# nlesc-dirac/sagecal

Measured on NVIDIA H100. Metric: baseline_visibilities_per_sec_predict_jacobian, higher is better.
Workload: dtype f64

## Files before the change

sagecal_b200/csrc/internal.cuh:

```cuda
#pragma once
#include <cuda_runtime.h>
#include <stdint.h>
#include <stdio.h>
#include <stdlib.h>

#define DB_CHECK(call)                                                                          \
  do {                                                                                          \
    cudaError_t err__ = (call);                                                                 \
    if (err__ != cudaSuccess) {                                                                 \
      fprintf(stderr, "dirac_b200: CUDA error %s at %s:%d: %s\n", cudaGetErrorName(err__),      \
              __FILE__, __LINE__, cudaGetErrorString(err__));                                   \
      exit(1);          \
    }                                                                                           \
  } while (0)


#define TILE_P 8
#define TILE_Q 32
#define TILE_THREADS (TILE_P * TILE_Q)

struct TileDesc {
  short pb, qb;
};

// ... 39 lines not shown
}
__host__ __device__ __forceinline__ double2 cadd(double2 a, double2 b) {
  return make_double2(a.x + b.x, a.y + b.y);
}
__host__ __device__ __forceinline__ double2 csub(double2 a, double2 b) {
  return make_double2(a.x - b.x, a.y - b.y);
}
__host__ __device__ __forceinline__ void cfma(double2 &acc, double2 a, double2 b) {
  acc.x = fma(a.x, b.x, acc.x);
  acc.x = fma(-a.y, b.y, acc.x);
  acc.y = fma(a.x, b.y, acc.y);
  acc.y = fma(a.y, b.x, acc.y);
}
__host__ __device__ __forceinline__ void cfmac(double2 &acc, double2 a, double2 b) {
  acc.x = fma(a.x, b.x, acc.x);
  acc.x = fma(a.y, b.y, acc.x);
  acc.y = fma(a.y, b.x, acc.y);
  acc.y = fma(-a.x, b.y, acc.y);
}
__host__ __device__ __forceinline__ void cfmacl(double2 &acc, double2 a, double2 b) {
  acc.x = fma(a.x, b.x, acc.x);
  acc.x = fma(a.y, b.y, acc.x);
  acc.y = fma(a.x, b.y, acc.y);
  acc.y = fma(-a.y, b.x, acc.y);
}

__host__ __device__ __forceinline__ double2 cdot2(double2 a0, double2 b0, double2 a1, double2 b1) {
  double re = a0.x * b0.x;
  re = fma(-a0.y, b0.y, re);
  re = fma(a1.x, b1.x, re);
  re = fma(-a1.y, b1.y, re);
  double im = a0.x * b0.y;
  im = fma(a0.y, b0.x, im);
  im = fma(a1.x, b1.y, im);
  im = fma(a1.y, b1.x, im);
  return make_double2(re, im);
}
__host__ __device__ __forceinline__ double2 cdot2c(double2 a0, double2 b0, double2 a1, double2 b1) {
  double re = a0.x * b0.x;
  re = fma(a0.y, b0.y, re);
  re = fma(a1.x, b1.x, re);
  re = fma(a1.y, b1.y, re);
  double im = a0.y * b0.x;
  im = fma(-a0.x, b0.y, im);
  im = fma(a1.y, b1.x, im);
  im = fma(-a1.x, b1.y, im);
  return make_double2(re, im);
}
__host__ __device__ __forceinline__ void cdot2c_acc(double2 &acc, double2 a0, double2 b0, double2 a1,
                                           double2 b1) {
  acc.x = fma(a0.x, b0.x, acc.x);
  acc.x = fma(a0.y, b0.y, acc.x);
  acc.x = fma(a1.x, b1.x, acc.x);
  acc.x = fma(a1.y, b1.y, acc.x);
  acc.y = fma(a0.y, b0.x, acc.y);
  acc.y = fma(-a0.x, b0.y, acc.y);
  acc.y = fma(a1.y, b1.x, acc.y);
  acc.y = fma(-a1.x, b1.y, acc.y);
}
__host__ __device__ __forceinline__ void mat_ab(const double2 *a, const double2 *b, double2 *c) {
  c[0] = cdot2(a[0], b[0], a[1], b[2]);
  c[1] = cdot2(a[0], b[1], a[1], b[3]);
  c[2] = cdot2(a[2], b[0], a[3], b[2]);
  c[3] = cdot2(a[2], b[1], a[3], b[3]);
}
__host__ __device__ __forceinline__ void mat_abh(const double2 *a, const double2 *b, double2 *c) {
  c[0] = cdot2c(a[0], b[0], a[1], b[1]);
  c[1] = cdot2c(a[0], b[2], a[1], b[3]);
  c[2] = cdot2c(a[2], b[0], a[3], b[1]);
  c[3] = cdot2c(a[2], b[2], a[3], b[3]);
}
__host__ __device__ __forceinline__ void mat_abh_acc(const double2 *a, const double2 *b, double2 *c) {
  cdot2c_acc(c[0], a[0], b[0], a[1], b[1]);
  cdot2c_acc(c[1], a[0], b[2], a[1], b[3]);
  cdot2c_acc(c[2], a[2], b[0], a[3], b[1]);
  cdot2c_acc(c[3], a[2], b[2], a[3], b[3]);
}
__host__ __device__ __forceinline__ void mat_ahb(const double2 *a, const double2 *b, double2 *c) {
  c[0] = cadd(cmulcl(a[0], b[0]), cmulcl(a[2], b[2]));
  c[1] = cadd(cmulcl(a[0], b[1]), cmulcl(a[2], b[3]));
  c[2] = cadd(cmulcl(a[1], b[0]), cmulcl(a[3], b[2]));
  c[3] = cadd(cmulcl(a[1], b[1]), cmulcl(a[3], b[3]));
}

__device__ __forceinline__ double2 ld_stream(const double2 *p) {
  double2 v;
  asm volatile("ld.global.nc.L1::no_allocate.v2.f64 {%0,%1}, [%2];" : "=d"(v.x), "=d"(v.y) : "l"(p));
  return v;
}
__device__ __forceinline__ void st_stream(double2 *p, double2 v) {
  asm volatile("st.global.L1::no_allocate.v2.f64 [%0], {%1,%2};" ::"l"(p), "d"(v.x), "d"(v.y)
               : "memory");
}

__device__ __forceinline__ double warp_sum(double v) {
#pragma unroll
  for (int o = 16; o > 0; o >>= 1) v += __shfl_xor_sync(0xffffffffu, v, o);
  return v;
}

__device__ __forceinline__ void load_jones(const double *pblk, int sta, double2 *J) {
  const double2 *s = reinterpret_cast<const double2 *>(pblk + 8 * (long long)sta);
  J[0] = __ldg(s + 0);
  J[1] = __ldg(s + 1);
  J[2] = __ldg(s + 2);
  J[3] = __ldg(s + 3);
}

__device__ __forceinline__ int row_chunk(long long r, long long R, int nchunk) {
  return nchunk == 1 ? 0 : (int)(r / ((R + nchunk - 1) / nchunk));
}

struct GradArgs {
  const double2 *coh;
  const double2 *res;
  const unsigned char *flag;
  const double *pp;
  const ClusterDesc *clus;
  const int *chunk_poff;
  const TileDesc *tiles;
  double *g;
  long long R;
  int N, Nbase, tilesz, M;
  int robust;
  double nu;
  double scale;
  int tb0;
  long long w_lo, w_hi;
};

struct ClusterPassArgs {
  const double2 *coh_k;
  const double2 *in;
  const unsigned char *flag;
  const double *pblk;
  const TileDesc *tiles;
  double2 *out;
  double *jte;
  double *partials;
  double *cost;
  unsigned int *counter;
  long long R;
  int N, Nbase;
  int t_begin, t_end, tslice;
  int mode;
  int write_out;
  double beta;
  const double *pblk_old;
  int form_hidden;
  const short2 *blpq;
  double *jte_part;
  unsigned int *gcounter;
  const double2 *wt;
};

struct WeightedJtjArgs {
  const double2 *coh_k;
  const double2 *wt;
  const unsigned char *flag;
  const double *pblk;
  const TileDesc *tiles;
  double *JTJ;
  double *HP, *HQ;
  long long R;
  int N, Nbase;
  int t_begin, t_end, tslice;
};

struct StreamAllArgs {
  const double2 *coh;
  const double2 *x;
  const unsigned char *flag;
  const double *pp;
  const double *pk;
  const ClusterDesc *clus;
  const int *chunk_poff;
  const short2 *blpq;
  double2 *out;
  double2 *E0, *E1, *E2;
  double *poly_part;
  double *partials, *cost;
  unsigned int *counter;
  long long R;
  int N, Nbase, tilesz, M;
  int out_mode, cost_mode;
  double inv_nu;
  int partial;
  long long row0;
  long long w_lo, w_hi;
};

struct GramArgs {
  const double2 *coh;
  const unsigned char *flag;
  const TileDesc *tiles;
  double *T;
  long long R;
  int N, Nbase;
  int k0;
  int t_begin, t_end, t_step;
};

struct AssembleArgs {
  const double *T;
  const double *pblk;
  const int *list;
  const int *tix;
  const int *poff;
  double *JTJ;
  long long stride;
  double *Hst;
  const double *mu_dev;
  double mu;
  int lower;
  int N, Nbase;
};

enum { DB_OPT_CP_ROWS = 0, DB_OPT_LINE_DIRECT = 1, DB_OPT_OS_CONSISTENT = 2,
       DB_OPT_RTR_NU_UNJOINED = 3, DB_OPT_ADMM_LM = 4, DB_OPT_SWEEP_RESIDUAL = 5,
       DB_OPT_COUNT = 8 };
int db_opt(int id);
int db_sm_count();
static inline int db_cp_max_slices(int Nbase, int tilesz) {
  const int nbg = (Nbase + 255) / 256;
  int nsl = (db_sm_count() + nbg - 1) / nbg;
  if ((tilesz + 31) / 32 > nsl) nsl = (tilesz + 31) / 32;
  return nsl;
}

extern "C" {
void db_launch_coh_to_planar(const double2 *src, double2 *dst, long long r0, int nr, int M,
                             long long R, cudaStream_t st);
void db_launch_coh_from_planar(const double2 *src, double2 *dst, long long r0, int nr, int M,
                               long long R, cudaStream_t st);
void db_launch_vis_to_planar(const double2 *src, double2 *dst, long long R, cudaStream_t st);
void db_launch_vis_from_planar(const double2 *src, double2 *dst, long long R, cudaStream_t st);
void db_launch_grad_tma(const GradArgs *a, int ntile, cudaStream_t st);
void db_launch_grad_window_tma(const GradArgs *a, int ntile, long long r_lo, long long r_hi,
                               cudaStream_t st);
void db_launch_grad_band_tma(const GradArgs *a, int ntile, int nchan, cudaStream_t st);
int db_cluster_pass_nblocks(int ntile, int nt, int tslice);
enum { DB_CP_LIN = 0, DB_CP_LIN_GRAD = 1, DB_CP_SPLIT = 2, DB_CP_TILE = 3, DB_CP_NONE = 4 };
int db_launch_cluster_pass(const ClusterPassArgs *a, int ntile, cudaStream_t st);
int db_cluster_pass_forms_hidden(int N, int Nbase);
void db_launch_coh_gram(const GramArgs *a, int ntile, int nk, cudaStream_t st);
void db_launch_station_sums(const AssembleArgs *a, int nb, cudaStream_t st);
void db_launch_assemble_tiles(const AssembleArgs *a, int nb, cudaStream_t st);
void db_launch_batch_mu0(const double *Hst, double *mu, int N, double tau, int nb, cudaStream_t st);
void db_launch_copy_add_diag(const double *A0, double *A, int n, double mu, cudaStream_t st);
int db_chol_max_n();
int db_chol_available();
size_t db_chol_ws_doubles(int n);
int db_tri_available(int n);
void db_chol_set_step(const double *pcur, double *pnew, double *sc, double *zero);
void db_launch_tri_solve(const double *L, int n, const double *b, double *x, cudaStream_t st);
void db_launch_tri_solve_ld(const double *L, int ld, int n, const double *b, double *x,
                            cudaStream_t st);
void db_launch_chol_factor_batched(const double *A, int n, const double *mu, double *ws,
                                   long long ws_stride, int *info, int nb, cudaStream_t st);
void db_launch_chol_solve(const double *A, int n, double mu, const double *b, double *x, double *ws,
                          int *info, cudaStream_t st);
int db_bigtri_available(int n);
size_t db_bigtri_ws_doubles(int n);
void db_launch_bigtri_solve(const double *L, int ld, int n, const double *b, double *x, double *ws,
                            int *status, cudaStream_t st);
int db_stream_all_nblocks(int Nbase, int tilesz);
void db_launch_predict_tma(const StreamAllArgs *a, cudaStream_t st);
void db_launch_cost_window_tma(const StreamAllArgs *a, cudaStream_t st);
int db_band_nblocks(int Nbase, int tilesz, int nchan);
void db_launch_band_tma(const StreamAllArgs *a, int nchan, cudaStream_t st);
void db_launch_band_tma(const StreamAllArgs *a, int nchan, cudaStream_t st);
unsigned db_launch_line_setup_tma(const StreamAllArgs *a, cudaStream_t st);
void db_launch_line_poly_finish(const double *part, unsigned nparts, double *partials, double *out,
                                unsigned int *counter, cudaStream_t st);
void db_line_setup_shape_reset();
void db_line_setup_shape(int *shape);
}
```

sagecal_b200/csrc/kernels_stream.cu:

```cuda
#include "internal.cuh"
#include "tma.cuh"

#define XP_ROWS 8
__global__ void k_coh_to_planar(const double2 *__restrict__ src, double2 *__restrict__ dst,
                                long long r0, int nr, int M, long long R) {
  __shared__ double2 tile[4][XP_ROWS][33];
  const int kx = blockIdx.x * 32 + threadIdx.x;
  const int ry = blockIdx.y * XP_ROWS + threadIdx.y;
  if (kx < M && ry < nr) {
    const double2 *s = src + ((long long)ry * M + kx) * 4;
#pragma unroll
    for (int c = 0; c < 4; c++) tile[c][threadIdx.y][threadIdx.x] = s[c];
  }
  __syncthreads();
  const int tid = threadIdx.y * 32 + threadIdx.x;
  const int rr = tid % XP_ROWS, kk = tid / XP_ROWS;
  const int k = blockIdx.x * 32 + kk;
  const int r = blockIdx.y * XP_ROWS + rr;
  if (k < M && r < nr) {
#pragma unroll
    for (int c = 0; c < 4; c++) dst[((long long)k * 4 + c) * R + r0 + r] = tile[c][rr][kk];
  }
}

// ... 353 lines not shown
          }
          if (a.write_out) st_stream(a.out + (long long)c * a.R + row, o);
        }
      }
      if (a.mode <= 1) {
        if (a.wt) {
#pragma unroll
          for (int c = 0; c < 4; c++) {
            const double2 wv = ld_stream(a.wt + (long long)c * a.R + row);
            const double ex = wv.x * e[c].x, ey = wv.y * e[c].y;
            cost = fma(ex, ex, cost);
            cost = fma(ey, ey, cost);
            e[c] = make_double2(wv.x * ex, wv.y * ey);
          }
        } else {
#pragma unroll
          for (int c = 0; c < 4; c++) {
            cost = fma(e[c].x, e[c].x, cost);
            cost = fma(e[c].y, e[c].y, cost);
          }
        }
      }
    }
  }
  if (a.mode <= 1) grid_reduce_sum(cost, a.partials, a.cost, a.counter);
}

__global__ void __launch_bounds__(2 * TILE_THREADS)
k_cluster_pass_split(ClusterPassArgs a) {
  __shared__ double sq[2 * TILE_P][8][TILE_Q];
  const TileDesc td = a.tiles[blockIdx.x];
  const int h = threadIdx.x >> 8, w = (threadIdx.x >> 5) & 7, lane = threadIdx.x & 31;
  const int p = td.pb * TILE_P + w;
  const int q = td.qb * TILE_Q + lane;
  const bool valid = (q > p) && (q < a.N);
  const int ts = a.t_begin + blockIdx.y * a.tslice;
  const int te = min(ts + a.tslice, a.t_end);
  double cost = 0.0;
  double2 Jr[2], Jq[4], W[8];
#pragma unroll
  for (int z = 0; z < 8; z++) W[z] = make_double2(0.0, 0.0);
  Jr[0] = Jr[1] = make_double2(0.0, 0.0);
#pragma unroll
  for (int c = 0; c < 4; c++) Jq[c] = make_double2(0.0, 0.0);
  if (valid) {
    {
      const double2 *jp = reinterpret_cast<const double2 *>(a.pblk + 8 * (long long)p + 4 * h);
      Jr[0] = __ldg(jp);
      Jr[1] = __ldg(jp + 1);
    }
    load_jones(a.pblk, q, Jq);
    const long long b = baseline_index(p, q, a.N);
    const long long c0 = (long long)(2 * h) * a.R, c1 = c0 + a.R;
#pragma unroll 2
    for (int t = ts; t < te; t++) {
      const long long row = (long long)t * a.Nbase + b;
      double2 C[4], v[2];
#pragma unroll
      for (int c = 0; c < 4; c++) C[c] = ld_stream(a.coh_k + (long long)c * a.R + row);
      v[0] = ld_stream(a.in + c0 + row);
      v[1] = ld_stream(a.in + c1 + row);
      const bool fl = a.flag[row] != 0;
      const double2 T0 = cdot2(Jr[0], C[0], Jr[1], C[2]);
      const double2 T1 = cdot2(Jr[0], C[1], Jr[1], C[3]);
      double2 m[2];
      m[0] = cdot2c(T0, Jq[0], T1, Jq[1]);
      m[1] = cdot2c(T0, Jq[2], T1, Jq[3]);
      if (fl) m[0] = m[1] = make_double2(0.0, 0.0);
      double2 e[2];
      if (a.mode == 0) {
#pragma unroll
        for (int j = 0; j < 2; j++) {
          const double2 d = cadd(make_double2(a.beta * v[j].x, a.beta * v[j].y), m[j]);
          if (a.write_out) st_stream(a.out + (j ? c1 : c0) + row, d);
          e[j] = csub(d, m[j]);
        }
      } else {
#pragma unroll
        for (int j = 0; j < 2; j++) {
          e[j] = (a.mode == 4) ? v[j] : csub(v[j], m[j]);
          if (a.write_out) st_stream(a.out + (j ? c1 : c0) + row, e[j]);
        }
      }
      if (a.wt) {
#pragma unroll
        for (int j = 0; j < 2; j++) {
          const double2 wv = ld_stream(a.wt + (j ? c1 : c0) + row);
          const double ex = wv.x * e[j].x, ey = wv.y * e[j].y;
          cost = fma(ex, ex, cost);
          cost = fma(ey, ey, cost);
          e[j] = make_double2(wv.x * ex, wv.y * ey);
        }
      } else {
#pragma unroll
        for (int j = 0; j < 2; j++) {
          cost = fma(e[j].x, e[j].x, cost);
          cost = fma(e[j].y, e[j].y, cost);
        }
      }
      if (!fl) {
#pragma unroll
        for (int j = 0; j < 2; j++)
#pragma unroll
          for (int lm = 0; lm < 4; lm++) cfmac(W[j * 4 + lm], e[j], C[lm]);
      }
    }
  }
  double2 Gp[2], Gq[4];
  Gp[0] = Gp[1] = make_double2(0.0, 0.0);
#pragma unroll
  for (int c = 0; c < 4; c++) Gq[c] = make_double2(0.0, 0.0);
  if (valid) {
#pragma unroll
    for (int l = 0; l < 2; l++)
#pragma unroll
      for (int j = 0; j < 2; j++)
#pragma unroll
        for (int m = 0; m < 2; m++) cfma(Gp[l], Jq[2 * j + m], W[j * 4 + l * 2 + m]);
#pragma unroll
    for (int j = 0; j < 2; j++)
#pragma unroll
      for (int m = 0; m < 2; m++)
#pragma unroll
        for (int l = 0; l < 2; l++) cfmac(Gq[2 * j + m], Jr[l], W[j * 4 + l * 2 + m]);
  }
  {
    double vp[4];
    vp[0] = warp_sum(Gp[0].x);
    vp[1] = warp_sum(Gp[0].y);
    vp[2] = warp_sum(Gp[1].x);
    vp[3] = warp_sum(Gp[1].y);
    if (p < a.N - 1 && lane < 4) {
      double v = vp[0];
#pragma unroll
      for (int c = 1; c < 4; c++) v = (lane == c) ? vp[c] : v;
      atomicAdd(a.jte + 8 * (long long)p + 4 * h + lane, v);
    }
  }
#pragma unroll
  for (int c = 0; c < 4; c++) {
    sq[h * TILE_P + w][2 * c][lane] = Gq[c].x;
    sq[h * TILE_P + w][2 * c + 1][lane] = Gq[c].y;
  }
  __syncthreads();
  if (h == 0) {
    double s = 0.0;
#pragma unroll
    for (int ww = 0; ww < 2 * TILE_P; ww++) s += sq[ww][w][lane];
    if (q < a.N && s != 0.0) atomicAdd(a.jte + 8 * (long long)q + w, s);
  }
  grid_reduce_sum(cost, a.partials, a.cost, a.counter);
}

template <int NST, bool GRAD>
__global__ void __launch_bounds__(512)
k_cluster_pass_lin(ClusterPassArgs a) {
  extern __shared__ __align__(128) unsigned char smem_raw[];
  constexpr int BL = 256;
  constexpr int STAGE_ELEMS = 8 * BL;
  double2 *ring = reinterpret_cast<double2 *>(smem_raw);
  double *acc = reinterpret_cast<double *>(ring + (size_t)NST * STAGE_ELEMS);
  unsigned long long *bars = reinterpret_cast<unsigned long long *>(acc + ((8 * a.N + 1) & ~1));
  const int tid = threadIdx.x, h = tid >> 8, bl = tid & (BL - 1);
  const long long b0 = (long long)blockIdx.x * BL;
  const int nvalid = (int)min((long long)BL, (long long)a.Nbase - b0);
  const bool valid = bl < nvalid;
  const int ts = a.t_begin + blockIdx.y * a.tslice;
  const int te = min(ts + a.tslice, a.t_end);
  const int nrow = te - ts;
  if (GRAD)
    for (int i = tid; i < 8 * a.N; i += 512) acc[i] = 0.0;
  if (tid == 0) {
#pragma unroll
    for (int s = 0; s < NST; s++) mbar_init(&bars[s], 1);
    mbar_fence_init();
  }
  __syncthreads();
  auto issue = [&](int j, int s) {
    const unsigned row_bytes = (unsigned)nvalid * 16u;
    const long long row0 = (long long)(ts + j) * a.Nbase + b0;
    double2 *dst = ring + (size_t)s * STAGE_ELEMS;
    mbar_expect_tx(&bars[s], 8u * row_bytes);
#pragma unroll
    for (int c = 0; c < 4; c++) {
      bulk_g2s(dst + c * BL, a.coh_k + (long long)c * a.R + row0, row_bytes, &bars[s]);
      bulk_g2s(dst + (4 + c) * BL, a.in + (long long)c * a.R + row0, row_bytes, &bars[s]);
    }
  };
  if (tid == 0) {
#pragma unroll
    for (int s = 0; s < NST - 1; s++)
      if (s < nrow) issue(s, s);
  }
  int p = 0, q = 0;
  double2 Jr[2], Jq[4], W[8];
#pragma unroll
  for (int z = 0; z < 8; z++) W[z] = make_double2(0.0, 0.0);
  Jr[0] = Jr[1] = make_double2(0.0, 0.0);
#pragma unroll
  for (int c = 0; c < 4; c++) Jq[c] = make_double2(0.0, 0.0);
  unsigned flagbits = 0;
  const long long b = b0 + bl;
  const bool recover = (!GRAD) && a.mode == 3 && a.pblk_old != nullptr && !a.form_hidden;
  const bool old_model = recover || a.form_hidden;
  const double gamma = recover ? (1.0 - a.beta) / a.beta : 0.0;
  double2 Jro[2], Jqo[4];
  Jro[0] = Jro[1] = make_double2(0.0, 0.0);
#pragma unroll
  for (int c = 0; c < 4; c++) Jqo[c] = make_double2(0.0, 0.0);
  auto load_old_jones = [&]() {
    const double2 *jo = reinterpret_cast<const double2 *>(a.pblk_old + 8 * (long long)p + 4 * h);
    Jro[0] = __ldg(jo);
    Jro[1] = __ldg(jo + 1);
    load_jones(a.pblk_old, q, Jqo);
  };
  if (valid) {
    const short2 pq = a.blpq[b];
    p = pq.x;
    q = pq.y;
    const double2 *jp = reinterpret_cast<const double2 *>(a.pblk + 8 * (long long)p + 4 * h);
    Jr[0] = __ldg(jp);
    Jr[1] = __ldg(jp + 1);
    load_jones(a.pblk, q, Jq);
    if (old_model && !GRAD) load_old_jones();
    for (int j = 0; j < nrow; j++)
      flagbits |= (a.flag[(long long)(ts + j) * a.Nbase + b] != 0 ? 1u : 0u) << j;
  }
  const long long c0 = (long long)(2 * h) * a.R, c1 = c0 + a.R;
  double cost = 0.0;
  for (int j = 0; j < nrow; j++) {
    const int s = j % NST;
    if (tid == 0 && j + NST - 1 < nrow) issue(j + NST - 1, (j + NST - 1) % NST);
    mbar_wait(&bars[s], (unsigned)((j / NST) & 1));
    if (valid) {
      const double2 *st = ring + (size_t)s * STAGE_ELEMS + bl;
      const long long row = (long long)(ts + j) * a.Nbase + b;
      double2 C[4], v[2];
#pragma unroll
      for (int c = 0; c < 4; c++) C[c] = lds_v2(st + c * BL);
      v[0] = lds_v2(st + (4 + 2 * h) * BL);
      v[1] = lds_v2(st + (5 + 2 * h) * BL);
      const bool fl = (flagbits >> j) & 1u;
      const double2 T0 = cdot2(Jr[0], C[0], Jr[1], C[2]);
      const double2 T1 = cdot2(Jr[0], C[1], Jr[1], C[3]);
      double2 m[2];
      m[0] = cdot2c(T0, Jq[0], T1, Jq[1]);
      m[1] = cdot2c(T0, Jq[2], T1, Jq[3]);
      if (fl) m[0] = m[1] = make_double2(0.0, 0.0);
      double2 mo[2];
      if (old_model) {
        if (GRAD) load_old_jones();
        const double2 U0 = cdot2(Jro[0], C[0], Jro[1], C[2]);
        const double2 U1 = cdot2(Jro[0], C[1], Jro[1], C[3]);
        mo[0] = cdot2c(U0, Jqo[0], U1, Jqo[1]);
        mo[1] = cdot2c(U0, Jqo[2], U1, Jqo[3]);
        if (fl) mo[0] = mo[1] = make_double2(0.0, 0.0);
      }
      if (a.form_hidden) {
#pragma unroll
        for (int jj = 0; jj < 2; jj++)
          v[jj] = cadd(make_double2(a.beta * v[jj].x, a.beta * v[jj].y), mo[jj]);
      }
      double2 e[2];
      if (a.mode == 0 || a.mode == 2) {
#pragma unroll
        for (int jj = 0; jj < 2; jj++) {
          const double2 d = cadd(make_double2(a.beta * v[jj].x, a.beta * v[jj].y), m[jj]);
          if (a.write_out) st_stream(a.out + (jj ? c1 : c0) + row, d);
          e[jj] = csub(d, m[jj]);
        }
      } else {
#pragma unroll
        for (int jj = 0; jj < 2; jj++) {
          e[jj] = csub(v[jj], m[jj]);
          double2 o = e[jj];
          if (recover) {
            o.x = fma(gamma, v[jj].x - mo[jj].x, o.x);
            o.y = fma(gamma, v[jj].y - mo[jj].y, o.y);
          }
          if (a.write_out) st_stream(a.out + (jj ? c1 : c0) + row, o);
        }
      }
      if (a.mode <= 1) {
#pragma unroll
        for (int jj = 0; jj < 2; jj++) {
          cost = fma(e[jj].x, e[jj].x, cost);
          cost = fma(e[jj].y, e[jj].y, cost);
        }
      }
      if (GRAD && !fl) {
#pragma unroll
        for (int jj = 0; jj < 2; jj++)
#pragma unroll
          for (int lm = 0; lm < 4; lm++) cfmac(W[jj * 4 + lm], e[jj], C[lm]);
      }
    }
    __syncthreads();
  }
  if (!GRAD) {
    if (a.mode <= 1) grid_reduce_sum(cost, a.partials, a.cost, a.counter);
    return;
  }
  double2 Gp[2], Gq[4];
  Gp[0] = Gp[1] = make_double2(0.0, 0.0);
#pragma unroll
  for (int c = 0; c < 4; c++) Gq[c] = make_double2(0.0, 0.0);
  if (valid) {
#pragma unroll
    for (int l = 0; l < 2; l++)
#pragma unroll
      for (int jj = 0; jj < 2; jj++)
#pragma unroll
        for (int m = 0; m < 2; m++) cfma(Gp[l], Jq[2 * jj + m], W[jj * 4 + l * 2 + m]);
#pragma unroll
    for (int jj = 0; jj < 2; jj++)
#pragma unroll
      for (int m = 0; m < 2; m++)
#pragma unroll
        for (int l = 0; l < 2; l++) cfmac(Gq[2 * jj + m], Jr[l], W[jj * 4 + l * 2 + m]);
  }
  double *gq = reinterpret_cast<double *>(ring);
  double *gp = gq + 512 * 8;
#pragma unroll
  for (int c = 0; c < 4; c++) {
    gq[tid * 8 + 2 * c] = Gq[c].x;
    gq[tid * 8 + 2 * c + 1] = Gq[c].y;
  }
  gp[tid * 4 + 0] = Gp[0].x;
  gp[tid * 4 + 1] = Gp[0].y;
  gp[tid * 4 + 2] = Gp[1].x;
  gp[tid * 4 + 3] = Gp[1].y;
  __syncthreads();
  const int pmin = a.blpq[b0].x, pmax = a.blpq[b0 + nvalid - 1].x;
  for (int i = tid; i < 8 * a.N; i += 512) {
    const int sidx = i >> 3, comp = i & 7;
    double tot = 0.0;
    for (int pp = pmin; pp <= pmax && pp < sidx; pp++) {
      const long long bb = baseline_index(pp, sidx, a.N) - b0;
      if (bb >= 0 && bb < nvalid) tot += gq[bb * 8 + comp] + gq[(256 + bb) * 8 + comp];
    }
    if (sidx >= pmin && sidx <= pmax) {
      const int hh = comp >> 2, cc = comp & 3;
      long long bb = baseline_index(sidx, sidx + 1, a.N) - b0;
      long long be = bb + (a.N - 1 - sidx);
      if (bb < 0) bb = 0;
      if (be > nvalid) be = nvalid;
      for (; bb < be; bb++) tot += gp[(hh * 256 + bb) * 4 + cc];
    }
    acc[i] = tot;
  }
  {
    __shared__ bool last_of_group;
    const int n8 = 8 * a.N;
    double *grp = a.jte_part + (size_t)blockIdx.x * gridDim.y * n8;
    double *mine = grp + (size_t)blockIdx.y * n8;
    for (int i = tid; i < n8; i += 512) mine[i] = acc[i];
    __threadfence();
    __syncthreads();
    if (tid == 0) last_of_group = (atomicAdd(a.gcounter + blockIdx.x, 1u) == gridDim.y - 1);
    __syncthreads();
    if (last_of_group) {
      __threadfence();
      for (int i = tid; i < n8; i += 512) {
        double sacc = 0.0;
        for (unsigned c = 0; c < gridDim.y; c++) sacc += __ldcg(grp + (size_t)c * n8 + i);
        if (sacc != 0.0) atomicAdd(a.jte + i, sacc);
      }
      if (tid == 0) a.gcounter[blockIdx.x] = 0;
    }
  }
  grid_reduce_sum(cost, a.partials, a.cost, a.counter);
}


__global__ void __launch_bounds__(TILE_THREADS)
k_coh_gram(GramArgs a) {
  const TileDesc td = a.tiles[blockIdx.x];
  const int w = threadIdx.x >> 5, lane = threadIdx.x & 31;
  const int p = td.pb * TILE_P + w;
  const int q = td.qb * TILE_Q + lane;
  if (!((q > p) && (q < a.N))) return;
  const long long b = baseline_index(p, q, a.N);
  const double2 *ck = a.coh + (long long)(a.k0 + blockIdx.y) * 4 * a.R;
  double d[4] = {0.0, 0.0, 0.0, 0.0};
  double2 o[6];
#pragma unroll
  for (int z = 0; z < 6; z++) o[z] = make_double2(0.0, 0.0);
#pragma unroll 4
  for (int t = a.t_begin; t < a.t_end; t += a.t_step) {
    const long long row = (long long)t * a.Nbase + b;
    double2 C[4];
#pragma unroll
    for (int c = 0; c < 4; c++) C[c] = ld_stream(ck + (long long)c * a.R + row);
    if (a.flag[row] == 0) {
#pragma unroll
      for (int c = 0; c < 4; c++) {
        d[c] = fma(C[c].x, C[c].x, d[c]);
        d[c] = fma(C[c].y, C[c].y, d[c]);
      }
      cfmacl(o[0], C[0], C[1]);
      cfmacl(o[1], C[0], C[2]);
      cfmacl(o[2], C[0], C[3]);
      cfmacl(o[3], C[1], C[2]);
      cfmacl(o[4], C[1], C[3]);
      cfmacl(o[5], C[2], C[3]);
    }
  }
  double2 *Tb = reinterpret_cast<double2 *>(a.T + ((long long)blockIdx.y * a.Nbase + b) * 16);
  Tb[0] = make_double2(d[0], d[1]);
  Tb[1] = make_double2(d[2], d[3]);
#pragma unroll
  for (int z = 0; z < 6; z++) Tb[2 + z] = o[z];
}

void db_launch_grad_tma(const GradArgs *a, int ntile, cudaStream_t st) {
  constexpr int TB = 4, NST = 2;
  const size_t smem = sizeof(double) * 2 * TILE_P * 8 * TILE_Q +
                      (size_t)TILE_P * NST * TB * 4 * 32 * sizeof(double2) + TILE_P * NST * 8;
  static bool configured = false;
  if (!configured) {
    DB_CHECK(cudaFuncSetAttribute(k_grad_tma_split<TB, NST>,
                                  cudaFuncAttributeMaxDynamicSharedMemorySize, (int)smem));
    configured = true;
  }
  dim3 grid(ntile, (a->tilesz + TB - 1) / TB);
  k_grad_tma_split<TB, NST><<<grid, 2 * TILE_THREADS, smem, st>>>(*a);
}

void db_launch_grad_band_tma(const GradArgs *a, int ntile, int nchan, cudaStream_t st) {
  constexpr int TB = 4, NST = 2;
  const size_t smem = sizeof(double) * 2 * TILE_P * 8 * TILE_Q +
                      (size_t)TILE_P * NST * TB * 4 * 32 * sizeof(double2) + TILE_P * NST * 8;
  static bool configured = false;
  if (!configured) {
    DB_CHECK(cudaFuncSetAttribute(k_grad_tma_band<TB, NST>,
                                  cudaFuncAttributeMaxDynamicSharedMemorySize, (int)smem));
    configured = true;
  }
  dim3 grid(ntile, (a->tilesz + TB - 1) / TB, nchan);
  k_grad_tma_band<TB, NST><<<grid, 2 * TILE_THREADS, smem, st>>>(*a);
}

void db_launch_grad_window_tma(const GradArgs *a, int ntile, long long r_lo, long long r_hi,
                               cudaStream_t st) {
  constexpr int TB = 4, NST = 2;
  if (r_hi <= r_lo) return;
  const size_t smem = sizeof(double) * 2 * TILE_P * 8 * TILE_Q +
                      (size_t)TILE_P * NST * TB * 4 * 32 * sizeof(double2) + TILE_P * NST * 8;
  static bool configured = false;
  if (!configured) {
    DB_CHECK(cudaFuncSetAttribute(k_grad_tma_window<TB, NST>,
                                  cudaFuncAttributeMaxDynamicSharedMemorySize, (int)smem));
    configured = true;
  }
  const int t_lo = (int)(r_lo / a->Nbase), t_hi = (int)((r_hi + a->Nbase - 1) / a->Nbase);
  const int tb_lo = t_lo / TB, tb_hi = (t_hi + TB - 1) / TB;
  GradArgs b = *a;
  b.tb0 = tb_lo;
  b.w_lo = r_lo;
  b.w_hi = r_hi;
  dim3 grid(ntile, tb_hi - tb_lo);
  k_grad_tma_window<TB, NST><<<grid, 2 * TILE_THREADS, smem, st>>>(b);
}

static bool cluster_pass_lin_fits(int N, int Nbase) {
  return (size_t)5 * 8 * 256 * sizeof(double2) + sizeof(double) * ((8 * N + 1) & ~1) + 40 <=
             (size_t)200 * 1024 && (Nbase + 255) / 256 <= 1024;
}

template <bool GRAD>
static void launch_cluster_pass_lin(const ClusterPassArgs *a, cudaStream_t st) {
  constexpr int NST = 5;
  const int nt = a->t_end - a->t_begin;
  const int nbg = (a->Nbase + 255) / 256;
  int nsl = (db_sm_count() + nbg - 1) / nbg;
  if (nsl > nt) nsl = nt;
  ClusterPassArgs b = *a;
  b.tslice = (nt + nsl - 1) / nsl;
  const int forced = db_opt(DB_OPT_CP_ROWS);
  if (forced > 0 && (!GRAD || (nt + forced - 1) / forced <= db_cp_max_slices(a->Nbase, nt)))
    b.tslice = forced;
  if (b.tslice > nt) b.tslice = nt;
  if (b.tslice > 32) b.tslice = 32;
  const size_t smem = (size_t)NST * 8 * 256 * sizeof(double2) +
                      sizeof(double) * ((8 * a->N + 1) & ~1) + NST * 8;
  static bool configured = false;
  if (!configured) {
    DB_CHECK(cudaFuncSetAttribute(k_cluster_pass_lin<NST, GRAD>,
                                  cudaFuncAttributeMaxDynamicSharedMemorySize, 200 * 1024));
    configured = true;
  }
  dim3 grid(nbg, (nt + b.tslice - 1) / b.tslice);
  k_cluster_pass_lin<NST, GRAD><<<grid, 512, smem, st>>>(b);
}

extern "C" {

void db_launch_coh_to_planar(const double2 *src, double2 *dst, long long r0, int nr, int M,
                             long long R, cudaStream_t st) {
  dim3 block(32, XP_ROWS), grid((M + 31) / 32, (nr + XP_ROWS - 1) / XP_ROWS);
  k_coh_to_planar<<<grid, block, 0, st>>>(src, dst, r0, nr, M, R);
}
void db_launch_coh_from_planar(const double2 *src, double2 *dst, long long r0, int nr, int M,
                               long long R, cudaStream_t st) {
  dim3 block(32, XP_ROWS), grid((M + 31) / 32, (nr + XP_ROWS - 1) / XP_ROWS);
  k_coh_from_planar<<<grid, block, 0, st>>>(src, dst, r0, nr, M, R);
}
void db_launch_vis_to_planar(const double2 *src, double2 *dst, long long R, cudaStream_t st) {
  long long n = 4 * R;
  k_vis_to_planar<<<(unsigned)((n + 255) / 256), 256, 0, st>>>(src, dst, R);
}
void db_launch_vis_from_planar(const double2 *src, double2 *dst, long long R, cudaStream_t st) {
  long long n = 4 * R;
  k_vis_from_planar<<<(unsigned)((n + 255) / 256), 256, 0, st>>>(src, dst, R);
}

int db_cluster_pass_nblocks(int ntile, int nt, int tslice) { return ntile * ((nt + tslice - 1) / tslice); }
int db_cluster_pass_forms_hidden(int N, int Nbase) { return cluster_pass_lin_fits(N, Nbase); }
int db_launch_cluster_pass(const ClusterPassArgs *a, int ntile, cudaStream_t st) {
  int nt = a->t_end - a->t_begin;
  dim3 grid(ntile, (nt + a->tslice - 1) / a->tslice);
  if (a->form_hidden && (a->wt || !db_cluster_pass_forms_hidden(a->N, a->Nbase))) {
    fprintf(stderr, "dirac_b200: cluster pass that forms the hidden data requested where only the tile "
                    "kernels run (%s:%d)\n", __FILE__, __LINE__);
    exit(1);
  }
  const bool fits = cluster_pass_lin_fits(a->N, a->Nbase);
  if (a->jte == nullptr || (a->mode > 1 && a->mode != 4)) {
    if (!a->wt && fits) {
      launch_cluster_pass_lin<false>(a, st);
      return DB_CP_LIN;
    }
    k_cluster_pass<<<grid, TILE_THREADS, 0, st>>>(*a);
    return DB_CP_TILE;
  } else if (a->mode == 4 || a->wt || !fits) {
    k_cluster_pass_split<<<grid, 2 * TILE_THREADS, 0, st>>>(*a);
    return DB_CP_SPLIT;
  }
  launch_cluster_pass_lin<true>(a, st);
  return DB_CP_LIN_GRAD;
}
void db_launch_coh_gram(const GramArgs *a, int ntile, int nk, cudaStream_t st) {
  dim3 grid(ntile, nk);
  k_coh_gram<<<grid, TILE_THREADS, 0, st>>>(*a);
}

}
```

sagecal_b200/csrc/lm.cu:

```cuda
#include <float.h>
#include <math.h>
#include <string.h>
#include <vector>

#include "../../include/dirac_b200.h"
#include "problem.h"

#define CS_CHECK(call)                                                                     \
  do {                                                                                     \
    cusolverStatus_t s__ = (call);                                                         \
    if (s__ != CUSOLVER_STATUS_SUCCESS) {                                                  \
      fprintf(stderr, "dirac_b200: cuSOLVER error %d at %s:%d\n", (int)s__, __FILE__, __LINE__); \
      exit(1);                                                                             \
    }                                                                                      \
  } while (0)
#define CB_CHECK(call)                                                                     \
  do {                                                                                     \
    cublasStatus_t s__ = (call);                                                           \
    if (s__ != CUBLAS_STATUS_SUCCESS) {                                                    \
      fprintf(stderr, "dirac_b200: cuBLAS error %d at %s:%d\n", (int)s__, __FILE__, __LINE__); \
      exit(1);                                                                             \
    }                                                                                      \
  } while (0)

extern "C" {
void db_launch_weighted_jtj(const WeightedJtjArgs *a, int ntile, cudaStream_t st);
void db_launch_sum_abs(const double2 *v, long long R, long long r0, long long r1, double *partials,
                       double *out, unsigned int *counter, cudaStream_t st);
void db_launch_update_weights(const double2 *e, double2 *wt, long long R, long long r0,
                              long long r1, double nu0, double *partials, double *out,
                              unsigned int *counter, cudaStream_t st);
void db_launch_scale_vis(double2 *v, long long R, long long r0, long long r1, double alpha,
                         int set_const, cudaStream_t st);
void db_launch_extract_diag(const double *A, double *dst, int n, cudaStream_t st);
void db_launch_lm_step(const double *p, const double *Dp, const double *jte, double *pnew,
                       double *sc, double *zero, int n, cudaStream_t st);
void db_launch_os_shift(const double2 *e, const double2 *wt, double2 *eps, double2 *wout, long long R,
                        long long row_sub0, long long nrow_sub, long long row_chunk0, long long kl,
                        long long nJ, cudaStream_t st);
}

template <typename T>
static T *dalloc(size_t n) {
  return (T *)db_malloc(n * sizeof(T) + 16);
}

void db_lm_init(dirac_b200_problem *pr) {
  LMWork &w = pr->lm;
  if (w.ready) return;
  DevProblem &d = pr->d;
  const int n8 = 8 * d.N;
  w.n8 = n8;
  w.T = dalloc<double>((size_t)d.Mt * d.Nbase * 16);
  w.T_valid = (unsigned char *)calloc(d.Mt, 1);
  w.Tsub = dalloc<double>((size_t)d.Nbase * 16);
  w.JTJ0 = dalloc<double>((size_t)n8 * n8);
  w.JTJ = dalloc<double>((size_t)n8 * n8);
  w.JTe = d.scal + 64 + n8;
  w.JTe_new = d.scal + 64 + 2 * n8;
  w.Hst = dalloc<double>((size_t)4 * d.N);
  w.Dp = d.scal + 64;
  w.pnew = dalloc<double>(n8);
  w.plast = dalloc<double>(n8);
  w.pold = dalloc<double>(n8);
  w.devinfo = reinterpret_cast<int *>(d.scal + 64 + 3 * n8);
  w.tau = dalloc<double>(n8);
  w.svdS = w.svdU = w.svdVT = nullptr;
  w.wbuf = w.ebuf = nullptr;
  w.os_eps = w.os_w = nullptr;
  w.HP = w.HQ = nullptr;
  w.JB = w.LB = nullptr;
  w.sys_T = w.sys_p = w.sys_H = nullptr;
  w.pref_slot = (int *)malloc(sizeof(int) * d.M);
  for (int k = 0; k < d.M; k++) w.pref_slot[k] = -1;
  w.jtj0_cur = nullptr;
  w.jtj_spec = nullptr;
  {
    const int nbg = (d.Nbase + 255) / 256;
    const int nsl = db_cp_max_slices(d.Nbase, d.tilesz);
    w.jte_part = dalloc<double>((size_t)nbg * (nsl + 1) * n8);
  }
  DB_CHECK(cudaEventCreateWithFlags(&w.ev_mail, cudaEventDisableTiming));
  DB_CHECK(cudaMallocHost((void **)&w.h_vec, sizeof(double) * (5 * n8 + 4 * d.N + 64)));
  static cusolverDnHandle_t g_cs = nullptr;
  static cublasHandle_t g_cb = nullptr;
  if (!g_cs) {
    CS_CHECK(cusolverDnCreate(&g_cs));
    CB_CHECK(cublasCreate(&g_cb));
  }
  w.cs = g_cs;
  w.cb = g_cb;
  CS_CHECK(cusolverDnSetStream(w.cs, d.stream));
  CB_CHECK(cublasSetStream(w.cb, d.stream));
  int l1 = 0, l2 = 0, l3 = 0;
  CS_CHECK(cusolverDnDpotrf_bufferSize(w.cs, CUBLAS_FILL_MODE_LOWER, n8, w.JTJ, n8, &l1));
  CS_CHECK(cusolverDnDgeqrf_bufferSize(w.cs, n8, n8, w.JTJ, n8, &l2));
  CS_CHECK(cusolverDnDormqr_bufferSize(w.cs, CUBLAS_SIDE_LEFT, CUBLAS_OP_T, n8, 1, n8, w.JTJ, n8,
                                       w.tau, w.Dp, n8, &l3));
  w.lwork = l1 > l2 ? l1 : l2;
  if (l3 > w.lwork) w.lwork = l3;
  int l4 = 0;
  CS_CHECK(cusolverDnDgesvd_bufferSize(w.cs, n8, n8, &l4));
  if (l4 > w.lwork) w.lwork = l4;
  w.own_chol = n8 <= db_chol_max_n() && db_chol_available() && !getenv("DIRAC_B200_CUSOLVER");
  if (w.own_chol && (size_t)w.lwork < db_chol_ws_doubles(n8)) w.lwork = (int)db_chol_ws_doubles(n8);
  w.cswork = dalloc<double>((size_t)w.lwork);
  w.bc = (!w.own_chol && n8 > 1024) ? db_bigchol_create(n8, BC_BLOCK, BC_INV_PANEL, BC_LOOKAHEAD) : nullptr;
  w.bt_ws = (!w.own_chol && db_bigtri_available(n8)) ? dalloc<double>(db_bigtri_ws_doubles(n8)) : nullptr;
  w.dbuf = dalloc<double2>((size_t)4 * d.R);
  w.ready = true;
}

static void robust_init(dirac_b200_problem *pr) {
  LMWork &w = pr->lm;
  if (w.wbuf) return;
  DevProblem &d = pr->d;
  w.wbuf = dalloc<double2>((size_t)4 * d.R);
  w.ebuf = dalloc<double2>((size_t)4 * d.R);
  w.HP = dalloc<double>((size_t)d.N * 20);
  w.HQ = dalloc<double>((size_t)d.N * 20);
}

static void os_init(dirac_b200_problem *pr) {
  robust_init(pr);
  LMWork &w = pr->lm;
  if (w.os_eps) return;
  w.os_eps = dalloc<double2>((size_t)4 * pr->d.R);
  w.os_w = dalloc<double2>((size_t)4 * pr->d.R);
}

void db_lm_free(dirac_b200_problem *pr) {
  LMWork &w = pr->lm;
  if (!w.ready) return;
  db_free(w.T); db_free(w.Tsub); db_free(w.JTJ0); db_free(w.JTJ);
  db_free(w.Hst); db_free(w.pnew); db_free(w.plast); db_free(w.pold); db_free(w.jte_part);
  db_free(w.tau); db_free(w.cswork); db_free(w.dbuf);
  if (w.bt_ws) db_free(w.bt_ws);
  db_bigchol_destroy(w.bc);
  if (w.svdS) { db_free(w.svdS); db_free(w.svdU); db_free(w.svdVT); }
  if (w.wbuf) { db_free(w.wbuf); db_free(w.ebuf); db_free(w.HP); db_free(w.HQ); }
  if (w.os_eps) { db_free(w.os_eps); db_free(w.os_w); }
  if (w.LB) {
    if (w.JB) db_free(w.JB);
    db_free(w.LB); db_free(w.HB); db_free(w.mu_dev); db_free(w.binfo_dev);
    db_free(w.LBptr_dev); db_free(w.blist_dev); db_free(w.btix_dev); db_free(w.bpoff_dev);
    cudaFreeHost(w.h_mu); cudaFreeHost(w.h_binfo);
  }
  free(w.pref_slot);
  cudaEventDestroy(w.ev_mail);
  cudaFreeHost(w.h_vec);
  free(w.T_valid);
  w.ready = false;
}

static int pick_tslice(const DevProblem &d, int nt) {
  int target_ctas = db_sm_count();
  int slices = (target_ctas + d.ntile - 1) / d.ntile;
  if (slices < 1) slices = 1;
  int ts = (nt + slices - 1) / slices;
  if (ts < 2) ts = 2;
  if (ts > nt) ts = nt;
  if (ts < 1) ts = 1;
  return ts;
}

int db_cluster_pass(dirac_b200_problem *pr, int k, const double *pblk_dev, const double2 *in,
                    double2 *out, int mode, int write_out, double *jte_dev, int cost_slot, int t0,
                    int t1, const double2 *wt, double beta = 1.0, bool jte_zeroed = false,
                    const double *pblk_old = nullptr, bool form_hidden = false);

int db_cluster_pass(dirac_b200_problem *pr, int k, const double *pblk_dev, const double2 *in,
                    double2 *out, int mode, int write_out, double *jte_dev, int cost_slot, int t0,
                    int t1, const double2 *wt, double beta, bool jte_zeroed,
                    const double *pblk_old, bool form_hidden) {
  DevProblem &d = pr->d;
  if (t1 <= t0) {
    if (mode <= 1 || mode == 4)
      DB_CHECK(cudaMemsetAsync(d.scal + cost_slot, 0, sizeof(double), d.stream));
    if (jte_dev) DB_CHECK(cudaMemsetAsync(jte_dev, 0, sizeof(double) * 8 * d.N, d.stream));
    return DB_CP_NONE;
  }
  ClusterPassArgs a;
  a.coh_k = d.coh + (size_t)k * 4 * d.R;
  a.in = in; a.flag = d.flag; a.pblk = pblk_dev; a.tiles = d.tiles; a.out = out; a.jte = jte_dev;
  a.blpq = d.blpq; a.jte_part = pr->lm.jte_part; a.gcounter = d.counters + 16;
  a.partials = pr->partials; a.cost = d.scal + cost_slot; a.counter = d.counters; a.R = d.R;
  a.N = d.N; a.Nbase = d.Nbase; a.t_begin = t0; a.t_end = t1; a.tslice = pick_tslice(d, t1 - t0);
  a.mode = mode; a.write_out = write_out; a.wt = wt; a.beta = beta;
  a.pblk_old = pblk_old; a.form_hidden = form_hidden;
  if (!(jte_dev && (mode <= 1 || mode == 4)) && a.tslice > 1)
    a.tslice = (a.tslice + 1) / 2;
  if (jte_dev && (mode <= 1 || mode == 4) && !jte_zeroed)
    DB_CHECK(cudaMemsetAsync(jte_dev, 0, sizeof(double) * 8 * d.N, d.stream));
  db_prof_begin((jte_dev && (mode <= 1 || mode == 4)) ? 2 : 8, (double)(t1 - t0) * d.Nbase * (129.0 + (write_out ? 64.0 : 0.0) +
                                                 (wt ? 64.0 : 0.0)), d.stream);
  const int kernel = db_launch_cluster_pass(&a, d.ntile, d.stream);
  db_prof_end(d.stream);
  db_count_launch(1);
  return kernel;
}

static void gram(dirac_b200_problem *pr, int k, int t0, int t1, int step, double *Tdst) {
  DevProblem &d = pr->d;
  GramArgs a;
  a.coh = d.coh; a.flag = d.flag; a.tiles = d.tiles; a.T = Tdst; a.R = d.R; a.N = d.N;
  a.Nbase = d.Nbase; a.k0 = k; a.t_begin = t0; a.t_end = t1; a.t_step = step;
  db_prof_begin(3, (double)((t1 - t0 + step - 1) / step) * d.Nbase * 65.0 + 128.0 * d.Nbase,
                d.stream);
  db_launch_coh_gram(&a, d.ntile, 1, d.stream);
  db_prof_end(d.stream);
  db_count_launch(1);
}

static AssembleArgs assemble_args(const DevProblem &d, const double *T, const double *pblk_dev,
                                  double *Hst) {
  AssembleArgs a;
  memset(&a, 0, sizeof(a));
  a.T = T; a.pblk = pblk_dev; a.Hst = Hst; a.N = d.N; a.Nbase = d.Nbase;
  return a;
}

static void station_sums(dirac_b200_problem *pr, const AssembleArgs &a, int nb) {
  DevProblem &d = pr->d;
  db_prof_begin(4, nb * 256.0 * d.Nbase, d.stream);
  db_launch_station_sums(&a, nb, d.stream);
  db_prof_end(d.stream);
  db_count_launch(1);
}

static void assemble_tiles(dirac_b200_problem *pr, const AssembleArgs &a, int nb) {
  DevProblem &d = pr->d;
  const double n = 8.0 * d.N;
  db_prof_begin(4, nb * (a.lower ? 128.0 * d.Nbase + 4.0 * n * (n + 1) : 256.0 * d.Nbase + 8.0 * n * n),
                d.stream);
  db_launch_assemble_tiles(&a, nb, d.stream);
  db_prof_end(d.stream);
  db_count_launch(1);
}

static void assemble(dirac_b200_problem *pr, const double *T, const double *pblk_dev,
                     double *JTJ) {
  AssembleArgs a = assemble_args(pr->d, T, pblk_dev, pr->lm.Hst);
  station_sums(pr, a, 1);
  if (!JTJ) return;
  a.JTJ = JTJ;
  assemble_tiles(pr, a, 1);
}

static void weighted_jtj(dirac_b200_problem *pr, int k, int t0, int t1, const double *pblk_dev,
                         const double2 *wt, double *JTJ) {
  DevProblem &d = pr->d;
  LMWork &w = pr->lm;
  const int n = w.n8;
  DB_CHECK(cudaMemsetAsync(JTJ, 0, sizeof(double) * (size_t)n * n, d.stream));
  DB_CHECK(cudaMemsetAsync(w.HP, 0, sizeof(double) * 20 * d.N, d.stream));
  DB_CHECK(cudaMemsetAsync(w.HQ, 0, sizeof(double) * 20 * d.N, d.stream));
  if (t1 <= t0) return;
  WeightedJtjArgs a;
  a.coh_k = d.coh + (size_t)k * 4 * d.R;
  a.wt = wt; a.flag = d.flag; a.pblk = pblk_dev; a.tiles = d.tiles; a.JTJ = JTJ; a.HP = w.HP;
  a.HQ = w.HQ; a.R = d.R; a.N = d.N; a.Nbase = d.Nbase; a.t_begin = t0; a.t_end = t1;
  a.tslice = pick_tslice(d, t1 - t0);
  db_prof_begin(6, (double)(t1 - t0) * d.Nbase * 129.0 + 8.0 * 64.0 * d.N * d.N, d.stream);
  db_launch_weighted_jtj(&a, d.ntile, d.stream);
  db_prof_end(d.stream);
  db_count_launch(2);
}

void db_chunk_range(const DevProblem &d, int k, int ck, int *t0, int *t1);
static void chunk_range(const DevProblem &d, int k, int ck, int *t0, int *t1) {
  db_chunk_range(d, k, ck, t0, t1);
}
void db_chunk_range(const DevProblem &d, int k, int ck, int *t0, int *t1) {
  int nchunk = d.h_clus[k].nchunk;
  int tilechunk = (d.tilesz + nchunk - 1) / nchunk;
  int a = ck * tilechunk;
  int b = a + tilechunk;
  if (a > d.tilesz) a = d.tilesz;
  if (b > d.tilesz) b = d.tilesz;
  *t0 = a;
  *t1 = b;
}

static int enqueue_solve(dirac_b200_problem *pr, double mu, int linsolv, double eps1) {
  DevProblem &d = pr->d;
  LMWork &w = pr->lm;
  const int n = w.n8;
  int *hinfo = (int *)(w.h_vec + 4 * n + 4 * d.N);
  hinfo[0] = hinfo[1] = 0;
  if (linsolv == 0 && w.own_chol) {
    db_prof_begin(5, 0.0, d.stream);
    db_launch_chol_solve(w.jtj0_cur ? w.jtj0_cur : w.JTJ0, n, mu, w.JTe, w.Dp, w.cswork, w.devinfo,
                         d.stream);
    db_prof_end(d.stream);
    db_count_launch(1);
    w.step_fused = w.step_armed;
    return 1;
  }
  if (linsolv == 0 && w.sys_T) {
    AssembleArgs a = assemble_args(d, w.sys_T, w.sys_p, const_cast<double *>(w.sys_H));
    a.JTJ = w.JTJ;
    a.mu = mu;
    a.lower = 1;
    assemble_tiles(pr, a, 1);
  } else {
    db_prof_begin(4, 16.0 * n * n, d.stream);
    db_launch_copy_add_diag(w.jtj0_cur ? w.jtj0_cur : w.JTJ0, w.JTJ, n, mu, d.stream);
    db_prof_end(d.stream);
    db_count_launch(1);
  }
  if (linsolv != 0 || !w.bt_ws)
    DB_CHECK(cudaMemcpyAsync(w.Dp, w.JTe, sizeof(double) * n, cudaMemcpyDeviceToDevice, d.stream));
  db_prof_begin(5, 0.0, d.stream);
  if (linsolv == 0) {
    CS_CHECK(cusolverDnDpotrf(w.cs, CUBLAS_FILL_MODE_LOWER, n, w.JTJ, n, w.cswork, w.lwork,
                              w.devinfo));
    if (w.bt_ws) {
      db_launch_bigtri_solve(w.JTJ, n, n, w.JTe, w.Dp, w.bt_ws, w.devinfo + 1, d.stream);
      db_count_launch(2);
    } else {
      CS_CHECK(cusolverDnDpotrs(w.cs, CUBLAS_FILL_MODE_LOWER, n, 1, w.JTJ, n, w.Dp, n,
                                w.devinfo + 1));
      db_count_launch(2);
    }
  } else if (linsolv == 1) {
    CS_CHECK(cusolverDnDgeqrf(w.cs, n, n, w.JTJ, n, w.tau, w.cswork, w.lwork, w.devinfo));
    CS_CHECK(cusolverDnDormqr(w.cs, CUBLAS_SIDE_LEFT, CUBLAS_OP_T, n, 1, n, w.JTJ, n, w.tau, w.Dp,
                              n, w.cswork, w.lwork, w.devinfo + 1));
    const double one = 1.0;
    CB_CHECK(cublasDtrsm(w.cb, CUBLAS_SIDE_LEFT, CUBLAS_FILL_MODE_UPPER, CUBLAS_OP_N,
                         CUBLAS_DIAG_NON_UNIT, n, 1, &one, w.JTJ, n, w.Dp, n));
    db_count_launch(3);
  } else {
    if (!w.svdS) {
      w.svdS = dalloc<double>(n);
      w.svdU = dalloc<double>((size_t)n * n);
      w.svdVT = dalloc<double>((size_t)n * n);
    }
    CS_CHECK(cusolverDnDgesvd(w.cs, 'A', 'A', n, n, w.JTJ, n, w.svdS, w.svdU, n, w.svdVT, n,
                              w.cswork, w.lwork, nullptr, w.devinfo));
    db_count_launch(1);
    double *hS = (double *)malloc(sizeof(double) * n);
    double *hb = (double *)malloc(sizeof(double) * n);
    const double one = 1.0, zero = 0.0;
    CB_CHECK(cublasDgemv(w.cb, CUBLAS_OP_T, n, n, &one, w.svdU, n, w.JTe, 1, &zero, w.Dp, 1));
    DB_CHECK(cudaMemcpyAsync(hS, w.svdS, sizeof(double) * n, cudaMemcpyDeviceToHost, d.stream));
    DB_CHECK(cudaMemcpyAsync(hb, w.Dp, sizeof(double) * n, cudaMemcpyDeviceToHost, d.stream));
    db_stream_sync(d.stream);
// ... 95 lines not shown
  db_launch_batch_mu0(w.HB, w.mu_dev, d.N, tau, nb, d.stream);
  db_count_launch(1);
  if (keep_jb) {
    b.JTJ = w.JB;
    b.stride = (long long)nn;
    assemble_tiles(pr, b, nb);
  }
  if (!own_batch) {
    b.JTJ = w.LB;
    b.stride = (long long)lstride;
    b.mu_dev = w.mu_dev;
    b.lower = 1;
    assemble_tiles(pr, b, nb);
  }
  db_prof_begin(5, 0.0, d.stream);
  if (own_batch) {
    db_launch_chol_factor_batched(w.JB, n, w.mu_dev, w.LB, (long long)lstride, w.binfo_dev, nb,
                                  d.stream);
    db_count_launch(1);
  } else if (!w.bc) {
    CS_CHECK(cusolverDnDpotrfBatched(w.cs, CUBLAS_FILL_MODE_LOWER, n, w.LBptr_dev, n, w.binfo_dev, nb));
    db_count_launch(1);
  } else {
    db_bigchol_factor_batch(w.bc, nb, w.binfo_dev, 1, d.stream);
  }
  db_prof_end(d.stream);
  DB_CHECK(cudaMemcpyAsync(w.h_mu, w.mu_dev, sizeof(double) * nb, cudaMemcpyDeviceToHost, d.stream));
  DB_CHECK(cudaMemcpyAsync(w.h_binfo, w.binfo_dev, sizeof(int) * (own_batch ? 2 * nb : nb),
                           cudaMemcpyDeviceToHost, d.stream));
  w.binfo_step = own_batch ? 2 : 1;
  db_stream_sync(d.stream);
}

static long g_noise_decisions = 0;
static long g_lm_stat[4] = {0, 0, 0, 0};
extern "C" void dirac_b200_lm_stats(long *out4, int reset) {
  for (int i = 0; i < 4; i++) {
    if (out4) out4[i] = g_lm_stat[i];
    if (reset) g_lm_stat[i] = 0;
  }
}
extern "C" long dirac_b200_noise_decisions(int reset) {
  const long v = g_noise_decisions;
  if (reset) g_noise_decisions = 0;
  return v;
}

struct LmAug {
  const double *y_dev, *bz_dev;
  const double *y_host, *bz_host;
  double rho;
};
static const LmAug *g_aug = nullptr;
static std::vector<double> g_hpnew;
static double *hpnew_aug(LMWork &w) {
  if ((int)g_hpnew.size() < w.n8) g_hpnew.resize(w.n8);
  return g_hpnew.data();
}
static double aug_cost(const LmAug *a, const double *p, int n) {
  double s = 0.0;
  for (int i = 0; i < n; i++) {
    const double dlt = p[i] - a->bz_host[i];
    s += a->y_host[i] * dlt + 0.5 * a->rho * dlt * dlt;
  }
  return s;
}
extern "C" void db_launch_lm_aug_rhs(double *jte, const double *p, const double *y, const double *bz,
                                     double rho, int n, cudaStream_t st);

struct LmOut {
  double init_eL2, eL2, jacTe_inf, Dp_L2, mu;
  int k, stop;
  bool res_in_dbuf;
};

struct OsLayout {
  int Nsubsets, Ntper;
  bool misaligned;
};
static OsLayout os_layout(int ntiles) {
  OsLayout o;
  o.Nsubsets = ntiles < 10 ? ntiles : 10;
  o.Ntper = o.Nsubsets > 0 ? (ntiles + o.Nsubsets - 1) / o.Nsubsets : ntiles;
  o.misaligned = o.Nsubsets > 0 && (ntiles % o.Nsubsets) != 0 && !db_opt(DB_OPT_OS_CONSISTENT);
  return o;
}

struct OsPath {
  bool misaligned;
  int s0, s1;
  long long nJ;
};

static OsPath os_subset_system(dirac_b200_problem *pr, int k, int t0, int t1, int l,
                               const double *pblk_dev, const double2 *wt) {
  DevProblem &d = pr->d;
  LMWork &w = pr->lm;
  const int ntiles = t1 - t0;
  const OsLayout L = os_layout(ntiles);
  const int Ntper = L.Ntper;
  OsPath path;
  path.misaligned = L.misaligned;
  path.nJ = 0;
  int s0 = t0 + l * Ntper;
  int s1 = (l * Ntper + Ntper < ntiles) ? s0 + Ntper : t1;
  if (s0 > t1) s0 = t1;
  if (!L.misaligned) {
    db_cluster_pass(pr, k, pblk_dev, w.dbuf, nullptr, 1, 0, w.JTe, 2, s0, s1, wt);
    if (wt) {
      weighted_jtj(pr, k, s0, s1, pblk_dev, wt, w.JTJ0);
    } else {
      gram(pr, k, s0, s1, 1, w.Tsub);
      assemble(pr, w.Tsub, pblk_dev, w.JTJ0);
    }
  } else {
    const long long nn = 8ll * ntiles * d.Nbase;
    const long long Nper = (nn + L.Nsubsets - 1) / L.Nsubsets;
    const long long kl = (long long)l * Nper;
    const int tl = l * Ntper;
    long long Nos;
    int tileI;
    if (tl + Ntper < ntiles) {
      Nos = Nper;
      tileI = Ntper;
    } else {
      Nos = nn - kl;
      tileI = ntiles - tl;
    }
    long long nJ = tileI > 0 ? 8ll * d.Nbase * tileI : 0;
    if (Nos < nJ) nJ = Nos;
    if (nJ < 0) nJ = 0;
    s0 = t0 + tl;
    s1 = s0 + (tileI > 0 ? tileI : 0);
    if (s0 > t1) s0 = s1 = t1;
    os_init(pr);
    db_cluster_pass(pr, k, pblk_dev, w.dbuf, w.ebuf, 1, 1, nullptr, 2, t0, t1, nullptr);
    if (s1 > s0) {
      db_launch_os_shift(w.ebuf, wt, w.os_eps, w.os_w, d.R, (long long)s0 * d.Nbase,
                         (long long)(s1 - s0) * d.Nbase, (long long)t0 * d.Nbase, kl, nJ, d.stream);
      db_count_launch(1);
    }
    db_cluster_pass(pr, k, pblk_dev, w.os_eps, nullptr, 4, 0, w.JTe, 2, s0, s1, w.os_w);
    weighted_jtj(pr, k, s0, s1, pblk_dev, w.os_w, w.JTJ0);
    path.nJ = nJ;
  }
  path.s0 = s0;
  path.s1 = s1;
  return path;
}

static void lm_core(dirac_b200_problem *pr, int k, int ck, int t0, int t1, double *pblk_dev,
                    const double2 *wt, int itmax, const double *opts, int linsolv, int os,
                    int os_shift, int randomize, bool have_first, double first_cost, int *nu_damp,
                    bool *evaluated_trial, const double2 *hidden_from, LmOut *out) {
  DevProblem &d = pr->d;
  LMWork &w = pr->lm;
  const int n = w.n8;
  const int ntiles = t1 - t0;
  const double tau = opts[0], eps1 = opts[1], eps2 = opts[2], eps2_sq = opts[2] * opts[2],
               eps3 = opts[3];
  double *hp = w.h_vec;
  double *hjte = w.h_vec + n;
  double *hDp = w.h_vec + 2 * n;
  double *hpnew = w.h_vec + 3 * n;
  double *hH = w.h_vec + 4 * n;

  double p_eL2;
  const LmAug *aug = (!os && !wt) ? g_aug : nullptr;
  const double half_rho = aug ? 0.5 * aug->rho : 0.0;
  if (aug) w.pref_slot[k] = -1;
  const bool defer = have_first && !os && !wt && linsolv == 0 && itmax > 0 && w.pref_slot[k] >= 0 &&
                     std::isnan(first_cost);
  DB_CHECK(cudaMemcpyAsync(hp, pblk_dev, sizeof(double) * n, cudaMemcpyDeviceToHost, d.stream));
  if (aug && have_first)
    db_launch_lm_aug_rhs(w.JTe, pblk_dev, aug->y_dev, aug->bz_dev, aug->rho, n, d.stream);
  if (have_first) {
    p_eL2 = first_cost;
    if (!defer) {
      if (!os)
        DB_CHECK(cudaMemcpyAsync(hjte, w.JTe, sizeof(double) * n, cudaMemcpyDeviceToHost,
                                 d.stream));
      if (std::isnan(first_cost))
        DB_CHECK(cudaMemcpyAsync(d.h_scal + 2, d.scal + 2, sizeof(double), cudaMemcpyDeviceToHost,
                                 d.stream));
      db_stream_sync(d.stream);
      if (std::isnan(first_cost)) p_eL2 = d.h_scal[2];
    } else {
      p_eL2 = 1.0;
    }
  } else {
    db_cluster_pass(pr, k, pblk_dev, w.dbuf, nullptr, 1, 0, os ? nullptr : w.JTe, 1, t0, t1, wt);
    if (aug) db_launch_lm_aug_rhs(w.JTe, pblk_dev, aug->y_dev, aug->bz_dev, aug->rho, n, d.stream);
    if (!os)
      DB_CHECK(cudaMemcpyAsync(hjte, w.JTe, sizeof(double) * n, cudaMemcpyDeviceToHost, d.stream));
    p_eL2 = db_read_scalar(pr, 1);
  }
  if (aug && !defer) p_eL2 += aug_cost(aug, hp, n);
  double init_p_eL2 = p_eL2;
  int stop = 0;
  if (!isfinite(p_eL2)) stop = 7;
  int nu = *nu_damp, nu2;
  double mu = 0.0, Dp_L2 = DBL_MAX, jacTe_inf = 0.0;
  *evaluated_trial = false;
  bool res_in_dbuf = false;
  bool pending_entry = defer;
  w.jtj_spec = nullptr;
  int kiter_adjust = 0;

  const OsLayout osl = os_layout(ntiles);
  const int Nsubsets = osl.Nsubsets;
  const int max_os_iter = os ? (int)ceil(0.1 * (double)Nsubsets) : 1;
  const bool os_misaligned = os && osl.misaligned;

  const int tix = d.h_clus[k].chunk0 + ck;
  double *Tfull = w.T + (size_t)tix * d.Nbase * 16;
  if (!wt && !os && !w.T_valid[tix] && ntiles > 0) {
    gram(pr, k, t0, t1, 1, Tfull);
    w.T_valid[tix] = 1;
  }

  double *hsc = w.h_vec + 4 * n + 4 * d.N + 8;
  double *hjte_new = hpnew;
  int kiter;
  std::vector<int> subI;
  for (kiter = 0; kiter < itmax && !stop; ++kiter) {
    if (!pending_entry && p_eL2 <= eps3) {
      stop = 6;
      break;
    }
    if (os && randomize) {
      subI.resize(Nsubsets);
      for (int i = 0; i < Nsubsets; ++i) {
        const int j = rand() % (i + 1);
        subI[i] = subI[j];
        subI[j] = i;
      }
    }
    for (int ositer = 0; ositer < max_os_iter; ositer++) {
      double mx = 0.0;
      const int slot = (!wt && !os && kiter == 0 && linsolv == 0) ? w.pref_slot[k] : -1;
      const bool prefac = slot >= 0;
      const bool need_mx = (kiter == 0) && !prefac;
      w.jtj0_cur = (prefac && w.JB) ? w.JB + (size_t)slot * n * n : nullptr;
      const bool in_place = !w.own_chol && linsolv == 0 && !wt && !os;
      w.sys_T = in_place ? Tfull : nullptr;
      w.sys_p = pblk_dev;
      w.sys_H = prefac ? w.HB + (size_t)slot * 4 * d.N : w.Hst;
      if (os) {
        const int l = randomize ? subI[ositer] : (os_shift + kiter + ositer) % Nsubsets;
        os_subset_system(pr, k, t0, t1, l, pblk_dev, wt);
        DB_CHECK(cudaMemcpyAsync(hjte, w.JTe, sizeof(double) * n, cudaMemcpyDeviceToHost,
                                 d.stream));
      } else if (prefac) {
        w.pref_slot[k] = -1;
      } else if (wt) {
        weighted_jtj(pr, k, t0, t1, pblk_dev, wt, w.JTJ0);
      } else if (w.jtj_spec) {
        w.jtj0_cur = w.jtj_spec;
        w.jtj_spec = nullptr;
      } else {
        assemble(pr, Tfull, pblk_dev, in_place ? nullptr : w.JTJ0);
      }
      if (need_mx) {
        if (wt || os_misaligned) {
          db_launch_extract_diag(w.JTJ0, w.JTe_new, n, d.stream);
          db_count_launch(1);
          DB_CHECK(cudaMemcpyAsync(hsc, w.JTe_new, sizeof(double) * n, cudaMemcpyDeviceToHost,
                                   d.stream));
        } else {
          DB_CHECK(cudaMemcpyAsync(hH, w.Hst, sizeof(double) * 4 * d.N, cudaMemcpyDeviceToHost,
                                   d.stream));
        }
      }
      if (need_mx || os) db_stream_sync(d.stream);
      if (need_mx) {
        if (wt || os_misaligned) {
          for (int i = 0; i < n; i++)
            if (fabs(hsc[i]) > fabs(mx)) mx = hsc[i];
        } else {
          for (int s = 0; s < d.N; s++) {
            if (fabs(hH[4 * s]) > fabs(mx)) mx = hH[4 * s];
            if (fabs(hH[4 * s + 1]) > fabs(mx)) mx = hH[4 * s + 1];
          }
        }
      }
      double p_L2 = 0.0;
      if (!pending_entry) {
        jacTe_inf = 0.0;
        for (int i = 0; i < n; i++) {
          double a = fabs(hjte[i]);
          if (a > jacTe_inf) jacTe_inf = a;
        }
        p_L2 = nrm2sq(hp, n);
        if (jacTe_inf <= eps1) {
          Dp_L2 = 0.0;
          stop = 1;
          if (!os) kiter_adjust = 1;
          break;
        }
      }
      if (kiter == 0) mu = prefac ? w.h_mu[slot] : tau * (mx + half_rho);
      bool use_factor = prefac;
      while (1) {
        int issolved;
        bool skip_info = false;
        w.step_fused = false;
        w.step_armed = w.own_chol && linsolv == 0;
        if (w.step_armed)
          db_chol_set_step(pblk_dev, w.pnew, d.scal + 8, os ? nullptr : w.JTe_new);
        if (use_factor) {
          use_factor = false;
          db_prof_begin(5, 0.0, d.stream);
          if (w.own_chol && db_tri_available(n)) {
            skip_info = true;
            db_launch_tri_solve_ld(w.LB + (size_t)slot * w.lb_stride, w.lb_ld, n, w.JTe, w.Dp,
                                   d.stream);
            w.step_fused = w.step_armed;
          } else if (w.bt_ws) {
            skip_info = true;
            db_launch_bigtri_solve(w.LB + (size_t)slot * w.lb_stride, n, n, w.JTe, w.Dp, w.bt_ws,
                                   nullptr, d.stream);
          } else {
            DB_CHECK(cudaMemsetAsync(w.devinfo, 0, 2 * sizeof(int), d.stream));
            DB_CHECK(cudaMemcpyAsync(w.Dp, w.JTe, sizeof(double) * n, cudaMemcpyDeviceToDevice,
                                     d.stream));
            CS_CHECK(cusolverDnDpotrs(w.cs, CUBLAS_FILL_MODE_LOWER, n, 1,
                                      w.LB + (size_t)slot * w.lb_stride, n, w.Dp, n, w.devinfo + 1));
          }
          db_prof_end(d.stream);
          db_count_launch(1);
          issolved = (w.h_binfo[slot * w.binfo_step] == 0) ? 1 : 0;
        } else {
          issolved = enqueue_solve(pr, mu + half_rho, linsolv, eps1);
        }
        if (w.step_armed) db_chol_set_step(nullptr, nullptr, nullptr, nullptr);
        if (!w.step_fused)
          db_launch_lm_step(pblk_dev, w.Dp, w.JTe, w.pnew, d.scal + 8, os ? nullptr : w.JTe_new, n,
                            d.stream);
        if (hidden_from) {
          const bool last = kiter == itmax - 1;
          db_cluster_pass(pr, k, w.pnew, hidden_from, last ? w.dbuf : nullptr, 1, last ? 1 : 0,
                          last ? nullptr : w.JTe_new, 1, t0, t1, nullptr, 1.0, true, w.pold,
                          true);
        } else {
          db_cluster_pass(pr, k, w.pnew, w.dbuf, nullptr, 1, 0, os ? nullptr : w.JTe_new, 1, t0, t1,
                          wt, 1.0, true);
        }
        if (aug)
          db_launch_lm_aug_rhs(w.JTe_new, w.pnew, aug->y_dev, aug->bz_dev, aug->rho, n, d.stream);
        if (!w.step_fused) db_count_launch(1);
        int *hinfo = (int *)(w.h_vec + 4 * n + 4 * d.N);
        DB_CHECK(cudaMemcpyAsync(d.h_scal, d.scal, sizeof(double) * (64 + 3 * n + 2),
                                 cudaMemcpyDeviceToHost, d.stream));
        double *spec_buf = nullptr;
        if (w.own_chol && linsolv == 0 && !wt && !os && kiter + 1 < itmax && w.T_valid[tix]) {
          const double *cur = w.jtj0_cur ? w.jtj0_cur : w.JTJ0;
          spec_buf = (cur == w.JTJ0) ? w.JTJ : w.JTJ0;
          DB_CHECK(cudaEventRecord(w.ev_mail, d.stream));
          assemble(pr, Tfull, w.pnew, spec_buf);
          db_event_sync(w.ev_mail);
        } else {
          db_stream_sync(d.stream);
        }
        {
          const double *hm = d.h_scal + 64;
          memcpy(hDp, hm, sizeof(double) * n);
          hsc[n] = d.h_scal[8];
          hsc[n + 1] = d.h_scal[9];
          hsc[n + 2] = d.h_scal[1];
          if (!os) memcpy(hjte_new, hm + (w.JTe_new - w.Dp), sizeof(double) * n);
          if (pending_entry) memcpy(hjte, hm + (w.JTe - w.Dp), sizeof(double) * n);
          memcpy(hinfo, hm + 3 * n, 2 * sizeof(int));
          if (skip_info) hinfo[0] = hinfo[1] = 0;
        }
        if (pending_entry) {
          pending_entry = false;
          p_eL2 = init_p_eL2 = d.h_scal[2];
          if (!isfinite(p_eL2)) {
            stop = 7;
            kiter_adjust = 1;
            break;
          }
          if (p_eL2 <= eps3) {
            stop = 6;
            kiter_adjust = 1;
            break;
          }
          jacTe_inf = 0.0;
          for (int i = 0; i < n; i++) {
            double a = fabs(hjte[i]);
            if (a > jacTe_inf) jacTe_inf = a;
          }
          p_L2 = nrm2sq(hp, n);
          if (jacTe_inf <= eps1) {
            Dp_L2 = 0.0;
            stop = 1;
            kiter_adjust = 1;
            break;
          }
        }
        if (issolved && linsolv != 2) issolved = (hinfo[0] == 0 && hinfo[1] == 0) ? 1 : 0;
        if (issolved) {
          Dp_L2 = hsc[n];
          if (Dp_L2 <= eps2_sq * p_L2) {
            stop = 2;
            break;
          }
          if (Dp_L2 >= (p_L2 + eps2) / (1e-12 * 1e-12)) {
            stop = 4;
            break;
          }
          if (wt)
            DB_CHECK(cudaMemcpyAsync(w.plast, w.pnew, sizeof(double) * n, cudaMemcpyDeviceToDevice,
                                     d.stream));
          *evaluated_trial = true;
          double pDp_eL2 = hsc[n + 2];
          if (aug) {
            for (int i = 0; i < n; i++) hpnew_aug(w)[i] = hp[i] + hDp[i];
            pDp_eL2 += aug_cost(aug, hpnew_aug(w), n);
          }
          if (!isfinite(pDp_eL2)) {
            stop = 7;
            break;
          }
          const double dL = mu * Dp_L2 + hsc[n + 1];
          const double dF = p_eL2 - pDp_eL2;
          if (fabs(dF) <= 1e-11 * p_eL2) g_noise_decisions++;
          if (dL > 0.0 && dF > 0.0) {
            double tmp = (2.0 * dF / dL - 1.0);
            tmp = 1.0 - tmp * tmp * tmp;
            mu = mu * ((tmp >= 0.3333333334) ? tmp : 0.3333333334);
            g_lm_stat[0]++;
            if (!(tmp >= 0.3333333334)) g_lm_stat[1]++;
            nu = 2;
            for (int i = 0; i < n; i++) hp[i] += hDp[i];
            DB_CHECK(cudaMemcpyAsync(pblk_dev, w.pnew, sizeof(double) * n,
                                     cudaMemcpyDeviceToDevice, d.stream));
            if (!os) {
              memcpy(hjte, hjte_new, sizeof(double) * n);
              double *t = w.JTe; w.JTe = w.JTe_new; w.JTe_new = t;
            }
            p_eL2 = pDp_eL2;
            w.jtj_spec = spec_buf;
            res_in_dbuf = hidden_from && kiter == itmax - 1;
            break;
          }
        }
        g_lm_stat[2]++;
        mu *= (double)nu;
        nu2 = nu << 1;
        if (nu2 <= nu) {
          stop = 5;
          break;
        }
        nu = nu2;
      }
      if (stop) break;
    }
  }
  if (kiter >= itmax && !kiter_adjust) stop = 3;
  kiter -= kiter_adjust;
  *nu_damp = nu;
  out->init_eL2 = init_p_eL2;
  out->eL2 = p_eL2;
  out->jacTe_inf = jacTe_inf;
  out->Dp_L2 = Dp_L2;
  out->mu = mu;
  out->k = kiter;
  out->stop = stop;
  out->res_in_dbuf = res_in_dbuf;
}

static void fill_info(double *info, const LmOut &o) {
  if (!info) return;
  info[0] = o.init_eL2; info[1] = o.eL2; info[2] = o.jacTe_inf; info[3] = o.Dp_L2; info[4] = o.mu;
  info[5] = (double)o.k; info[6] = (double)o.stop;
  info[7] = info[8] = info[9] = 0.0;
}

void db_lm_set_aug(const double *y_dev, const double *bz_dev, const double *y_host,
                   const double *bz_host, double rho) {
  static LmAug a;
  if (!y_dev) {
    g_aug = nullptr;
    return;
  }
  a.y_dev = y_dev; a.bz_dev = bz_dev; a.y_host = y_host; a.bz_host = bz_host; a.rho = rho;
  g_aug = &a;
}

void db_lm_chunk(dirac_b200_problem *pr, int k, int ck, double *pblk_dev, double2 *r, int itmax,
                 const double *opts, int linsolv, int os, int randomize, double *info,
                 bool hidden_ready) {
  static const double defopts[4] = {1e-3, 1e-17, 1e-17, 1e-17};
  DevProblem &d = pr->d;
  db_lm_init(pr);
  LMWork &w = pr->lm;
  int t0, t1;
  chunk_range(d, k, ck, &t0, &t1);
  if (hidden_ready) {
    int nu = 2;
    bool ev;
    LmOut o;
    lm_core(pr, k, ck, t0, t1, pblk_dev, nullptr, itmax, opts ? opts : defopts, linsolv, os, 0,
            randomize, false, 0.0, &nu, &ev, nullptr, &o);
    fill_info(info, o);
    return;
  }
  const double beta = pr->world > 1 ? pr->beta : 1.0;
  const bool form = !os && pr->world <= 1 && d.h_clus[k].nchunk == 1 && r == pr->res &&
                    db_cluster_pass_forms_hidden(d.N, d.Nbase);
  if (beta != 1.0 || form)
    DB_CHECK(cudaMemcpyAsync(w.pold, pblk_dev, sizeof(double) * w.n8, cudaMemcpyDeviceToDevice,
                             d.stream));
  db_cluster_pass(pr, k, pblk_dev, r, form ? nullptr : w.dbuf, 0, form ? 0 : 1,
                  os ? nullptr : w.JTe, 2, t0, t1, nullptr, beta);
  const double c0 = nan("");
  int nu = 2;
  bool ev;
  LmOut o;
  lm_core(pr, k, ck, t0, t1, pblk_dev, nullptr, itmax, opts ? opts : defopts, linsolv, os, 0,
          randomize, true, c0, &nu, &ev, form ? r : nullptr, &o);
  if (o.res_in_dbuf) {
    pr->res = w.dbuf;
    w.dbuf = r;
  } else if (form) {
    db_cluster_pass(pr, k, pblk_dev, r, r, 3, 1, nullptr, 1, t0, t1, nullptr, 1.0, false,
                    w.pold, true);
  } else {
    db_cluster_pass(pr, k, pblk_dev, w.dbuf, r, 3, 1, nullptr, 1, t0, t1, nullptr, beta,
                    false, beta != 1.0 ? w.pold : nullptr);
  }
  fill_info(info, o);
}

bool db_cluster_needs_rowmap(const dirac_b200_problem *pr, int k) {
  const int nchunk = pr->d.h_clus[k].nchunk;
  return nchunk > 1 && (pr->d.tilesz % nchunk) != 0;
}
void db_cluster_hidden(dirac_b200_problem *pr, int k, double2 *r, int sign, double beta) {
  DevProblem &d = pr->d;
  db_lm_init(pr);
  LMWork &w = pr->lm;
  const double2 *coh_k = d.coh + (size_t)k * 4 * d.R;
  const int *poff = d.chunk_poff + d.h_clus[k].chunk0;
  if (sign > 0)
    db_launch_cluster_rowmap(coh_k, r, nullptr, w.dbuf, d.flag, d.pp, poff, d.h_clus[k].nchunk,
                             d.blpq, d.R, d.Nbase, 1, beta, d.stream);
  else
    db_launch_cluster_rowmap(coh_k, w.dbuf, beta != 1.0 ? r : nullptr, r, d.flag, d.pp, poff,
                             d.h_clus[k].nchunk, d.blpq, d.R, d.Nbase, -1, beta, d.stream);
  db_count_launch(1);
}

static double digamma_(double x) {
  double result = 0.0, xx, xx2, xx4;
  for (; x < 7.0; ++x) result -= 1.0 / x;
  x -= 0.5;
  xx = 1.0 / x;
  xx2 = xx * xx;
  xx4 = xx2 * xx2;
  result += log(x) + (1. / 24.) * xx2 - (7.0 / 960.0) * xx4 + (31.0 / 8064.0) * xx4 * xx2 -
            (127.0 / 30720.0) * xx4 * xx4;
  return result;
}

static double pick_nu(double sumq, double nulow, double nuhigh) {
  const int Nd = 30;
  const double deltanu = (nuhigh - nulow) / (double)Nd;
  int best = 0;
  double bestv = 0.0;
  for (int ci = 0; ci < Nd; ci++) {
    const double thisnu = nulow + (double)ci * deltanu;
    double q = digamma_(thisnu * 0.5 + 0.5) - log((thisnu + 1.0) * 0.5);
    q += -digamma_(thisnu * 0.5) + log(thisnu * 0.5);
    q += -sumq + 1.0;
    if (ci == 0 || fabs(q) < bestv) {
      bestv = fabs(q);
      best = ci;
    }
  }
  return nulow + (double)best * deltanu;
}

static double irls_update(dirac_b200_problem *pr, int k, int t0, int t1, const double *pe,
                          double nu0, double nulow, double nuhigh, double *out3) {
  DevProblem &d = pr->d;
  LMWork &w = pr->lm;
  const long long r0 = (long long)t0 * d.Nbase, r1 = (long long)t1 * d.Nbase;
  const double ndata = 8.0 * (double)(r1 - r0);
  db_cluster_pass(pr, k, pe, w.dbuf, w.ebuf, 1, 1, nullptr, 2, t0, t1, nullptr);
  db_launch_sum_abs(w.wbuf, d.R, r0, r1, pr->partials, d.scal + 3, d.counters, d.stream);
  db_launch_update_weights(w.ebuf, w.wbuf, d.R, r0, r1, nu0, pr->partials, d.scal + 4, d.counters,
                           d.stream);
  db_count_launch(2);
  DB_CHECK(cudaMemcpyAsync(d.h_scal + 3, d.scal + 3, 2 * sizeof(double), cudaMemcpyDeviceToHost,
                           d.stream));
  db_stream_sync(d.stream);
  const double lambda = d.h_scal[3];
  const double sumq = d.h_scal[4] / ndata;
  const double nu = pick_nu(sumq, nulow, nuhigh);
  db_launch_scale_vis(w.wbuf, d.R, r0, r1, lambda / ndata, 0, d.stream);
  db_count_launch(1);
  if (out3) {
    out3[0] = lambda;
    out3[1] = sumq;
    out3[2] = nu;
  }
  return nu;
}

void db_rlm_chunk(dirac_b200_problem *pr, int k, int ck, double *pblk_dev, double2 *r, int itmax,
                  int linsolv, int os, int randomize, double nulow, double nuhigh,
                  double *robust_nu, double *info, bool hidden_ready) {
  static const double defopts[4] = {1e-3, 1e-17, 1e-17, 1e-17};
  const int wt_itmax = 3;
  DevProblem &d = pr->d;
  db_lm_init(pr);
  robust_init(pr);
  LMWork &w = pr->lm;
  const int n8 = w.n8;
  int t0, t1;
  chunk_range(d, k, ck, &t0, &t1);
  const long long r0 = (long long)t0 * d.Nbase, r1 = (long long)t1 * d.Nbase;
  const double beta = pr->world > 1 ? pr->beta : 1.0;
  if (!hidden_ready) {
    if (beta != 1.0)
      DB_CHECK(cudaMemcpyAsync(w.pold, pblk_dev, sizeof(double) * w.n8, cudaMemcpyDeviceToDevice,
                               d.stream));
    db_cluster_pass(pr, k, pblk_dev, r, w.dbuf, 2, 1, nullptr, 1, t0, t1, nullptr, beta);
  }
  if (r1 > r0) db_launch_scale_vis(w.wbuf, d.R, r0, r1, 1.0, 1, d.stream);
  db_count_launch(1);
  double nu_t = *robust_nu;
  int nu = 2;
  LmOut o;
  memset(&o, 0, sizeof(o));
  for (int nw = 0; nw < wt_itmax; nw++) {
    bool evaluated = false;
    lm_core(pr, k, ck, t0, t1, pblk_dev, w.wbuf, itmax, defopts, linsolv, os, nw, randomize, false,
            0.0, &nu, &evaluated, nullptr, &o);
    if (nw < wt_itmax - 1 && r1 > r0) {
      const double *pe = (nw == 0 && evaluated) ? w.plast : pblk_dev;
      nu_t = irls_update(pr, k, t0, t1, pe, nu_t, nulow, nuhigh, nullptr);
    }
  }
  *robust_nu = nu_t;
  if (!hidden_ready)
    db_cluster_pass(pr, k, pblk_dev, w.dbuf, r, 3, 1, nullptr, 1, t0, t1, nullptr, beta, false,
                    beta != 1.0 ? w.pold : nullptr);
  (void)n8;
  fill_info(info, o);
}

extern "C" double dirac_b200_normal_eq(dirac_b200_problem *pr, int clus, int chunk,
                                       const double *pblk, const double *xd, double *JTJ,
                                       double *JTe) {
  DevProblem &d = pr->d;
  db_lm_init(pr);
  LMWork &w = pr->lm;
  const int n = w.n8;
  int t0, t1;
  chunk_range(d, clus, chunk, &t0, &t1);
  db_upload_vis(pr, xd, w.dbuf);
  DB_CHECK(cudaMemcpyAsync(w.pnew, pblk, sizeof(double) * n, cudaMemcpyHostToDevice, d.stream));
  db_cluster_pass(pr, clus, w.pnew, w.dbuf, nullptr, 1, 0, w.JTe, 1, t0, t1, nullptr);
  gram(pr, clus, t0, t1, 1, w.Tsub);
  assemble(pr, w.Tsub, w.pnew, w.JTJ0);
  double c = db_read_scalar(pr, 1);
  if (JTe) DB_CHECK(cudaMemcpy(JTe, w.JTe, sizeof(double) * n, cudaMemcpyDeviceToHost));
  if (JTJ)
    DB_CHECK(cudaMemcpy(JTJ, w.JTJ0, sizeof(double) * (size_t)n * n, cudaMemcpyDeviceToHost));
  DB_CHECK(cudaGetLastError());
  return c;
}

extern "C" double dirac_b200_normal_eq_weighted(dirac_b200_problem *pr, int clus, int chunk,
                                                const double *pblk, const double *xd,
                                                const double *wt, double *JTJ, double *JTe) {
  DevProblem &d = pr->d;
  db_lm_init(pr);
// ... 8 lines not shown
  db_cluster_pass(pr, clus, w.pnew, w.dbuf, nullptr, 1, 0, w.JTe, 1, t0, t1, w.wbuf);
  weighted_jtj(pr, clus, t0, t1, w.pnew, w.wbuf, w.JTJ0);
  double c = db_read_scalar(pr, 1);
  if (JTe) DB_CHECK(cudaMemcpy(JTe, w.JTe, sizeof(double) * n, cudaMemcpyDeviceToHost));
  if (JTJ)
    DB_CHECK(cudaMemcpy(JTJ, w.JTJ0, sizeof(double) * (size_t)n * n, cudaMemcpyDeviceToHost));
  DB_CHECK(cudaGetLastError());
  return c;
}

extern "C" void dirac_b200_assemble_damped(dirac_b200_problem *pr, int clus, int chunk,
                                           const double *pblk, int nmu, const double *mus,
                                           int factor, double *out, int *info) {
  DevProblem &d = pr->d;
  db_lm_init(pr);
  LMWork &w = pr->lm;
  const int n = w.n8;
  int t0, t1;
  chunk_range(d, clus, chunk, &t0, &t1);
  DB_CHECK(cudaMemcpyAsync(w.pnew, pblk, sizeof(double) * n, cudaMemcpyHostToDevice, d.stream));
  gram(pr, clus, t0, t1, 1, w.Tsub);
  assemble(pr, w.Tsub, w.pnew, nullptr);
  for (int i = 0; i < nmu; i++) {
    AssembleArgs a = assemble_args(d, w.Tsub, w.pnew, w.Hst);
    a.JTJ = w.JTJ;
    a.mu = mus[i];
    a.lower = 1;
    assemble_tiles(pr, a, 1);
    if (factor)
      CS_CHECK(cusolverDnDpotrf(w.cs, CUBLAS_FILL_MODE_LOWER, n, w.JTJ, n, w.cswork, w.lwork,
                                w.devinfo));
    DB_CHECK(cudaMemcpyAsync(out + (size_t)i * n * n, w.JTJ, sizeof(double) * (size_t)n * n,
                             cudaMemcpyDeviceToHost, d.stream));
    if (factor)
      DB_CHECK(cudaMemcpyAsync(info + i, w.devinfo, sizeof(int), cudaMemcpyDeviceToHost, d.stream));
    db_stream_sync(d.stream);
  }
  DB_CHECK(cudaGetLastError());
}

extern "C" void dirac_b200_assemble_batch(dirac_b200_problem *pr, const double *pp, const int *list,
                                          int nb, double tau, int lower, double *mu_out, double *out) {
  DevProblem &d = pr->d;
  db_lm_init(pr);
  DB_CHECK(cudaMemcpy(d.pp, pp, sizeof(double) * d.npar, cudaMemcpyHostToDevice));
  LMWork &w = pr->lm;
  const size_t nn = (size_t)w.n8 * w.n8;
  std::vector<int> tix(d.M), poff(d.M);
  for (int k = 0; k < d.M; k++) {
    tix[k] = d.h_clus[k].chunk0;
    poff[k] = d.h_chunk_poff[tix[k]];
  }
  for (int y = 0; y < nb; y++) {
    const int k = list[y];
    int t0, t1;
    chunk_range(d, k, 0, &t0, &t1);
    gram(pr, k, t0, t1, 1, w.T + (size_t)tix[k] * d.Nbase * 16);
    w.T_valid[tix[k]] = 1;
  }
  int *ibuf = dalloc<int>(nb + 2 * d.M);
  double *H = dalloc<double>((size_t)4 * d.N * nb), *mu = dalloc<double>(nb);
  double *A = dalloc<double>(nn * nb);
  DB_CHECK(cudaMemcpy(ibuf, list, sizeof(int) * nb, cudaMemcpyHostToDevice));
  DB_CHECK(cudaMemcpy(ibuf + nb, tix.data(), sizeof(int) * d.M, cudaMemcpyHostToDevice));
  DB_CHECK(cudaMemcpy(ibuf + nb + d.M, poff.data(), sizeof(int) * d.M, cudaMemcpyHostToDevice));
  AssembleArgs b = assemble_args(d, w.T, d.pp, H);
  b.list = ibuf; b.tix = ibuf + nb; b.poff = ibuf + nb + d.M;
  b.JTJ = A;
  b.stride = (long long)nn;
  station_sums(pr, b, nb);
  db_launch_batch_mu0(H, mu, d.N, tau, nb, d.stream);
  if (lower) {
    b.mu_dev = mu;
    b.lower = 1;
  }
  assemble_tiles(pr, b, nb);
  DB_CHECK(cudaMemcpyAsync(mu_out, mu, sizeof(double) * nb, cudaMemcpyDeviceToHost, d.stream));
  DB_CHECK(cudaMemcpyAsync(out, A, sizeof(double) * nn * nb, cudaMemcpyDeviceToHost, d.stream));
  db_stream_sync(d.stream);
  db_free(ibuf); db_free(H); db_free(mu); db_free(A);
  DB_CHECK(cudaGetLastError());
}

extern "C" void dirac_b200_os_normal_eq(dirac_b200_problem *pr, int clus, int chunk, int l,
                                        const double *pblk, const double *xd, const double *wt,
                                        double *JTJ, double *JTe, long long *path) {
  DevProblem &d = pr->d;
  db_lm_init(pr);
  robust_init(pr);
  LMWork &w = pr->lm;
  const int n = w.n8;
  int t0, t1;
  chunk_range(d, clus, chunk, &t0, &t1);
  db_upload_vis(pr, xd, w.dbuf);
  if (wt) db_upload_vis(pr, wt, w.wbuf);
  DB_CHECK(cudaMemcpyAsync(w.pnew, pblk, sizeof(double) * n, cudaMemcpyHostToDevice, d.stream));
  const OsPath p = os_subset_system(pr, clus, t0, t1, l, w.pnew, wt ? w.wbuf : nullptr);
  DB_CHECK(cudaMemcpyAsync(JTe, w.JTe, sizeof(double) * n, cudaMemcpyDeviceToHost, d.stream));
  DB_CHECK(cudaMemcpyAsync(JTJ, w.JTJ0, sizeof(double) * (size_t)n * n, cudaMemcpyDeviceToHost,
                           d.stream));
  db_stream_sync(d.stream);
  DB_CHECK(cudaGetLastError());
  path[0] = p.misaligned ? 1 : 0;
  path[1] = p.s0;
  path[2] = p.s1;
  path[3] = p.nJ;
}

extern "C" void dirac_b200_irls_update(dirac_b200_problem *pr, int clus, int chunk,
                                       const double *pblk, const double *xd, double *wt_inout,
                                       double nu0, double nulow, double nuhigh, double *out3) {
  DevProblem &d = pr->d;
  db_lm_init(pr);
  robust_init(pr);
  LMWork &w = pr->lm;
  int t0, t1;
  chunk_range(d, clus, chunk, &t0, &t1);
  db_upload_vis(pr, xd, w.dbuf);
  db_upload_vis(pr, wt_inout, w.wbuf);
  DB_CHECK(cudaMemcpyAsync(w.pnew, pblk, sizeof(double) * w.n8, cudaMemcpyHostToDevice, d.stream));
  irls_update(pr, clus, t0, t1, w.pnew, nu0, nulow, nuhigh, out3);
  db_download_vis(pr, w.wbuf, wt_inout);
  DB_CHECK(cudaGetLastError());
}

extern "C" void dirac_b200_lm_chunk(dirac_b200_problem *pr, int clus, int chunk, double *pblk_inout,
                                    const double *xd, int itmax, const double *opts, int linsolv,
                                    int os, int robust, double nulow, double nuhigh,
                                    double *nu_inout, double *info) {
  DevProblem &d = pr->d;
  db_lm_init(pr);
  LMWork &w = pr->lm;
  const int n = w.n8;
  db_upload_vis(pr, xd, w.dbuf);
  double *pblk_dev = w.pold;
  DB_CHECK(cudaMemcpyAsync(pblk_dev, pblk_inout, sizeof(double) * n, cudaMemcpyHostToDevice,
                           d.stream));
  if (robust)
    db_rlm_chunk(pr, clus, chunk, pblk_dev, pr->res, itmax, linsolv, os, 0, nulow, nuhigh, nu_inout,
                 info, true);
  else
    db_lm_chunk(pr, clus, chunk, pblk_dev, pr->res, itmax, opts, linsolv, os, 0, info, true);
  DB_CHECK(cudaMemcpyAsync(pblk_inout, pblk_dev, sizeof(double) * n, cudaMemcpyDeviceToHost,
                           d.stream));
  db_stream_sync(d.stream);
  DB_CHECK(cudaGetLastError());
}

extern "C" int dirac_b200_cluster_pass_eval(dirac_b200_problem *pr, int clus, int chunk, int mode,
                                            int write_out, int with_jte, int form_hidden, double beta,
                                            const double *pblk, const double *pblk_old,
                                            const double *in, const double *wt,
                                            const double *out_init, int inplace, double *out,
                                            double *jte, double *cost) {
  DevProblem &d = pr->d;
  if (clus < 0 || clus >= d.M || chunk < 0 || chunk >= d.h_clus[clus].nchunk) return -1;
  if (mode < 0 || mode > 4 || (mode == 4 && !with_jte) || ((mode == 2 || mode == 3) && with_jte))
    return -1;
  if (form_hidden &&
      ((mode != 1 && mode != 3) || wt || !db_cluster_pass_forms_hidden(d.N, d.Nbase)))
    return -1;
  if (!pblk_old && (form_hidden || (mode == 3 && beta != 1.0))) return -1;
  db_lm_init(pr);
  LMWork &w = pr->lm;
  const int n = w.n8;
  int t0, t1;
  chunk_range(d, clus, chunk, &t0, &t1);
  double2 *vin = dalloc<double2>((size_t)4 * d.R);
  double2 *vout = inplace ? vin : dalloc<double2>((size_t)4 * d.R);
  double2 *vwt = wt ? dalloc<double2>((size_t)4 * d.R) : nullptr;
  double *pb = dalloc<double>((size_t)2 * n);
  db_upload_vis(pr, in, vin);
  if (!inplace) db_upload_vis(pr, out_init, vout);
  if (wt) db_upload_vis(pr, wt, vwt);
  DB_CHECK(cudaMemcpyAsync(pb, pblk, sizeof(double) * n, cudaMemcpyHostToDevice, d.stream));
  if (pblk_old)
    DB_CHECK(cudaMemcpyAsync(pb + n, pblk_old, sizeof(double) * n, cudaMemcpyHostToDevice, d.stream));
  const int slot = mode == 0 ? 2 : 1;
  const int kernel = db_cluster_pass(pr, clus, pb, vin, vout, mode, write_out,
                                     with_jte ? w.JTe : nullptr, slot, t0, t1, vwt, beta, false,
                                     pblk_old ? pb + n : nullptr, form_hidden != 0);
  db_download_vis(pr, vout, out);
  if (with_jte)
    DB_CHECK(cudaMemcpy(jte, w.JTe, sizeof(double) * n, cudaMemcpyDeviceToHost));
  else
    memset(jte, 0, sizeof(double) * n);
  *cost = (mode <= 1 || mode == 4) ? db_read_scalar(pr, slot) : 0.0;
  db_free(vin);
  if (!inplace) db_free(vout);
  db_free(vwt);
  db_free(pb);
  DB_CHECK(cudaGetLastError());
  return kernel;
}

extern "C" int dirac_b200_cluster_hidden_eval(dirac_b200_problem *pr, int clus, int sign, double beta,
                                              const double *pp, const double *r, const double *dh,
                                              double *out) {
  DevProblem &d = pr->d;
  if (clus < 0 || clus >= d.M || sign == 0) return -1;
  db_lm_init(pr);
  LMWork &w = pr->lm;
  double2 *vr = dalloc<double2>((size_t)4 * d.R);
  DB_CHECK(cudaMemcpyAsync(d.pp, pp, sizeof(double) * d.npar, cudaMemcpyHostToDevice, d.stream));
  db_upload_vis(pr, r, vr);
  db_upload_vis(pr, dh, w.dbuf);
  db_cluster_hidden(pr, clus, vr, sign, beta);
  db_download_vis(pr, sign > 0 ? w.dbuf : vr, out);
  db_free(vr);
  DB_CHECK(cudaGetLastError());
  return 0;
}

extern "C" double dirac_b200_bench_predict(dirac_b200_problem *pr, int out_mode, int reps) {
  DevProblem &d = pr->d;
  cudaEvent_t e0, e1;
  DB_CHECK(cudaEventCreate(&e0));
  DB_CHECK(cudaEventCreate(&e1));
  for (int i = 0; i < 2; i++) db_predict_dev(pr, d.pp, pr->res, out_mode, 1, 0.0, 0);
  DB_CHECK(cudaEventRecord(e0, d.stream));
  for (int i = 0; i < reps; i++) db_predict_dev(pr, d.pp, pr->res, out_mode, 1, 0.0, 0);
  DB_CHECK(cudaEventRecord(e1, d.stream));
  db_event_sync(e1);
  float ms = 0.f;
  DB_CHECK(cudaEventElapsedTime(&ms, e0, e1));
  cudaEventDestroy(e0);
  cudaEventDestroy(e1);
  return 1e3 * ms / reps;
}

extern "C" double dirac_b200_bench_grad(dirac_b200_problem *pr, int reps) {
  DevProblem &d = pr->d;
  cudaEvent_t e0, e1;
  DB_CHECK(cudaEventCreate(&e0));
  DB_CHECK(cudaEventCreate(&e1));
  db_predict_dev(pr, d.pp, pr->res, 1, 0, 0.0, 0);
  for (int i = 0; i < 2; i++) db_grad_dev(pr, d.pp, pr->g, 0, 0.0);
  DB_CHECK(cudaEventRecord(e0, d.stream));
  for (int i = 0; i < reps; i++) db_grad_dev(pr, d.pp, pr->g, 0, 0.0);
  DB_CHECK(cudaEventRecord(e1, d.stream));
  db_event_sync(e1);
  float ms = 0.f;
  DB_CHECK(cudaEventElapsedTime(&ms, e0, e1));
  cudaEventDestroy(e0);
  cudaEventDestroy(e1);
  return 1e3 * ms / reps;
}

extern "C" double dirac_b200_bench_cluster_pass(dirac_b200_problem *pr, int clus, int mode,
                                                int with_grad, int write_out, int reps) {
  DevProblem &d = pr->d;
  db_lm_init(pr);
  LMWork &w = pr->lm;
  double *pblk = d.pp + d.h_chunk_poff[d.h_clus[clus].chunk0];
  cudaEvent_t e0, e1;
  DB_CHECK(cudaEventCreate(&e0));
  DB_CHECK(cudaEventCreate(&e1));
  for (int i = 0; i < 3; i++)
    db_cluster_pass(pr, clus, pblk, pr->res, w.dbuf, mode, write_out, with_grad ? w.JTe : nullptr,
                    1, 0, d.tilesz, nullptr);
  DB_CHECK(cudaEventRecord(e0, d.stream));
  for (int i = 0; i < reps; i++)
    db_cluster_pass(pr, (clus + i) % d.M, pblk, pr->res, w.dbuf, mode, write_out,
                    with_grad ? w.JTe : nullptr, 1, 0, d.tilesz, nullptr);
  DB_CHECK(cudaEventRecord(e1, d.stream));
  db_event_sync(e1);
  float ms = 0.f;
  DB_CHECK(cudaEventElapsedTime(&ms, e0, e1));
  cudaEventDestroy(e0);
  cudaEventDestroy(e1);
  return 1e3 * ms / reps;
}
```

sagecal_b200/csrc/problem.cu:

```cuda
#include <string.h>
#include <thread>
#include <vector>

#include "../../include/dirac_b200.h"
#include "internal.cuh"
#include "problem.h"

static unsigned long long g_launches = 0;
static unsigned long long g_sky_uploads = 0, g_coh_host_bytes = 0;
void db_count_sky_upload() { g_sky_uploads++; }
void db_count_coh_host_bytes(size_t bytes) { g_coh_host_bytes += bytes; }
extern "C" void dirac_b200_transfer_stats(unsigned long long *sky_uploads,
                                          unsigned long long *coh_host_bytes, int reset) {
  if (sky_uploads) *sky_uploads = g_sky_uploads;
  if (coh_host_bytes) *coh_host_bytes = g_coh_host_bytes;
  if (reset) g_sky_uploads = g_coh_host_bytes = 0;
}
void db_count_launch(int n) { g_launches += (unsigned long long)n; }
extern "C" unsigned long long dirac_b200_launch_count(void) { return g_launches; }

struct ProfRec { cudaEvent_t a, b; int kind; double bytes; };
static std::vector<ProfRec> g_prof;
static std::vector<cudaEvent_t> g_evpool;
static int g_prof_on = 0;
static cudaEvent_t prof_event() {
  if (!g_evpool.empty()) { cudaEvent_t e = g_evpool.back(); g_evpool.pop_back(); return e; }
  cudaEvent_t e;
  DB_CHECK(cudaEventCreate(&e));
  return e;
}
#define DB_PROF_KINDS 18
static unsigned long long g_kind_count[DB_PROF_KINDS] = {0};
extern "C" unsigned long long dirac_b200_kernel_count(int kind) {
  return (kind >= 0 && kind < DB_PROF_KINDS) ? g_kind_count[kind] : 0ull;
}
void db_prof_begin(int kind, double bytes, cudaStream_t st) {
  if (kind >= 0 && kind < DB_PROF_KINDS) g_kind_count[kind]++;
  if (!g_prof_on) return;
  ProfRec r; r.a = prof_event(); r.b = prof_event(); r.kind = kind; r.bytes = bytes;
  DB_CHECK(cudaEventRecord(r.a, st));
  g_prof.push_back(r);
}
void db_prof_end(cudaStream_t st) {
  if (!g_prof_on) return;
  DB_CHECK(cudaEventRecord(g_prof.back().b, st));
}
extern "C" void dirac_b200_profile_enable(int on) {
  for (auto &r : g_prof) { g_evpool.push_back(r.a); g_evpool.push_back(r.b); }
  g_prof.clear();
  g_prof_on = on;
}
extern "C" int dirac_b200_profile_read(int kind, double *ms, double *bytes) {
  DB_CHECK(cudaDeviceSynchronize());
  int cnt = 0; double t = 0.0, by = 0.0;
  for (auto &r : g_prof) if (r.kind == kind) {
    float f = 0.f; DB_CHECK(cudaEventElapsedTime(&f, r.a, r.b)); t += f; by += r.bytes; cnt++;
  }
  if (ms) *ms = t;
  if (bytes) *bytes = by;
  return cnt;
}

static cudaStream_t g_user_stream = nullptr;
static int g_have_user_stream = 0;
extern "C" void dirac_b200_set_stream(void *stream) {
  g_user_stream = (cudaStream_t)stream;
  g_have_user_stream = (stream != nullptr);
}
cudaStream_t db_new_stream(int *owned) {
  if (g_have_user_stream) { *owned = 0; return g_user_stream; }
  cudaStream_t st;
  DB_CHECK(cudaStreamCreateWithFlags(&st, cudaStreamNonBlocking));
  *owned = 1;
  return st;
}

static int g_opt[DB_OPT_COUNT] = {0, 0, 0, 0, 0, 0, 0, 0};
int db_opt(int id) { return (id >= 0 && id < DB_OPT_COUNT) ? g_opt[id] : 0; }
extern "C" int dirac_b200_set_option(const char *name, int value) {
  if (!strcmp(name, "cp_rows")) { g_opt[DB_OPT_CP_ROWS] = value; return 0; }
  if (!strcmp(name, "line_direct")) { g_opt[DB_OPT_LINE_DIRECT] = value; return 0; }
  if (!strcmp(name, "os_consistent")) { g_opt[DB_OPT_OS_CONSISTENT] = value; return 0; }
  if (!strcmp(name, "rtr_nu_unjoined")) { g_opt[DB_OPT_RTR_NU_UNJOINED] = value; return 0; }
  if (!strcmp(name, "admm_lm")) { g_opt[DB_OPT_ADMM_LM] = value; return 0; }
  if (!strcmp(name, "sweep_residual")) { g_opt[DB_OPT_SWEEP_RESIDUAL] = value; return 0; }
  return -1;
}
int db_sm_count() {
  static int n[64];
  int dev = 0;
  if (cudaGetDevice(&dev) != cudaSuccess || dev < 0 || dev >= 64) return 132;
  if (!n[dev]) {
    int v = 0;
    if (cudaDeviceGetAttribute(&v, cudaDevAttrMultiProcessorCount, dev) != cudaSuccess || v <= 0) v = 132;
    n[dev] = v;
  }
  return n[dev];
}

void require_gpu() {
  int n = 0;
  cudaError_t e = cudaGetDeviceCount(&n);
  if (e != cudaSuccess || n == 0) {
    fprintf(stderr,
            "dirac_b200: no CUDA device available (%s). This library has no CPU fallback.\n",
            cudaGetErrorString(e));
    exit(1);
  }
}

#include <map>
#include <unordered_map>
static std::multimap<size_t, void *> g_free_blocks;
static std::unordered_map<void *, size_t> g_live_blocks;
static size_t g_cached_bytes = 0;
static size_t cache_cap() {
  static size_t cap = (size_t)-1;
  if (cap == (size_t)-1) {
    const char *e = getenv("DIRAC_B200_CACHE_GB");
    if (e) {
      cap = (size_t)(atof(e) * 1073741824.0);
    } else {
      size_t fr = 0, tot = 0;
      cap = (cudaMemGetInfo(&fr, &tot) == cudaSuccess) ? tot / 4 * 3 : ((size_t)6 << 30);
    }
  }
  return cap;
}
static void cache_release_all() {
  for (auto &kv : g_free_blocks) cudaFree(kv.second);
  g_free_blocks.clear();
  g_cached_bytes = 0;
}
extern "C" void dirac_b200_release_cache(void) { cache_release_all(); }
void *db_malloc(size_t bytes) {
  bytes = (bytes + 255) & ~(size_t)255;
  auto it = g_free_blocks.find(bytes);
  void *p = nullptr;
  if (it != g_free_blocks.end()) {
    p = it->second;
    g_free_blocks.erase(it);
    g_cached_bytes -= bytes;
  } else {
    cudaError_t e = cudaMalloc(&p, bytes);
    if (e != cudaSuccess) {
      cudaGetLastError();
      cache_release_all();
      DB_CHECK(cudaMalloc(&p, bytes));
    }
  }
  g_live_blocks[p] = bytes;
  return p;
}
void db_free(void *p) {
  if (!p) return;
  auto it = g_live_blocks.find(p);
  if (it == g_live_blocks.end()) {
    cudaFree(p);
    return;
  }
  const size_t bytes = it->second;
  g_live_blocks.erase(it);
  if (g_cached_bytes + bytes > cache_cap()) {
    cudaFree(p);
  } else {
    g_free_blocks.insert({bytes, p});
    g_cached_bytes += bytes;
  }
}

static cudaStream_t new_call_stream() {
  require_gpu();
  cudaStream_t st;
  DB_CHECK(cudaStreamCreateWithFlags(&st, cudaStreamNonBlocking));
  return st;
}
DeviceScope::DeviceScope() : st(new_call_stream()), own_(true) {}
DeviceScope::DeviceScope(cudaStream_t borrowed) : st(borrowed), own_(false) {}
DeviceScope::~DeviceScope() {
  cudaStreamSynchronize(st);
  for (void *p : bufs_) cudaFree(p);
  if (own_) cudaStreamDestroy(st);
}
void DeviceScope::sync() {
  db_stream_sync(st);
  DB_CHECK(cudaGetLastError());
}

template <typename T>
static T *dev_alloc(size_t n) {
  return (T *)db_malloc(n * sizeof(T) + 16);
}

void db_build_tiles(int N, std::vector<TileDesc> &tiles) {
  int npb = (N - 1 + TILE_P - 1) / TILE_P;
  int nqb = (N + TILE_Q - 1) / TILE_Q;
  for (int pb = 0; pb < npb; pb++)
    for (int qb = 0; qb < nqb; qb++) {
      int pmin = pb * TILE_P;
      int qmax = qb * TILE_Q + TILE_Q - 1;
      if (qmax > N - 1) qmax = N - 1;
      if (qmax > pmin) {
        TileDesc t;
        t.pb = (short)pb;
        t.qb = (short)qb;
        tiles.push_back(t);
      }
    }
}

static dirac_b200_problem *create_impl(int N, int Nbase, int tilesz, const baseline_t *barr,
                                       const clus_source_t *carr, int M, int Mt, const double *coh,
                                       const double *x, long long npar);

extern "C" dirac_b200_problem *dirac_b200_create(int N, int Nbase, int tilesz,
                                                 const baseline_t *barr, const clus_source_t *carr,
                                                 int M, int Mt, const double *coh,
                                                 const double *x) {
  return create_impl(N, Nbase, tilesz, barr, carr, M, Mt, coh, x, (long long)8 * N * Mt);
}

extern "C" dirac_b200_problem *dirac_b200_create_shard(int N, int Nbase, int tilesz,
                                                       const baseline_t *barr,
                                                       const clus_source_t *carr_local,
                                                       int M_local, int Mt_local,
                                                       long long npar_global, const double *coh,
                                                       const double *x) {
  return create_impl(N, Nbase, tilesz, barr, carr_local, M_local, Mt_local, coh, x, npar_global);
}

extern "C" void dirac_b200_set_comm(dirac_b200_problem *pr, int rank, int world,
                                    void (*allreduce)(void *, long long, void *, void *),
                                    void *user, int m_global, int k_global0, double beta) {
  pr->rank = rank;
  pr->world = world;
  pr->allreduce = allreduce;
  pr->comm_user = user;
  pr->m_global = m_global;
  pr->k_global0 = k_global0;
  pr->beta = (beta > 0.0) ? beta : 1.0 / (double)(world > 0 ? world : 1);
}


void db_canonical_flags(int N, int Nbase, int tilesz, const baseline_t *barr, unsigned char *hflag) {
  const long long R = (long long)Nbase * tilesz;
  const long long Nb = (long long)N * (N - 1) / 2;
  int nthr = (R > (1 << 20)) ? 8 : 1;
  if (nthr > tilesz) nthr = tilesz;
  std::vector<long long> bad(nthr, -1);
  auto work = [&](int th) {
    for (int t = th; t < tilesz; t += nthr) {
      long long r = (long long)t * Nb;
      for (int p = 0; p < N - 1; p++)
        for (int q = p + 1; q < N; q++, r++) {
          if (barr[r].sta1 != p || barr[r].sta2 != q) {
            if (bad[th] < 0) bad[th] = r;
            return;
          }
          hflag[r] = barr[r].flag;
        }
    }
  };
  if (nthr == 1) {
    work(0);
  } else {
    std::vector<std::thread> pool;
    for (int th = 0; th < nthr; th++) pool.emplace_back(work, th);
    for (auto &th : pool) th.join();
  }
  for (int th = 0; th < nthr; th++)
    if (bad[th] >= 0) {
      const long long r = bad[th];
      fprintf(stderr, "dirac_b200: barr[%lld]=(%d,%d) is not in the canonical order of "
                      "generate_baselines; unsupported row order\n", r, barr[r].sta1, barr[r].sta2);
      exit(1);
    }
}

static dirac_b200_problem *create_impl(int N, int Nbase, int tilesz, const baseline_t *barr,
                                       const clus_source_t *carr, int M, int Mt, const double *coh,
                                       const double *x, long long npar) {
  require_gpu();
  if (Nbase != N * (N - 1) / 2) {
    fprintf(stderr, "dirac_b200: Nbase=%d is not N(N-1)/2 for N=%d; only the canonical baseline "
                    "set of generate_baselines is supported\n", Nbase, N);
    exit(1);
  }
  if (N > 32767) {
    fprintf(stderr, "dirac_b200: N=%d stations exceed the supported 32767\n", N);
    exit(1);
  }
  dirac_b200_problem *pr = new dirac_b200_problem();
  memset(&pr->d, 0, sizeof(DevProblem));
  DevProblem &d = pr->d;
  d.N = N; d.Nbase = Nbase; d.tilesz = tilesz; d.M = M; d.Mt = Mt;
  d.R = (long long)Nbase * tilesz;
  d.npar = npar;
  pr->rank = 0; pr->world = 1; pr->allreduce = nullptr; pr->comm_user = nullptr;
  pr->m_global = M; pr->k_global0 = 0; pr->beta = 1.0;
  DB_CHECK(cudaGetDevice(&d.device));
  d.stream = db_new_stream(&pr->own_stream);
  const long long R = d.R;

  d.x = dev_alloc<double2>((size_t)4 * R);
  pr->vis_stage = dev_alloc<double2>((size_t)4 * R);
  if (x) db_upload_vis(pr, x, d.x);

  std::vector<unsigned char> hflag(R);
  db_canonical_flags(N, Nbase, tilesz, barr, hflag.data());
  d.flag = dev_alloc<unsigned char>(R);
  DB_CHECK(cudaMemcpyAsync(d.flag, hflag.data(), R, cudaMemcpyHostToDevice, d.stream));
  db_stream_sync(d.stream);

  d.h_clus = (ClusterDesc *)malloc(sizeof(ClusterDesc) * M);
  int mt = 0;
  for (int k = 0; k < M; k++) {
    d.h_clus[k].nchunk = carr[k].nchunk;
    d.h_clus[k].chunk0 = mt;
    mt += carr[k].nchunk;
  }
  if (mt != Mt) {
    fprintf(stderr, "dirac_b200: sum of nchunk (%d) != Mt (%d)\n", mt, Mt);
    exit(1);
  }
  d.h_chunk_poff = (int *)malloc(sizeof(int) * Mt);
  for (int k = 0; k < M; k++)
    for (int c = 0; c < carr[k].nchunk; c++) d.h_chunk_poff[d.h_clus[k].chunk0 + c] = carr[k].p[c];
  d.clus = dev_alloc<ClusterDesc>(M);
  d.chunk_poff = dev_alloc<int>(Mt);
  DB_CHECK(cudaMemcpy(d.clus, d.h_clus, sizeof(ClusterDesc) * M, cudaMemcpyHostToDevice));
  DB_CHECK(cudaMemcpy(d.chunk_poff, d.h_chunk_poff, sizeof(int) * Mt, cudaMemcpyHostToDevice));

  std::vector<TileDesc> tiles;
  db_build_tiles(N, tiles);
  d.ntile = (int)tiles.size();
  d.tiles = dev_alloc<TileDesc>(tiles.size());
  DB_CHECK(cudaMemcpy(d.tiles, tiles.data(), sizeof(TileDesc) * tiles.size(),
                      cudaMemcpyHostToDevice));

  {
    std::vector<short2> pq(Nbase);
    int b = 0;
    for (int p = 0; p < N - 1; p++)
      for (int q = p + 1; q < N; q++, b++) pq[b] = make_short2((short)p, (short)q);
    d.blpq = dev_alloc<short2>(Nbase);
    DB_CHECK(cudaMemcpy(d.blpq, pq.data(), sizeof(short2) * Nbase, cudaMemcpyHostToDevice));
  }

  d.pp = dev_alloc<double>((size_t)d.npar);
  d.coh = dev_alloc<double2>((size_t)M * 4 * R);
  if (coh) {
    long long rows_per = (128ll << 20) / ((long long)M * 64);
    if (rows_per < 1) rows_per = 1;
    if (rows_per > R) rows_per = R;
    double2 *stage = dev_alloc<double2>((size_t)rows_per * M * 4);
    for (long long r0 = 0; r0 < R; r0 += rows_per) {
      int nr = (int)((R - r0 < rows_per) ? (R - r0) : rows_per);
      DB_CHECK(cudaMemcpyAsync(stage, coh + (size_t)r0 * M * 8, (size_t)nr * M * 64,
                               cudaMemcpyHostToDevice, d.stream));
      db_launch_coh_to_planar(stage, d.coh, r0, nr, M, R, d.stream);
      db_count_launch(1);
    }
    db_count_coh_host_bytes((size_t)R * M * 64);
    db_stream_sync(d.stream);
    db_free(stage);
  }

  const int nb2 = db_cluster_pass_nblocks(d.ntile, tilesz, 1);
  const int nb3 = db_stream_all_nblocks(Nbase, tilesz);
  pr->npartials = (nb2 > nb3 ? nb2 : nb3) + 1024;
  pr->partials = dev_alloc<double>(pr->npartials);
  d.scal = dev_alloc<double>(64 + 3 * 8 * (size_t)N + 8);
  DB_CHECK(cudaMemset(d.scal, 0, sizeof(double) * (64 + 3 * 8 * (size_t)N + 8)));
  DB_CHECK(cudaMallocHost((void **)&d.h_scal, (64 + 3 * 8 * (size_t)N + 8) * sizeof(double)));
  d.counters = dev_alloc<unsigned int>(16 + 1024);
  DB_CHECK(cudaMemset(d.counters, 0, (16 + 1024) * sizeof(unsigned int)));
  pr->res = dev_alloc<double2>((size_t)4 * R);
  pr->g = dev_alloc<double>((size_t)d.npar);
  DB_CHECK(cudaGetLastError());
  return pr;
}

extern "C" void dirac_b200_destroy(dirac_b200_problem *pr) {
  if (!pr) return;
  DevProblem &d = pr->d;
  cudaStreamSynchronize(d.stream);
  db_lm_free(pr);
  db_rtr_free(pr);
  db_free(d.coh); db_free(d.x); db_free(d.flag); db_free(d.pp); db_free(d.clus);
  db_free(d.chunk_poff); db_free(d.tiles); db_free(d.blpq); db_free(d.scal); db_free(d.counters);
  db_free(pr->partials); db_free(pr->res); db_free(pr->g); db_free(pr->vis_stage);
  if (pr->pm) db_free(pr->pm);
  if (pr->xb) { db_free(pr->xb); db_free(pr->pp_start); }
  if (pr->E0) db_free(pr->E0);
  cudaFreeHost(d.h_scal);
  free(d.h_clus); free(d.h_chunk_poff);
  if (pr->own_stream) cudaStreamDestroy(d.stream);
  delete pr;
}

void db_upload_vis(dirac_b200_problem *pr, const double *h, double2 *dst) {
  DevProblem &d = pr->d;
  DB_CHECK(cudaMemcpyAsync(pr->vis_stage, h, (size_t)d.R * 64, cudaMemcpyHostToDevice, d.stream));
  db_launch_vis_to_planar(pr->vis_stage, dst, d.R, d.stream);
  db_count_launch(1);
}
void db_download_vis(dirac_b200_problem *pr, const double2 *src, double *h) {
  DevProblem &d = pr->d;
  db_launch_vis_from_planar(src, pr->vis_stage, d.R, d.stream);
  db_count_launch(1);
  DB_CHECK(cudaMemcpyAsync(h, pr->vis_stage, (size_t)d.R * 64, cudaMemcpyDeviceToHost, d.stream));
  db_stream_sync(d.stream);
}

extern "C" void dirac_b200_set_data(dirac_b200_problem *pr, const double *x) {
  db_upload_vis(pr, x, pr->d.x);
  db_stream_sync(pr->d.stream);
}

void db_download_coh(const double2 *coh, double *x, int M, long long R, cudaStream_t st) {
  long long rows_per = (128ll << 20) / ((long long)M * 64);
  if (rows_per < 1) rows_per = 1;
  if (rows_per > R) rows_per = R;
  double2 *stage = dev_alloc<double2>((size_t)rows_per * M * 4);
  for (long long r0 = 0; r0 < R; r0 += rows_per) {
    int nr = (int)((R - r0 < rows_per) ? (R - r0) : rows_per);
    db_launch_coh_from_planar(coh, stage, r0, nr, M, R, st);
    db_count_launch(1);
    DB_CHECK(cudaMemcpyAsync(x + (size_t)r0 * M * 8, stage, (size_t)nr * M * 64,
                             cudaMemcpyDeviceToHost, st));
  }
  db_stream_sync(st);
  db_count_coh_host_bytes((size_t)R * M * 64);
  db_free(stage);
}

extern "C" void dirac_b200_get_coherencies(dirac_b200_problem *pr, double *coh) {
  db_download_coh(pr->d.coh, coh, pr->d.M, pr->d.R, pr->d.stream);
}

void db_predict_dev(dirac_b200_problem *pr, const double *pp_dev, double2 *out, int out_mode,
                    int cost_mode, double nu, int slot) {
  DevProblem &d = pr->d;
  StreamAllArgs a;
  memset(&a, 0, sizeof(a));
// ... 161 lines not shown
```

sagecal_b200/csrc/problem.h:

```cpp
#pragma once
#include <cusolverDn.h>
#include <cublas_v2.h>

#include <vector>

#include "../../include/dirac_b200.h"
#include "internal.cuh"

struct BigChol;
BigChol *db_bigchol_create(int n, int nbk, bool inv_panel, bool lookahead);
enum { BC_BLOCK = 256 };
static const bool BC_INV_PANEL = true, BC_LOOKAHEAD = true;
void db_bigchol_destroy(BigChol *bc);
void db_bigchol_bind_batch(BigChol *bc, double *A0, long long stride, int maxb);
void db_bigchol_factor_batch(BigChol *bc, int nb, int *info, int info_step, cudaStream_t st);

struct LMWork {
  bool ready;
  int n8;
  double *T;
  unsigned char *T_valid;
  double *Tsub;
  double *JTJ0, *JTJ;
  double *JTe, *JTe_new;
  double *Hst;
  double *Dp;
  double *pnew;
  double *h_vec;
  int *devinfo;
  double *cswork;
  int lwork;
  bool own_chol;
  double *bt_ws;
  BigChol *bc;
  double *jte_part;
  bool step_armed, step_fused;
  double *jtj_spec;
  cudaEvent_t ev_mail;
  double *tau;
  double *svdS, *svdU, *svdVT;
  cusolverDnHandle_t cs;
  cublasHandle_t cb;
  double2 *dbuf;
  double2 *wbuf;
  double2 *ebuf;
  double2 *os_eps, *os_w;
  double *HP, *HQ;
  double *plast;
  double *pold;
  double *JB, *LB;
  size_t lb_stride;
  int lb_ld, binfo_step;
  double *HB;
  double *mu_dev;
  double *h_mu;
  int *binfo_dev, *h_binfo;
  double **LBptr_dev;
  int *blist_dev, *btix_dev, *bpoff_dev;
  int *pref_slot;
  const double *jtj0_cur;
  const double *sys_T, *sys_p, *sys_H;
};

struct dirac_b200_problem {
  DevProblem d;
  double *partials;
  int npartials;
  double2 *res;
  double2 *vis_stage;
  double *g;
  LMWork lm;
  int own_stream;
  int rank, world;
  void (*allreduce)(void *dev, long long count, void *stream, void *user);
  void *comm_user;
  int m_global;
  int k_global0;
  double beta;
  const double *aug_y_host, *aug_bz_host, *aug_rho;
  double *aug_dev;
  double2 *pm;
  double *xb;
  double *pp_start;
  double2 *E0, *E1, *E2;
  double *poly_part;
  struct RtrWork *rtr;
};

void db_stream_sync(cudaStream_t st);
void db_event_sync(cudaEvent_t ev);
void db_flag_wait(const volatile unsigned long long *flag, unsigned long long epoch,
                  cudaStream_t st);
void *db_malloc(size_t bytes);
void db_free(void *p);
void require_gpu();

class DeviceScope {
 public:
  DeviceScope();
  explicit DeviceScope(cudaStream_t borrowed);
  ~DeviceScope();
  DeviceScope(const DeviceScope &) = delete;
  DeviceScope &operator=(const DeviceScope &) = delete;
  template <class T> T *alloc(size_t n) {
    void *p = nullptr;
    DB_CHECK(cudaMalloc(&p, sizeof(T) * n));
    bufs_.push_back(p);
    return (T *)p;
  }
  template <class T> T *upload(const T *h, size_t n) {
    T *d = alloc<T>(n ? n : 1);
    if (n) DB_CHECK(cudaMemcpyAsync(d, h, sizeof(T) * n, cudaMemcpyHostToDevice, st));
    return d;
  }
  template <class T> T *upload(const std::vector<T> &h) { return upload(h.data(), h.size()); }
  void sync();
  const cudaStream_t st;

 private:
  const bool own_;
  std::vector<void *> bufs_;
};

void db_download_coh(const double2 *coh, double *x, int M, long long R, cudaStream_t st);
void db_count_launch(int n);
void db_prof_begin(int kind, double bytes, cudaStream_t st);
void db_prof_end(cudaStream_t st);
cudaStream_t db_new_stream(int *owned);
void db_upload_vis(dirac_b200_problem *pr, const double *h, double2 *dst);
void db_download_vis(dirac_b200_problem *pr, const double2 *src, double *h);
void db_predict_dev(dirac_b200_problem *pr, const double *pp_dev, double2 *out, int out_mode,
                    int cost_mode, double nu, int slot);
double db_read_scalar(dirac_b200_problem *pr, int slot);
void db_grad_dev(dirac_b200_problem *pr, const double *pp_dev, double *g_dev, int robust,
                 double nu);
double db_cost_window_dev(dirac_b200_problem *pr, const double *pp_dev, double2 *out, double nu,
                          long long r_lo, long long r_hi);
void db_grad_window_dev(dirac_b200_problem *pr, const double *pp_dev, double *g_dev, double nu,
                        long long r_lo, long long r_hi);
int db_bfgsfit_dev(dirac_b200_problem *pr, double *pp, int max_lbfgs, int lbfgs_m, int solver_mode,
                   double mean_nu, double *res_0, double *res_1, bool keep_residual);
void db_count_sky_upload();
void db_count_coh_host_bytes(size_t bytes);
void db_lm_init(dirac_b200_problem *pr);
void db_prefactor_sweep(dirac_b200_problem *pr, double tau);
void db_allreduce(dirac_b200_problem *pr, void *dev, long long count);
void db_allreduce_world(dirac_b200_problem *pr, void *dev, long long count);
int db_nccl_world();
void db_allreduce_stream(dirac_b200_allreduce_fn fn, void *user, void *dev, long long count,
                         cudaStream_t st);
int db_manifold_projectback(double *Y, int n, int Mt, int Nf, int Niter, const int *cr,
                            cudaStream_t st);void db_lm_set_aug(const double *y_dev, const double *bz_dev, const double *y_host,
                   const double *bz_host, double rho);
int db_overlap_available(const dirac_b200_problem *pr);
cudaStream_t db_comm_stream();
void db_allreduce_segments(dirac_b200_problem *pr, double **ptr, const long long *count, int nseg,
                           cudaStream_t st);
extern "C" {
void db_launch_residual_cost(const double2 *x, const double2 *pm, double2 *out, long long n4,
                             int out_mode, int cost_mode, double inv_nu, double *partials,
                             double *cost, unsigned int *counter, cudaStream_t st);
void db_launch_sumsq(const double2 *v, long long n4, double *partials, double *out,
                     unsigned int *counter, cudaStream_t st);
void db_launch_axpby(const double2 *x, double2 *y, long long n4, double a, double b,
                     cudaStream_t st);
void db_launch_cluster_rowmap(const double2 *coh_k, const double2 *in, const double2 *in2,
                              double2 *out, const unsigned char *flag, const double *pp,
                              const int *chunk_poff, int nchunk, const short2 *blpq, long long R,
                              int Nbase, int sign, double beta, cudaStream_t st);
}

struct BandView {
  const double2 *coh, *x;
  const unsigned char *flag;
  int nc;
};
struct BandDev {
  int N, Nbase, tilesz, M, Mt, maxnc, ntile;
  long long R, npar;
  ClusterDesc *clus;
  int *chunk_poff;
  TileDesc *tiles;
  short2 *blpq;
  double *pp, *g, *partials, *scal, *h_scal;
  unsigned int *counters;
  double2 *res;
  cudaStream_t st;
};
// ... 14 lines not shown
```

sagecal_b200/csrc/rtr.cu:

```cuda
#include <math.h>
#include <string.h>
#include <algorithm>
#include <vector>

#include "../../include/dirac_b200.h"
#include "problem.h"
#include "rtr.h"
#include "rtr_algo.h"

int db_cluster_pass(dirac_b200_problem *pr, int k, const double *pblk_dev, const double2 *in,
                    double2 *out, int mode, int write_out, double *jte_dev, int cost_slot, int t0,
                    int t1, const double2 *wt, double beta, bool jte_zeroed,
                    const double *pblk_old, bool form_hidden = false);
void db_chunk_range(const DevProblem &d, int k, int ck, int *t0, int *t1);

struct RtrWork {
  int N, Nbase, nslice;
  double2 *TDpart, *TD;
  double *scpart, *sc;
  double *xdev, *edev;
  double *outdev;
  double *h;
  double *mbox, *mbox_dev;
  unsigned int *arrive;
  unsigned long long epoch;
};

static RtrWork *rtr_init(dirac_b200_problem *pr) {
  if (pr->rtr) return pr->rtr;
  DevProblem &d = pr->d;
  RtrWork *w = new RtrWork();
  w->N = d.N;
  w->Nbase = d.Nbase;
  const int nbb = (d.Nbase + 127) / 128;
  int ns = (db_sm_count() + nbb - 1) / nbb;
  if (ns > d.tilesz) ns = d.tilesz;
  if (ns < 1) ns = 1;
  w->nslice = ns;
  const size_t nb = (size_t)d.Nbase;
  w->TD = (double2 *)db_malloc(sizeof(double2) * 32 * nb);
  w->sc = (double *)db_malloc(sizeof(double) * 3 * nb);
  w->TDpart = ns > 1 ? (double2 *)db_malloc(sizeof(double2) * 32 * nb * ns) : nullptr;
  w->scpart = ns > 1 ? (double *)db_malloc(sizeof(double) * 3 * nb * ns) : nullptr;
  const size_t n8 = (size_t)8 * d.N;
  w->xdev = (double *)db_malloc(sizeof(double) * n8);
  w->edev = (double *)db_malloc(sizeof(double) * n8);
  w->outdev = (double *)db_malloc(sizeof(double) * (n8 + 2 * d.N + 8));
  DB_CHECK(cudaMallocHost((void **)&w->h, sizeof(double) * (3 * n8 + 2 * d.N + 16)));
  DB_CHECK(cudaHostAlloc((void **)&w->mbox, sizeof(double) * (n8 + 2 * d.N + 16),
                         cudaHostAllocMapped));
  DB_CHECK(cudaHostGetDevicePointer((void **)&w->mbox_dev, w->mbox, 0));
  memset(w->mbox, 0, sizeof(double) * (n8 + 2 * d.N + 16));
  w->arrive = (unsigned int *)db_malloc(256);
  DB_CHECK(cudaMemsetAsync(w->arrive, 0, 256, d.stream));
  w->epoch = 0;
  pr->rtr = w;
  return w;
}

void db_rtr_free(dirac_b200_problem *pr) {
  RtrWork *w = pr->rtr;
  if (!w) return;
  db_free(w->TD); db_free(w->sc);
  if (w->TDpart) { db_free(w->TDpart); db_free(w->scpart); }
  db_free(w->xdev); db_free(w->edev); db_free(w->outdev);
  cudaFreeHost(w->h);
  cudaFreeHost(w->mbox);
  db_free(w->arrive);
  delete w;
  pr->rtr = nullptr;
}

struct RtrDevEval {
  dirac_b200_problem *pr;
  RtrWork *w;
  int k, t0, t1, N, n8;
  long long nrows;
  std::vector<double> x_on_dev;
  bool force_dev = false;
  int last_ns = 0, last_tslice = 0;
  bool last_inline = false;

  double condense(const double *xw_host, double nu, bool tensors) {
    DevProblem &d = pr->d;
    RtrStatsArgs a;
    a.coh_k = d.coh + (size_t)k * 4 * d.R;
    a.d = pr->lm.dbuf;
    a.flag = d.flag;
    a.blpq = d.blpq;
    a.xw = nullptr;
    if (xw_host) {
      upload_x(xw_host);
      a.xw = w->xdev;
    }
    a.nu = nu;
    a.R = d.R; a.N = d.N; a.Nbase = d.Nbase;
    a.t_begin = t0; a.t_end = t1;
    const int nt = t1 - t0;
    int ns = w->nslice < nt ? w->nslice : nt;
    a.tslice = (nt + ns - 1) / ns;
    ns = (nt + a.tslice - 1) / a.tslice;
    last_ns = ns;
    last_tslice = a.tslice;
    a.TD = ns > 1 ? w->TDpart : w->TD;
    a.sc = ns > 1 ? w->scpart : w->sc;
    a.tensors = tensors ? 1 : 0;
    db_prof_begin(9, (double)nt * d.Nbase * 129.0, d.stream);
    db_launch_rtr_stats(&a, ns, d.stream);
    db_prof_end(d.stream);
    db_count_launch(1);
    if (ns > 1) {
      if (tensors)
        db_launch_rtr_reduce((const double *)w->TDpart, (double *)w->TD, (size_t)64 * d.Nbase, ns,
                             d.stream);
      db_launch_rtr_reduce(w->scpart, w->sc, (size_t)3 * d.Nbase, ns, d.stream);
      db_count_launch(tensors ? 2 : 1);
    }
    if (!xw_host) return 0.0;
    db_launch_rtr_plane_sum(w->sc, d.Nbase, 1, w->outdev, d.stream);
    db_count_launch(1);
    DB_CHECK(cudaMemcpyAsync(w->h + 2 * n8, w->outdev, sizeof(double), cudaMemcpyDeviceToHost,
                             d.stream));
    db_stream_sync(d.stream);
    return w->h[2 * n8];
  }

  void upload_x(const double *x) {
    if (x_on_dev.size() == (size_t)n8 && !memcmp(x_on_dev.data(), x, sizeof(double) * n8)) return;
    memcpy(w->h, x, sizeof(double) * n8);
    DB_CHECK(cudaMemcpyAsync(w->xdev, w->h, sizeof(double) * n8, cudaMemcpyHostToDevice,
                             pr->d.stream));
    x_on_dev.assign(x, x + n8);
  }

  void launch(const double *x, const double *eta, double *fcost, double *vec, double *cnt) {
    DevProblem &d = pr->d;
    const bool inl = N <= RTR_INLINE_MAXN && !force_dev;
    last_inline = inl;
    RtrEvalInl P;
    RtrEvalArgs &a = P.a;
    a.TD = w->TD; a.sc = w->sc; a.x = w->xdev; a.eta = eta ? w->edev : nullptr;
    a.out = vec ? w->outdev : nullptr;
    a.cost = fcost ? w->outdev + n8 : nullptr;
    a.count = cnt ? w->outdev + n8 + N : nullptr;
    a.N = N; a.Nbase = d.Nbase;
    a.arrive = w->arrive;
    a.hmail = w->mbox_dev;
    a.flag = reinterpret_cast<unsigned long long *>(w->mbox_dev + n8 + 2 * N + 2);
    a.epoch = ++w->epoch;
    if (inl) {
      memcpy(P.xin, x, sizeof(double) * n8);
      if (eta) memcpy(P.ein, eta, sizeof(double) * n8);
    } else {
      double *he = w->h + n8;
      upload_x(x);
      if (eta) {
        memcpy(he, eta, sizeof(double) * n8);
        DB_CHECK(cudaMemcpyAsync(w->edev, he, sizeof(double) * n8, cudaMemcpyHostToDevice,
                                 d.stream));
      }
    }
    db_prof_begin(10, 2.0 * d.Nbase * (512.0 + 24.0), d.stream);
    if (inl) db_launch_rtr_eval_inl(&P, d.stream);
    else db_launch_rtr_eval(&a, d.stream);
    db_prof_end(d.stream);
    db_count_launch(1);
// ... 111 lines not shown
```

sagecal_b200/csrc/sage.cu:

```cuda
#include <math.h>
#include <string.h>
#include <thread>
#include <vector>

#include "../../include/dirac_b200.h"
#include "problem.h"

void db_lm_chunk(dirac_b200_problem *pr, int k, int ck, double *pblk_dev, double2 *r, int itmax,
                 const double *opts, int linsolv, int os, int randomize, double *info,
                 bool hidden_ready);
void db_rlm_chunk(dirac_b200_problem *pr, int k, int ck, double *pblk_dev, double2 *r, int itmax,
                  int linsolv, int os, int randomize, double nulow, double nuhigh,
                  double *robust_nu, double *info, bool hidden_ready);
bool db_cluster_needs_rowmap(const dirac_b200_problem *pr, int k);
void db_cluster_hidden(dirac_b200_problem *pr, int k, double2 *r, int sign, double beta);
int db_lbfgs_fit(dirac_b200_problem *pr, double *p, int m, int itmax, int M, int robust,
                 double nu, bool res_held);
void db_lbfgs_fit_minibatch(dirac_b200_problem *pr, double *p, int m, int itmax, int M, double nu);
void db_rtr_chunk(dirac_b200_problem *pr, int k, int ck, double *pblk_dev, double2 *r, int kind,
                  int itmax_a, int itmax_b, double nulow, double nuhigh, double *robust_nu,
                  double *info, bool hidden_ready, const double *aug_y, const double *aug_bz,
                  double aug_rho);
#define SM_RTR_ADMM_ 7

static bool is_robust_mode(int solver_mode) {
  return solver_mode == SM_OSLM_OSRLM_RLBFGS || solver_mode == SM_RLM_RLBFGS ||
         solver_mode == SM_RTR_OSRLM_RLBFGS || solver_mode == SM_NSD_RLBFGS ||
         solver_mode == SM_RTR_ADMM_;
}

extern "C" int dirac_b200_sagefit(dirac_b200_problem *pr, double *pp, double *x_out,
                                  int max_emiter, int max_iter, int max_lbfgs, int lbfgs_m,
                                  int linsolv, int solver_mode, double nulow, double nuhigh,
                                  int randomize, double *mean_nu, double *res_0, double *res_1) {
  if (solver_mode < 0 || solver_mode > 6 + (pr->aug_rho ? 1 : 0)) {
    fprintf(stderr, "%s: %d: undefined solver mode\n", __FILE__, __LINE__);
    exit(1);
  }
  DevProblem &d = pr->d;
  const int M = d.M;
  const int m = (int)pr->d.npar;
  const long long n = (long long)d.Nbase * d.tilesz * 8;
  const ClusterDesc *hc = d.h_clus;
  if (pr->lm.ready) memset(pr->lm.T_valid, 0, d.Mt);
  double opts[5] = {1e-3, 1e-15, 1e-15, 1e-20, -1e-6};
  double info[10] = {0, 0, 0, 0, 0, 0, 0, 0, 0, 0};
  double robust_nu0 = nulow;
  double rtr_nu = nulow;
  const bool sharded = pr->world > 1;
  const int MG = sharded ? pr->m_global : M;
  const int k0 = sharded ? pr->k_global0 : 0;
  std::vector<double> nerr(MG, 0.0), robust_nuM(MG, 0.0);
  const bool robust = is_robust_mode(solver_mode);
  const size_t xb_len = (size_t)8 * d.R + (size_t)m + (size_t)MG;
  if (sharded) {
    db_lm_init(pr);
    if (!pr->pm) pr->pm = (decltype(pr->pm))db_malloc(sizeof(double2) * 4 * d.R);
    if (!pr->xb) {
      pr->xb = (double *)db_malloc(sizeof(double) * (xb_len + 8));
      pr->pp_start = (double *)db_malloc(sizeof(double) * ((size_t)m + 8));
    }
  }
  auto allreduce_host = [&](double *v, int cnt) {
    DB_CHECK(cudaMemcpyAsync(pr->g, v, sizeof(double) * cnt, cudaMemcpyHostToDevice, d.stream));
    db_allreduce(pr, pr->g, cnt);
    DB_CHECK(cudaMemcpyAsync(v, pr->g, sizeof(double) * cnt, cudaMemcpyDeviceToHost, d.stream));
    db_stream_sync(d.stream);
  };

  DB_CHECK(cudaMemcpyAsync(d.pp, pp, sizeof(double) * m, cudaMemcpyHostToDevice, d.stream));
  db_predict_dev(pr, d.pp, pr->res, 1, 1, 0.0, 0);
  *res_0 = sqrt(db_read_scalar(pr, 0)) / (double)n;

  int weighted_iter = 0;
  const int total_iter = MG * max_iter;
  const int iter_bar = (int)ceil((0.80 / (double)MG) * ((double)total_iter));
  for (int ci = 0; ci < max_emiter; ci++) {
    if (sharded) {
      DB_CHECK(cudaMemcpyAsync(pr->pm, pr->res, sizeof(double2) * 4 * d.R, cudaMemcpyDeviceToDevice,
                               d.stream));
      DB_CHECK(cudaMemcpyAsync(pr->pp_start, d.pp, sizeof(double) * m, cudaMemcpyDeviceToDevice,
                               d.stream));
      for (int g = 0; g < MG; g++)
        if (g < k0 || g >= k0 + M) nerr[g] = 0.0;
    }
    {
      const bool last_em = (ci == max_emiter - 1);
      const bool plain = (solver_mode == SM_LM_LBFGS) || (solver_mode == SM_OSLM_LBFGS && last_em);
      if (plain && linsolv == 0 && max_iter > 0 && !weighted_iter && !pr->aug_rho)
        db_prefactor_sweep(pr, opts[0]);
    }
    for (int cl = 0; cl < M; cl++) {
      const int cj = cl;
      const int cg = k0 + cl;
      int this_itermax;
      if (weighted_iter) {
        this_itermax = (int)((0.20 * nerr[cg]) * ((double)total_iter)) + iter_bar;
      } else {
        this_itermax = max_iter;
      }
      if (this_itermax > 0) {
        double init_res = 0.0, final_res = 0.0;
        const bool hr = db_cluster_needs_rowmap(pr, cj);
        if (hr) db_cluster_hidden(pr, cj, pr->res, +1, pr->world > 1 ? pr->beta : 1.0);
        for (int ck = 0; ck < hc[cj].nchunk; ck++) {
          const int poff = d.h_chunk_poff[hc[cj].chunk0 + ck];
          double *pblk = d.pp + poff;
          const bool last = (ci == max_emiter - 1);
          if (solver_mode == SM_RTR_ADMM_) {
            if (!ci) rtr_nu = robust_nu0;
            db_rtr_chunk(pr, cj, ck, pblk, pr->res, 5, this_itermax + 5, this_itermax + 10, nulow,
                         nuhigh, &rtr_nu, info, hr, pr->aug_y_host + poff, pr->aug_bz_host + poff,
                         pr->aug_rho[cg]);
            if (last) robust_nuM[cg] += rtr_nu;
            init_res += info[0];
            final_res += info[1];
            continue;
          }
          if (pr->aug_rho)
            db_lm_set_aug(pr->aug_dev + poff, pr->aug_dev + d.npar + poff, pr->aug_y_host + poff,
                          pr->aug_bz_host + poff, pr->aug_rho[cg]);
          if (solver_mode == SM_OSLM_LBFGS) {
            db_lm_chunk(pr, cj, ck, pblk, pr->res, this_itermax, opts, linsolv, last ? 0 : 1,
                        randomize, info, hr);
          } else if (solver_mode == SM_LM_LBFGS) {
            db_lm_chunk(pr, cj, ck, pblk, pr->res, this_itermax, opts, linsolv, 0, randomize, info,
                        hr);
          } else if (solver_mode == SM_RLM_RLBFGS) {
            if (last) {
              double nu = robust_nu0;
              db_rlm_chunk(pr, cj, ck, pblk, pr->res, this_itermax, linsolv, 0, randomize, nulow,
                           nuhigh, &nu, info, hr);
              robust_nuM[cg] += nu;
            } else {
              db_lm_chunk(pr, cj, ck, pblk, pr->res, this_itermax, opts, linsolv, 1, randomize,
                          info, hr);
            }
          } else if (solver_mode == SM_RTR_OSLM_LBFGS) {
            db_rtr_chunk(pr, cj, ck, pblk, pr->res, 4, this_itermax + 5, this_itermax + 10, nulow,
                         nuhigh, &rtr_nu, info, hr, nullptr, nullptr, 0.0);
          } else if (solver_mode == SM_RTR_OSRLM_RLBFGS) {
            if (!ci) rtr_nu = robust_nu0;
            db_rtr_chunk(pr, cj, ck, pblk, pr->res, 5, this_itermax + 5, this_itermax + 10, nulow,
                         nuhigh, &rtr_nu, info, hr, nullptr, nullptr, 0.0);
            if (last) robust_nuM[cg] += rtr_nu;
          } else if (solver_mode == SM_NSD_RLBFGS) {
            if (!ci) rtr_nu = robust_nu0;
            db_rtr_chunk(pr, cj, ck, pblk, pr->res, 6, this_itermax + 15, 0, nulow, nuhigh, &rtr_nu,
                         info, hr, nullptr, nullptr, 0.0);
            if (last) robust_nuM[cg] += rtr_nu;
          } else {
            if (last) {
              double nu = robust_nu0;
              db_rlm_chunk(pr, cj, ck, pblk, pr->res, this_itermax, linsolv, 1, randomize, nulow,
                           nuhigh, &nu, info, hr);
              robust_nuM[cg] += nu;
            } else {
              db_lm_chunk(pr, cj, ck, pblk, pr->res, this_itermax, opts, linsolv, 1, randomize,
                          info, hr);
            }
          }
          init_res += info[0];
          final_res += info[1];
          if (pr->aug_rho) db_lm_set_aug(nullptr, nullptr, nullptr, nullptr, 0.0);
        }
        if (hr) db_cluster_hidden(pr, cj, pr->res, -1, pr->world > 1 ? pr->beta : 1.0);
        if (init_res > 0.0) {
          nerr[cg] = (init_res - final_res) / init_res;
          if (nerr[cg] < 0.0) nerr[cg] = 0.0;
        } else {
          nerr[cg] = 0.0;
        }
        if (robust && ci == max_emiter - 1) robust_nuM[cg] /= (double)hc[cj].nchunk;
      }
    }
    if (sharded) {
      double *xb = pr->xb;
      double2 *xr = reinterpret_cast<double2 *>(xb);
      double2 *xp = reinterpret_cast<double2 *>(xb + (size_t)8 * d.R);
      DB_CHECK(cudaMemcpyAsync(xr, pr->res, sizeof(double2) * 4 * d.R, cudaMemcpyDeviceToDevice,
                               d.stream));
      db_launch_axpby(pr->pm, xr, 4 * d.R, -1.0, 1.0, d.stream);
      DB_CHECK(cudaMemcpyAsync(xp, d.pp, sizeof(double) * m, cudaMemcpyDeviceToDevice, d.stream));
      db_launch_axpby(reinterpret_cast<double2 *>(pr->pp_start), xp, m / 2, -1.0, 1.0, d.stream);
      DB_CHECK(cudaMemcpyAsync(xb + (size_t)8 * d.R + m, nerr.data(), sizeof(double) * MG,
                               cudaMemcpyHostToDevice, d.stream));
      db_allreduce(pr, xb, (long long)xb_len);
      DB_CHECK(cudaMemcpyAsync(nerr.data(), xb + (size_t)8 * d.R + m, sizeof(double) * MG,
                               cudaMemcpyDeviceToHost, d.stream));
      DB_CHECK(cudaMemcpyAsync(pr->res, pr->pm, sizeof(double2) * 4 * d.R, cudaMemcpyDeviceToDevice,
                               d.stream));
      db_launch_axpby(xr, pr->res, 4 * d.R, 1.0, 1.0, d.stream);
      DB_CHECK(cudaMemcpyAsync(d.pp, pr->pp_start, sizeof(double) * m, cudaMemcpyDeviceToDevice,
                               d.stream));
      db_launch_axpby(xp, reinterpret_cast<double2 *>(d.pp), m / 2, 1.0, 1.0, d.stream);
      db_count_launch(4);
      db_stream_sync(d.stream);
    }
    double total_err = 0.0;
    for (int cj = 0; cj < MG; cj++) total_err += fabs(nerr[cj]);
    if (total_err > 0.0)
      for (int cj = 0; cj < MG; cj++) nerr[cj] *= 1.0 / total_err;
    if (randomize) weighted_iter = !weighted_iter;
  }
  if (robust) {
    if (sharded) allreduce_host(robust_nuM.data(), MG);
    double s = 0.0;
    for (int cj = 0; cj < MG; cj++) s += fabs(robust_nuM[cj]);
    robust_nu0 = s / (double)MG;
    if (robust_nu0 < nulow) robust_nu0 = nulow;
    else if (robust_nu0 > nuhigh) robust_nu0 = nuhigh;
  }
  DB_CHECK(cudaMemcpyAsync(pp, d.pp, sizeof(double) * m, cudaMemcpyDeviceToHost, d.stream));
  db_stream_sync(d.stream);

  const bool minibatch = max_lbfgs > 0 && robust && lbfgs_m < 0;
  const bool lbfgs_stage = max_lbfgs > 0 && (!robust || lbfgs_m != 0);
  int steps = 0;
  if (max_lbfgs > 0) {
    if (robust) {
      if (lbfgs_m > 0) {
        steps = db_lbfgs_fit(pr, pp, m, max_lbfgs, lbfgs_m, 1, robust_nu0, true);
      } else if (lbfgs_m < 0) {
        db_lbfgs_fit_minibatch(pr, pp, m, max_lbfgs, -lbfgs_m, robust_nu0);
      }
    } else {
      steps = db_lbfgs_fit(pr, pp, m, max_lbfgs, lbfgs_m, 0, 0.0, true);
    }
  }
  if (lbfgs_stage)
    DB_CHECK(cudaMemcpyAsync(d.pp, pp, sizeof(double) * m, cudaMemcpyHostToDevice, d.stream));
  if (steps > 0 || (db_opt(DB_OPT_SWEEP_RESIDUAL) && !minibatch)) {
    db_launch_sumsq(pr->res, 4 * d.R, pr->partials, d.scal, d.counters, d.stream);
    db_count_launch(1);
  } else {
    db_predict_dev(pr, d.pp, pr->res, 1, 1, 0.0, 0);
  }
  *res_1 = sqrt(db_read_scalar(pr, 0)) / (double)n;
  if (x_out) db_download_vis(pr, pr->res, x_out);
  *mean_nu = robust_nu0;
  DB_CHECK(cudaGetLastError());
  return (*res_1 > *res_0) ? -1 : 0;
}

extern "C" int sagefit_visibilities(double *u, double *v, double *w, double *x, int N, int Nbase,
                                    int tilesz, baseline_t *barr, clus_source_t *carr,
                                    double *coh, int M, int Mt, double freq0, double fdelta,
                                    double *pp, double uvmin, int Nt, int max_emiter, int max_iter,
                                    int max_lbfgs, int lbfgs_m, int gpu_threads, int linsolv,
                                    int solver_mode, double nulow, double nuhigh, int randomize,
                                    double *mean_nu, double *res_0, double *res_1) {
  (void)u; (void)v; (void)w; (void)freq0; (void)fdelta; (void)uvmin; (void)Nt; (void)gpu_threads;
  dirac_b200_problem *pr = dirac_b200_create(N, Nbase, tilesz, barr, carr, M, Mt, coh, x);
  int rv = dirac_b200_sagefit(pr, pp, x, max_emiter, max_iter, max_lbfgs, lbfgs_m, linsolv,
                              solver_mode, nulow, nuhigh, randomize, mean_nu, res_0, res_1);
  dirac_b200_destroy(pr);
  return rv;
}

#define SAGEFIT_ALIAS(name)                                                                      \
  extern "C" int name(double *u, double *v, double *w, double *x, int N, int Nbase, int tilesz,  \
                      baseline_t *barr, clus_source_t *carr, double *coh, int M, int Mt,         \
                      double freq0, double fdelta, double *pp, double uvmin, int Nt,             \
                      int max_emiter, int max_iter, int max_lbfgs, int lbfgs_m, int gpu_threads, \
                      int linsolv, int solver_mode, double nulow, double nuhigh, int randomize,  \
                      double *mean_nu, double *res_0, double *res_1) {                           \
    return sagefit_visibilities(u, v, w, x, N, Nbase, tilesz, barr, carr, coh, M, Mt, freq0,     \
                                fdelta, pp, uvmin, Nt, max_emiter, max_iter, max_lbfgs, lbfgs_m, \
                                gpu_threads, linsolv, solver_mode, nulow, nuhigh, randomize,     \
                                mean_nu, res_0, res_1);                                          \
  }
SAGEFIT_ALIAS(sagefit_visibilities_dual_pt_flt)
SAGEFIT_ALIAS(sagefit_visibilities_dual_pt)
SAGEFIT_ALIAS(sagefit_visibilities_dual_pt_one_gpu)

int db_bfgsfit_dev(dirac_b200_problem *pr, double *pp, int max_lbfgs, int lbfgs_m, int solver_mode,
                   double mean_nu, double *res_0, double *res_1, bool keep_residual) {
  DevProblem &d = pr->d;
  const int m = d.N * d.Mt * 8;
  const long long n = (long long)d.Nbase * d.tilesz * 8;
// ... 102 lines not shown
```

sagecal_b200/lib.py:

```python
from __future__ import annotations

import ctypes as C
import os

import numpy as np

from .dirac_api import DiracAPI, SkyModel, baseline_t, clus_source_t, c_double_p, dptr, cptr

_HERE = os.path.dirname(os.path.abspath(__file__))
LIB_PATH = os.path.join(_HERE, "libdirac_b200.so")

EXPORTED = [
    "sagefit_visibilities", "sagefit_visibilities_dual_pt_flt", "sagefit_visibilities_dual_pt",
    "sagefit_visibilities_dual_pt_one_gpu", "bfgsfit_visibilities", "bfgsfit_visibilities_gpu",
    "precalculate_coherencies", "predict_visibilities_multifreq", "generate_baselines",
    "preset_flags_and_data", "whiten_data", "dirac_b200_create", "dirac_b200_destroy", "dirac_b200_set_data",
    "dirac_b200_precalculate", "dirac_b200_get_coherencies", "dirac_b200_predict",
    "dirac_b200_grad", "dirac_b200_cost_window", "dirac_b200_grad_window", "dirac_b200_normal_eq",
    "dirac_b200_launch_count", "dirac_b200_sagefit",
    "dirac_b200_set_stream", "dirac_b200_profile_enable", "dirac_b200_profile_read",
    "dirac_b200_kernel_count", "dirac_b200_normal_eq_weighted", "dirac_b200_create_shard",
    "dirac_b200_set_comm", "dirac_b200_spd_solve", "dirac_b200_tri_solve", "dirac_b200_tri_solve_ld",
    "dirac_b200_set_option", "dirac_b200_nccl_unique_id", "dirac_b200_nccl_init",
    "dirac_b200_nccl_finalize", "dirac_b200_nccl_ready", "dirac_b200_comm_stats",
# ... 227 lines not shown
        return c, out

    def cost(self, pp, robust=False, nu=0.0):
        return self.api.lib.dirac_b200_predict(self.h, dptr(pp), None, 0, 2 if robust else 1, nu)

    def grad(self, pp, robust=False, nu=0.0):
        g = np.zeros(self.m)
        self.api.lib.dirac_b200_grad(self.h, dptr(pp), dptr(g), 1 if robust else 0, nu)
        return g

    def cost_window(self, pp, row0, nrows, nu):
        return self.api.lib.dirac_b200_cost_window(self.h, dptr(pp), row0, nrows, nu)

    def grad_window(self, pp, row0, nrows, nu):
        g = np.zeros(self.m)
        self.api.lib.dirac_b200_grad_window(self.h, dptr(pp), dptr(g), row0, nrows, nu)
        return g

    def sagefit(self, pp, x_out=None, max_emiter=3, max_iter=2, max_lbfgs=10, lbfgs_m=7, linsolv=0,
                solver_mode=1, nulow=2.0, nuhigh=30.0, randomize=0):
        nu, r0, r1 = C.c_double(0.0), C.c_double(0.0), C.c_double(0.0)
        rv = self.api.lib.dirac_b200_sagefit(self.h, dptr(pp),
                                             dptr(x_out) if x_out is not None else None,
                                             max_emiter, max_iter, max_lbfgs, lbfgs_m, linsolv,
                                             solver_mode, nulow, nuhigh, randomize, C.byref(nu),
                                             C.byref(r0), C.byref(r1))
        return rv, nu.value, r0.value, r1.value

    def line_model(self, xk, pk, alphas, nu, alpha_res):
        L = self.api.lib
        L.dirac_b200_line_model.restype = None
        L.dirac_b200_line_model.argtypes = [C.c_void_p, c_double_p, c_double_p, C.c_int, c_double_p,
                                            C.c_double, C.c_double, c_double_p, c_double_p, c_double_p,
                                            c_double_p, C.POINTER(C.c_int)]
        xk = np.ascontiguousarray(xk, dtype=np.float64)
        pk = np.ascontiguousarray(pk, dtype=np.float64)
        alphas = np.ascontiguousarray(alphas, dtype=np.float64)
        E = np.zeros(3 * self.n)
        poly = np.zeros(5)
        costs = np.zeros(2 * len(alphas))
        res = np.zeros(self.n)
        shape = (C.c_int * 3)()
        L.dirac_b200_line_model(self.h, dptr(xk), dptr(pk), len(alphas), dptr(alphas), nu, alpha_res,
                                dptr(E), dptr(poly), dptr(costs), dptr(res), shape)
        return dict(E0=E[:self.n], E1=E[self.n:2 * self.n], E2=E[2 * self.n:], poly=poly,
                    cost_gauss=costs[0::2], cost_robust=costs[1::2], res=res, shape=tuple(shape))

    RTR_COST, RTR_VEC, RTR_COUNTS, RTR_ETA, RTR_UNIT = 1, 2, 4, 8, 16

    def lbfgs_trace(self, pp, itmax, M, robust=False, nu=2.0):
        L = self.api.lib
        L.dirac_b200_lbfgs_trace.restype = C.c_int
        L.dirac_b200_lbfgs_trace.argtypes = [C.c_void_p, c_double_p, C.c_int, C.c_int, C.c_int,
                                             C.c_double, c_double_p, C.POINTER(C.c_longlong),
                                             C.POINTER(C.c_int), c_double_p, c_double_p]
        p = np.array(pp, dtype=np.float64)
        n = max(itmax, 1)
        alphak, gnorm = np.zeros(n), np.zeros(n)
        ncost = np.zeros(n, dtype=np.int64)
        slot = np.zeros(n, dtype=np.int32)
        it = np.zeros((n, self.m))
        k = L.dirac_b200_lbfgs_trace(self.h, dptr(p), itmax, M, int(robust), nu, dptr(alphak),
                                     ncost.ctypes.data_as(C.POINTER(C.c_longlong)),
                                     slot.ctypes.data_as(C.POINTER(C.c_int)), dptr(gnorm),
                                     dptr(it.reshape(-1)))
        if k < 0:
            return None
        return dict(p=p, niter=k, alphak=alphak[:k], ncost=ncost[:k], slot=slot[:k],
                    gnorm=gnorm[:k], iterates=it[:k])

    def rtr_eval(self, k, ck, evals, xw=None, nu=2.0, keep=True, force_device=False):
        L = self.api.lib
        L.dirac_b200_rtr_eval.restype = None
        L.dirac_b200_rtr_eval.argtypes = [C.c_void_p, C.c_int, C.c_int, c_double_p, C.c_double,
                                          C.c_int, C.c_int, C.c_int, C.POINTER(C.c_int), c_double_p,
                                          c_double_p, c_double_p, c_double_p, c_double_p, c_double_p]
        n8, ne = 8 * self.N, len(evals)
        ops = np.zeros(ne, dtype=np.int32)
        X = np.zeros((ne, n8))
        ETA = np.zeros((ne, n8))
        for i, e in enumerate(evals):
            X[i] = e["x"]
            if e.get("eta") is not None:
                ETA[i] = e["eta"]
                ops[i] |= self.RTR_ETA
            ops[i] |= ((self.RTR_COST if e.get("cost") else 0) | (self.RTR_VEC if e.get("vec") else 0)
                       | (self.RTR_COUNTS if e.get("counts") else 0)
                       | (self.RTR_UNIT if e.get("unit") else 0))
        cost = np.zeros(ne)
        vec = np.zeros((ne, n8))
        cnt = np.zeros((ne, self.N))
        info = np.zeros(4)
        xw_arr = None if xw is None else np.ascontiguousarray(xw, dtype=np.float64)
        L.dirac_b200_rtr_eval(self.h, k, ck, dptr(xw_arr) if xw_arr is not None else None, nu,
                              1 if keep else 0, 1 if force_device else 0, ne,
                              ops.ctypes.data_as(C.POINTER(C.c_int)), dptr(X), dptr(ETA), dptr(cost),
                              dptr(vec), dptr(cnt), dptr(info))
        res = [dict(cost=cost[i] if ops[i] & self.RTR_COST else None,
                    vec=vec[i] if ops[i] & self.RTR_VEC else None,
                    counts=cnt[i] if ops[i] & self.RTR_COUNTS else None) for i in range(ne)]
        return dict(results=res, slw=info[0], nslice=int(info[1]), tslice=int(info[2]),
                    inline=bool(info[3]))

    def os_normal_eq(self, clus, chunk, l, pblk, xd, wt=None):
        L = self.api.lib
        L.dirac_b200_os_normal_eq.restype = None
        L.dirac_b200_os_normal_eq.argtypes = [C.c_void_p, C.c_int, C.c_int, C.c_int, c_double_p,
                                              c_double_p, c_double_p, c_double_p, c_double_p,
                                              C.POINTER(C.c_longlong)]
        n8 = 8 * self.N
        JTJ = np.zeros((n8, n8))
        JTe = np.zeros(n8)
        path = (C.c_longlong * 4)()
        pblk = np.ascontiguousarray(pblk, dtype=np.float64)
        xd = np.ascontiguousarray(xd, dtype=np.float64)
        wt = None if wt is None else np.ascontiguousarray(wt, dtype=np.float64)
        L.dirac_b200_os_normal_eq(self.h, clus, chunk, l, dptr(pblk), dptr(xd),
                                  dptr(wt) if wt is not None else None, dptr(JTJ.reshape(-1)),
                                  dptr(JTe), path)
        return JTJ, JTe, dict(misaligned=bool(path[0]), s0=int(path[1]), s1=int(path[2]),
                              nJ=int(path[3]))

    def irls_update(self, clus, chunk, pblk, xd, wt, nu0, nulow=2.0, nuhigh=30.0):
        L = self.api.lib
        L.dirac_b200_irls_update.restype = None
        L.dirac_b200_irls_update.argtypes = [C.c_void_p, C.c_int, C.c_int, c_double_p, c_double_p,
                                             c_double_p, C.c_double, C.c_double, C.c_double,
                                             c_double_p]
        w = np.array(wt, dtype=np.float64)
        out3 = np.zeros(3)
        L.dirac_b200_irls_update(self.h, clus, chunk,
                                 dptr(np.ascontiguousarray(pblk, dtype=np.float64)),
                                 dptr(np.ascontiguousarray(xd, dtype=np.float64)), dptr(w), nu0,
                                 nulow, nuhigh, dptr(out3))
        return w, out3[0], out3[1], out3[2]

    def lm_chunk(self, clus, chunk, pblk, xd, itmax, opts=None, linsolv=0, os_=False, robust=False,
                 nulow=2.0, nuhigh=30.0, nu0=2.0):
        L = self.api.lib
        L.dirac_b200_lm_chunk.restype = None
        L.dirac_b200_lm_chunk.argtypes = [C.c_void_p, C.c_int, C.c_int, c_double_p, c_double_p,
                                          C.c_int, c_double_p, C.c_int, C.c_int, C.c_int, C.c_double,
                                          C.c_double, C.POINTER(C.c_double), c_double_p]
        p = np.array(pblk, dtype=np.float64)
        info = np.zeros(10)
        nu = C.c_double(nu0)
        o = None if opts is None else np.ascontiguousarray(opts, dtype=np.float64)
        L.dirac_b200_lm_chunk(self.h, clus, chunk, dptr(p),
                              dptr(np.ascontiguousarray(xd, dtype=np.float64)), itmax,
                              dptr(o) if o is not None else None, linsolv, int(os_), int(robust),
                              nulow, nuhigh, C.byref(nu), dptr(info))
        return p, info, nu.value

    CLUSTER_PASS_KERNELS = ("lin", "lin_grad", "split", "tile", "none")

    def cluster_pass(self, clus, chunk, mode, pblk, x, write_out=True, with_jte=False,
                     form_hidden=False, beta=1.0, pblk_old=None, wt=None, out_init=None,
                     inplace=False):
        L = self.api.lib
        L.dirac_b200_cluster_pass_eval.restype = C.c_int
        L.dirac_b200_cluster_pass_eval.argtypes = ([C.c_void_p] + [C.c_int] * 6 + [C.c_double]
                                                   + [c_double_p] * 5 + [C.c_int] + [c_double_p] * 3)
        f64 = lambda v: None if v is None else np.ascontiguousarray(v, dtype=np.float64)
        pblk, pblk_old, x, wt = f64(pblk), f64(pblk_old), f64(x), f64(wt)
        out_init = np.zeros(self.n) if out_init is None else f64(out_init)
        out = np.full(self.n, np.nan)
        jte = np.full(8 * self.N, np.nan)
        cost = np.full(1, np.nan)
        opt = lambda v: dptr(v) if v is not None else None
        k = L.dirac_b200_cluster_pass_eval(self.h, clus, chunk, mode, int(write_out), int(with_jte),
                                           int(form_hidden), beta, dptr(pblk), opt(pblk_old),
                                           dptr(x), opt(wt), dptr(out_init), int(inplace),
                                           dptr(out), dptr(jte), dptr(cost))
        return dict(kernel=None if k < 0 else self.CLUSTER_PASS_KERNELS[k], out=out, jte=jte,
                    cost=float(cost[0]))

    def cluster_hidden(self, clus, sign, beta, pp, r, dh):
        L = self.api.lib
        L.dirac_b200_cluster_hidden_eval.restype = C.c_int
        L.dirac_b200_cluster_hidden_eval.argtypes = ([C.c_void_p, C.c_int, C.c_int, C.c_double]
                                                     + [c_double_p] * 4)
        f64 = lambda v: np.ascontiguousarray(v, dtype=np.float64)
        out = np.full(self.n, np.nan)
        rv = L.dirac_b200_cluster_hidden_eval(self.h, clus, sign, beta, dptr(f64(pp)), dptr(f64(r)),
                                              dptr(f64(dh)), dptr(out))
        return None if rv != 0 else out

    def normal_eq(self, clus, chunk, pblk, xd):
        n8 = 8 * self.N
        JTJ = np.zeros((n8, n8))
        JTe = np.zeros(n8)
        pblk = np.ascontiguousarray(pblk, dtype=np.float64)
        c = self.api.lib.dirac_b200_normal_eq(self.h, clus, chunk, dptr(pblk), dptr(xd),
                                              dptr(JTJ.reshape(-1)), dptr(JTe))
        return c, JTJ, JTe

    def normal_eq_weighted(self, clus, chunk, pblk, xd, wt):
        n8 = 8 * self.N
        JTJ = np.zeros((n8, n8))
        JTe = np.zeros(n8)
        pblk = np.ascontiguousarray(pblk, dtype=np.float64)
        c = self.api.lib.dirac_b200_normal_eq_weighted(self.h, clus, chunk, dptr(pblk), dptr(xd),
                                                       dptr(wt), dptr(JTJ.reshape(-1)), dptr(JTe))
        return c, JTJ, JTe


_api = None


def load() -> DiracB200:
    global _api
    if _api is None:
        _api = DiracB200()
    return _api
```

Baseline: 7.427 billion.

## Fuse next cluster's opening gradient and cost into closing LM pass

On the last LM trial of a cluster visit, the linear-mapped cluster pass also streams the next cluster's coherencies and computes that cluster's J^T e and cost from the same residual. The next visit then copies these instead of running its own opening pass, saving one full sweep over the residual buffer. This is gated on the residual being larger than L2 and on plain single-chunk LM visits. The price is a heavier kernel: a shallower pipeline (3 stages instead of 5), 12 rows per stage, and extra state handoff between solver calls.

```diff
diff --git a/sagecal_b200/csrc/internal.cuh b/sagecal_b200/csrc/internal.cuh
--- a/sagecal_b200/csrc/internal.cuh
+++ b/sagecal_b200/csrc/internal.cuh
@@ -215,6 +215,10 @@
   double *jte_part;
   unsigned int *gcounter;
   const double2 *wt;
+  const double2 *coh_next;
+  const double *pblk_next;
+  double *jte_next, *cost_next, *partials_next;
+  unsigned int *counter_next;
 };
 
 struct WeightedJtjArgs {
@@ -281,9 +285,10 @@
 
 enum { DB_OPT_CP_ROWS = 0, DB_OPT_LINE_DIRECT = 1, DB_OPT_OS_CONSISTENT = 2,
        DB_OPT_RTR_NU_UNJOINED = 3, DB_OPT_ADMM_LM = 4, DB_OPT_SWEEP_RESIDUAL = 5,
-       DB_OPT_COUNT = 8 };
+       DB_OPT_HANDOFF = 6, DB_OPT_COUNT = 8 };
 int db_opt(int id);
 int db_sm_count();
+long long db_l2_bytes();
 static inline int db_cp_max_slices(int Nbase, int tilesz) {
   const int nbg = (Nbase + 255) / 256;
   int nsl = (db_sm_count() + nbg - 1) / nbg;
@@ -303,9 +308,11 @@
                                cudaStream_t st);
 void db_launch_grad_band_tma(const GradArgs *a, int ntile, int nchan, cudaStream_t st);
 int db_cluster_pass_nblocks(int ntile, int nt, int tslice);
-enum { DB_CP_LIN = 0, DB_CP_LIN_GRAD = 1, DB_CP_SPLIT = 2, DB_CP_TILE = 3, DB_CP_NONE = 4 };
+enum { DB_CP_LIN = 0, DB_CP_LIN_GRAD = 1, DB_CP_SPLIT = 2, DB_CP_TILE = 3, DB_CP_NONE = 4,
+       DB_CP_LIN_NEXT = 5 };
 int db_launch_cluster_pass(const ClusterPassArgs *a, int ntile, cudaStream_t st);
 int db_cluster_pass_forms_hidden(int N, int Nbase);
+int db_cluster_pass_opens_next(int N, int Nbase);
 void db_launch_coh_gram(const GramArgs *a, int ntile, int nk, cudaStream_t st);
 void db_launch_station_sums(const AssembleArgs *a, int nb, cudaStream_t st);
 void db_launch_assemble_tiles(const AssembleArgs *a, int nb, cudaStream_t st);
diff --git a/sagecal_b200/csrc/kernels_stream.cu b/sagecal_b200/csrc/kernels_stream.cu
--- a/sagecal_b200/csrc/kernels_stream.cu
+++ b/sagecal_b200/csrc/kernels_stream.cu
@@ -529,12 +529,14 @@
   grid_reduce_sum(cost, a.partials, a.cost, a.counter);
 }
 
-template <int NST, bool GRAD>
+template <int NST, bool GRAD, bool NEXT>
 __global__ void __launch_bounds__(512)
 k_cluster_pass_lin(ClusterPassArgs a) {
+  static_assert(!(GRAD && NEXT), "the pass that opens the next visit carries no J^T e of its own");
+  constexpr bool SUMS = GRAD || NEXT;
   extern __shared__ __align__(128) unsigned char smem_raw[];
   constexpr int BL = 256;
-  constexpr int STAGE_ELEMS = 8 * BL;
+  constexpr int STAGE_ELEMS = (NEXT ? 12 : 8) * BL;
   double2 *ring = reinterpret_cast<double2 *>(smem_raw);
   double *acc = reinterpret_cast<double *>(ring + (size_t)NST * STAGE_ELEMS);
   unsigned long long *bars = reinterpret_cast<unsigned long long *>(acc + ((8 * a.N + 1) & ~1));
@@ -545,7 +547,7 @@
   const int ts = a.t_begin + blockIdx.y * a.tslice;
   const int te = min(ts + a.tslice, a.t_end);
   const int nrow = te - ts;
-  if (GRAD)
+  if (SUMS)
     for (int i = tid; i < 8 * a.N; i += 512) acc[i] = 0.0;
   if (tid == 0) {
 #pragma unroll
@@ -557,11 +559,13 @@
     const unsigned row_bytes = (unsigned)nvalid * 16u;
     const long long row0 = (long long)(ts + j) * a.Nbase + b0;
     double2 *dst = ring + (size_t)s * STAGE_ELEMS;
-    mbar_expect_tx(&bars[s], 8u * row_bytes);
+    mbar_expect_tx(&bars[s], (NEXT ? 12u : 8u) * row_bytes);
 #pragma unroll
     for (int c = 0; c < 4; c++) {
       bulk_g2s(dst + c * BL, a.coh_k + (long long)c * a.R + row0, row_bytes, &bars[s]);
       bulk_g2s(dst + (4 + c) * BL, a.in + (long long)c * a.R + row0, row_bytes, &bars[s]);
+      if (NEXT)
+        bulk_g2s(dst + (8 + c) * BL, a.coh_next + (long long)c * a.R + row0, row_bytes, &bars[s]);
     }
   };
   if (tid == 0) {
@@ -599,12 +603,12 @@
     Jr[0] = __ldg(jp);
     Jr[1] = __ldg(jp + 1);
     load_jones(a.pblk, q, Jq);
-    if (old_model && !GRAD) load_old_jones();
+    if (old_model && !SUMS) load_old_jones();
     for (int j = 0; j < nrow; j++)
       flagbits |= (a.flag[(long long)(ts + j) * a.Nbase + b] != 0 ? 1u : 0u) << j;
   }
   const long long c0 = (long long)(2 * h) * a.R, c1 = c0 + a.R;
-  double cost = 0.0;
+  double cost = 0.0, cost_next = 0.0;
   for (int j = 0; j < nrow; j++) {
     const int s = j % NST;
     if (tid == 0 && j + NST - 1 < nrow) issue(j + NST - 1, (j + NST - 1) % NST);
@@ -626,7 +630,7 @@
       if (fl) m[0] = m[1] = make_double2(0.0, 0.0);
       double2 mo[2];
       if (old_model) {
-        if (GRAD) load_old_jones();
+        if (SUMS) load_old_jones();
         const double2 U0 = cdot2(Jro[0], C[0], Jro[1], C[2]);
         const double2 U1 = cdot2(Jro[0], C[1], Jro[1], C[3]);
         mo[0] = cdot2c(U0, Jqo[0], U1, Jqo[1]);
@@ -671,12 +675,46 @@
 #pragma unroll
           for (int lm = 0; lm < 4; lm++) cfmac(W[jj * 4 + lm], e[jj], C[lm]);
       }
+      if (NEXT) {
+        const double2 *jn = reinterpret_cast<const double2 *>(a.pblk_next + 8 * (long long)p + 4 * h);
+        const double2 Jrn0 = __ldg(jn), Jrn1 = __ldg(jn + 1);
+        double2 Jqn[4], Cn[4];
+        load_jones(a.pblk_next, q, Jqn);
+#pragma unroll
+        for (int c = 0; c < 4; c++) Cn[c] = lds_v2(st + (8 + c) * BL);
+        const double2 V0 = cdot2(Jrn0, Cn[0], Jrn1, Cn[2]);
+        const double2 V1 = cdot2(Jrn0, Cn[1], Jrn1, Cn[3]);
+        double2 mn[2];
+        mn[0] = cdot2c(V0, Jqn[0], V1, Jqn[1]);
+        mn[1] = cdot2c(V0, Jqn[2], V1, Jqn[3]);
+        if (fl) mn[0] = mn[1] = make_double2(0.0, 0.0);
+        double2 en[2];
+#pragma unroll
+        for (int jj = 0; jj < 2; jj++) {
+          const double2 d = cadd(make_double2(1.0 * e[jj].x, 1.0 * e[jj].y), mn[jj]);
+          en[jj] = csub(d, mn[jj]);
+          cost_next = fma(en[jj].x, en[jj].x, cost_next);
+          cost_next = fma(en[jj].y, en[jj].y, cost_next);
+        }
+        if (!fl) {
+#pragma unroll
+          for (int jj = 0; jj < 2; jj++)
+#pragma unroll
+            for (int lm = 0; lm < 4; lm++) cfmac(W[jj * 4 + lm], en[jj], Cn[lm]);
+        }
+      }
     }
     __syncthreads();
   }
-  if (!GRAD) {
+  if (!SUMS) {
     if (a.mode <= 1) grid_reduce_sum(cost, a.partials, a.cost, a.counter);
     return;
+  }
+  if (NEXT && valid) {
+    const double2 *jn = reinterpret_cast<const double2 *>(a.pblk_next + 8 * (long long)p + 4 * h);
+    Jr[0] = __ldg(jn);
+    Jr[1] = __ldg(jn + 1);
+    load_jones(a.pblk_next, q, Jq);
   }
   double2 Gp[2], Gq[4];
   Gp[0] = Gp[1] = make_double2(0.0, 0.0);
@@ -741,12 +779,20 @@
       for (int i = tid; i < n8; i += 512) {
         double sacc = 0.0;
         for (unsigned c = 0; c < gridDim.y; c++) sacc += __ldcg(grp + (size_t)c * n8 + i);
-        if (sacc != 0.0) atomicAdd(a.jte + i, sacc);
+        if (sacc != 0.0) atomicAdd((NEXT ? a.jte_next : a.jte) + i, sacc);
       }
       if (tid == 0) a.gcounter[blockIdx.x] = 0;
     }
   }
-  grid_reduce_sum(cost, a.partials, a.cost, a.counter);
+  if (!NEXT) {
+    grid_reduce_sum(cost, a.partials, a.cost, a.counter);
+    return;
+  }
+  if (a.mode <= 1) {
+    grid_reduce_sum(cost, a.partials, a.cost, a.counter);
+    __syncthreads();
+  }
+  grid_reduce_sum(cost_next, a.partials_next, a.cost_next, a.counter_next);
 }
 
 
@@ -840,14 +886,16 @@
   k_grad_tma_window<TB, NST><<<grid, 2 * TILE_THREADS, smem, st>>>(b);
 }
 
-static bool cluster_pass_lin_fits(int N, int Nbase) {
-  return (size_t)5 * 8 * 256 * sizeof(double2) + sizeof(double) * ((8 * N + 1) & ~1) + 40 <=
-             (size_t)200 * 1024 && (Nbase + 255) / 256 <= 1024;
-}
-
-template <bool GRAD>
+static bool cluster_pass_lin_fits(int N, int Nbase, int stages = 5, int runs = 8) {
+  return (size_t)stages * runs * 256 * sizeof(double2) + sizeof(double) * ((8 * N + 1) & ~1) +
+                 8 * stages <= (size_t)200 * 1024 && (Nbase + 255) / 256 <= 1024;
+}
+#define CP_NEXT_STAGES 3
+
+template <bool GRAD, bool NEXT>
 static void launch_cluster_pass_lin(const ClusterPassArgs *a, cudaStream_t st) {
-  constexpr int NST = 5;
+  constexpr int NST = NEXT ? CP_NEXT_STAGES : 5;
+  constexpr int RUNS = NEXT ? 12 : 8;
   const int nt = a->t_end - a->t_begin;
   const int nbg = (a->Nbase + 255) / 256;
   int nsl = (db_sm_count() + nbg - 1) / nbg;
@@ -855,20 +903,20 @@
   ClusterPassArgs b = *a;
   b.tslice = (nt + nsl - 1) / nsl;
   const int forced = db_opt(DB_OPT_CP_ROWS);
-  if (forced > 0 && (!GRAD || (nt + forced - 1) / forced <= db_cp_max_slices(a->Nbase, nt)))
+  if (forced > 0 && (!(GRAD || NEXT) || (nt + forced - 1) / forced <= db_cp_max_slices(a->Nbase, nt)))
     b.tslice = forced;
   if (b.tslice > nt) b.tslice = nt;
   if (b.tslice > 32) b.tslice = 32;
-  const size_t smem = (size_t)NST * 8 * 256 * sizeof(double2) +
+  const size_t smem = (size_t)NST * RUNS * 256 * sizeof(double2) +
                       sizeof(double) * ((8 * a->N + 1) & ~1) + NST * 8;
   static bool configured = false;
   if (!configured) {
-    DB_CHECK(cudaFuncSetAttribute(k_cluster_pass_lin<NST, GRAD>,
+    DB_CHECK(cudaFuncSetAttribute(k_cluster_pass_lin<NST, GRAD, NEXT>,
                                   cudaFuncAttributeMaxDynamicSharedMemorySize, 200 * 1024));
     configured = true;
   }
   dim3 grid(nbg, (nt + b.tslice - 1) / b.tslice);
-  k_cluster_pass_lin<NST, GRAD><<<grid, 512, smem, st>>>(b);
+  k_cluster_pass_lin<NST, GRAD, NEXT><<<grid, 512, smem, st>>>(b);
 }
 
 extern "C" {
@@ -894,6 +942,9 @@
 
 int db_cluster_pass_nblocks(int ntile, int nt, int tslice) { return ntile * ((nt + tslice - 1) / tslice); }
 int db_cluster_pass_forms_hidden(int N, int Nbase) { return cluster_pass_lin_fits(N, Nbase); }
+int db_cluster_pass_opens_next(int N, int Nbase) {
+  return cluster_pass_lin_fits(N, Nbase) && cluster_pass_lin_fits(N, Nbase, CP_NEXT_STAGES, 12);
+}
 int db_launch_cluster_pass(const ClusterPassArgs *a, int ntile, cudaStream_t st) {
   int nt = a->t_end - a->t_begin;
   dim3 grid(ntile, (nt + a->tslice - 1) / a->tslice);
@@ -902,10 +953,20 @@
                     "kernels run (%s:%d)\n", __FILE__, __LINE__);
     exit(1);
   }
+  if (a->coh_next) {
+    if (!a->form_hidden || a->jte || (a->mode != 1 && a->mode != 3) ||
+        !db_cluster_pass_opens_next(a->N, a->Nbase)) {
+      fprintf(stderr, "dirac_b200: closing pass that opens the next visit requested outside a plain "
+                      "form_hidden trial or SUB of the linear-mapped kernel (%s:%d)\n", __FILE__, __LINE__);
+      exit(1);
+    }
+    launch_cluster_pass_lin<false, true>(a, st);
+    return DB_CP_LIN_NEXT;
+  }
   const bool fits = cluster_pass_lin_fits(a->N, a->Nbase);
   if (a->jte == nullptr || (a->mode > 1 && a->mode != 4)) {
     if (!a->wt && fits) {
-      launch_cluster_pass_lin<false>(a, st);
+      launch_cluster_pass_lin<false, false>(a, st);
       return DB_CP_LIN;
     }
     k_cluster_pass<<<grid, TILE_THREADS, 0, st>>>(*a);
@@ -914,7 +975,7 @@
     k_cluster_pass_split<<<grid, 2 * TILE_THREADS, 0, st>>>(*a);
     return DB_CP_SPLIT;
   }
-  launch_cluster_pass_lin<true>(a, st);
+  launch_cluster_pass_lin<true, false>(a, st);
   return DB_CP_LIN_GRAD;
 }
 void db_launch_coh_gram(const GramArgs *a, int ntile, int nk, cudaStream_t st) {
diff --git a/sagecal_b200/csrc/lm.cu b/sagecal_b200/csrc/lm.cu
--- a/sagecal_b200/csrc/lm.cu
+++ b/sagecal_b200/csrc/lm.cu
@@ -79,7 +79,11 @@
     const int nbg = (d.Nbase + 255) / 256;
     const int nsl = db_cp_max_slices(d.Nbase, d.tilesz);
     w.jte_part = dalloc<double>((size_t)nbg * (nsl + 1) * n8);
-  }
+    w.cost_part = dalloc<double>((size_t)nbg * (nsl + 1));
+  }
+  w.JTe_next = dalloc<double>(n8 + 1);
+  w.cost_next = w.JTe_next + n8;
+  w.next_tag = -1;
   DB_CHECK(cudaEventCreateWithFlags(&w.ev_mail, cudaEventDisableTiming));
   DB_CHECK(cudaMallocHost((void **)&w.h_vec, sizeof(double) * (5 * n8 + 4 * d.N + 64)));
   static cusolverDnHandle_t g_cs = nullptr;
@@ -134,6 +138,7 @@
   if (!w.ready) return;
   db_free(w.T); db_free(w.Tsub); db_free(w.JTJ0); db_free(w.JTJ);
   db_free(w.Hst); db_free(w.pnew); db_free(w.plast); db_free(w.pold); db_free(w.jte_part);
+  db_free(w.cost_part); db_free(w.JTe_next);
   db_free(w.tau); db_free(w.cswork); db_free(w.dbuf);
   if (w.bt_ws) db_free(w.bt_ws);
   db_bigchol_destroy(w.bc);
@@ -167,13 +172,18 @@
 int db_cluster_pass(dirac_b200_problem *pr, int k, const double *pblk_dev, const double2 *in,
                     double2 *out, int mode, int write_out, double *jte_dev, int cost_slot, int t0,
                     int t1, const double2 *wt, double beta = 1.0, bool jte_zeroed = false,
-                    const double *pblk_old = nullptr, bool form_hidden = false);
+                    const double *pblk_old = nullptr, bool form_hidden = false, int k_next = -1,
+                    const double *pblk_next = nullptr);
 
 int db_cluster_pass(dirac_b200_problem *pr, int k, const double *pblk_dev, const double2 *in,
                     double2 *out, int mode, int write_out, double *jte_dev, int cost_slot, int t0,
                     int t1, const double2 *wt, double beta, bool jte_zeroed,
-                    const double *pblk_old, bool form_hidden) {
-  DevProblem &d = pr->d;
+                    const double *pblk_old, bool form_hidden, int k_next,
+                    const double *pblk_next) {
+  DevProblem &d = pr->d;
+  LMWork &w = pr->lm;
+  if (k_next >= 0)
+    DB_CHECK(cudaMemsetAsync(w.JTe_next, 0, sizeof(double) * (8 * d.N + 1), d.stream));
   if (t1 <= t0) {
     if (mode <= 1 || mode == 4)
       DB_CHECK(cudaMemsetAsync(d.scal + cost_slot, 0, sizeof(double), d.stream));
@@ -181,6 +191,9 @@
     return DB_CP_NONE;
   }
   ClusterPassArgs a;
+  a.coh_next = k_next >= 0 ? d.coh + (size_t)k_next * 4 * d.R : nullptr;
+  a.pblk_next = pblk_next; a.jte_next = w.JTe_next; a.cost_next = w.cost_next;
+  a.partials_next = w.cost_part; a.counter_next = d.counters + 1;
   a.coh_k = d.coh + (size_t)k * 4 * d.R;
   a.in = in; a.flag = d.flag; a.pblk = pblk_dev; a.tiles = d.tiles; a.out = out; a.jte = jte_dev;
   a.blpq = d.blpq; a.jte_part = pr->lm.jte_part; a.gcounter = d.counters + 16;
@@ -193,7 +206,7 @@
   if (jte_dev && (mode <= 1 || mode == 4) && !jte_zeroed)
     DB_CHECK(cudaMemsetAsync(jte_dev, 0, sizeof(double) * 8 * d.N, d.stream));
   db_prof_begin((jte_dev && (mode <= 1 || mode == 4)) ? 2 : 8, (double)(t1 - t0) * d.Nbase * (129.0 + (write_out ? 64.0 : 0.0) +
-                                                 (wt ? 64.0 : 0.0)), d.stream);
+                                                 (wt ? 64.0 : 0.0) + (k_next >= 0 ? 64.0 : 0.0)), d.stream);
   const int kernel = db_launch_cluster_pass(&a, d.ntile, d.stream);
   db_prof_end(d.stream);
   db_count_launch(1);
@@ -595,7 +608,8 @@
 static void lm_core(dirac_b200_problem *pr, int k, int ck, int t0, int t1, double *pblk_dev,
                     const double2 *wt, int itmax, const double *opts, int linsolv, int os,
                     int os_shift, int randomize, bool have_first, double first_cost, int *nu_damp,
-                    bool *evaluated_trial, const double2 *hidden_from, LmOut *out) {
+                    bool *evaluated_trial, const double2 *hidden_from, LmOut *out,
+                    int k_next = -1, const double *pblk_next = nullptr) {
   DevProblem &d = pr->d;
   LMWork &w = pr->lm;
   const int n = w.n8;
@@ -784,7 +798,7 @@
           const bool last = kiter == itmax - 1;
           db_cluster_pass(pr, k, w.pnew, hidden_from, last ? w.dbuf : nullptr, 1, last ? 1 : 0,
                           last ? nullptr : w.JTe_new, 1, t0, t1, nullptr, 1.0, true, w.pold,
-                          true);
+                          true, last ? k_next : -1, pblk_next);
         } else {
           db_cluster_pass(pr, k, w.pnew, w.dbuf, nullptr, 1, 0, os ? nullptr : w.JTe_new, 1, t0, t1,
                           wt, 1.0, true);
@@ -953,23 +967,40 @@
   const double beta = pr->world > 1 ? pr->beta : 1.0;
   const bool form = !os && pr->world <= 1 && d.h_clus[k].nchunk == 1 && r == pr->res &&
                     db_cluster_pass_forms_hidden(d.N, d.Nbase);
+  const int handoff = db_opt(DB_OPT_HANDOFF);
+  const bool handoff_on = handoff > 0 || (handoff == 0 && 128.0 * d.R > (double)db_l2_bytes());
+  const bool opened = form && w.next_tag == k;
+  w.next_tag = -1;
+  const int k_next = (form && handoff_on && w.open_next >= 0 && d.h_clus[w.open_next].nchunk == 1 &&
+                      !g_aug && db_cluster_pass_opens_next(d.N, d.Nbase))
+                         ? w.open_next : -1;
+  const double *pblk_next = k_next >= 0 ? d.pp + d.h_chunk_poff[d.h_clus[k_next].chunk0] : nullptr;
   if (beta != 1.0 || form)
     DB_CHECK(cudaMemcpyAsync(w.pold, pblk_dev, sizeof(double) * w.n8, cudaMemcpyDeviceToDevice,
                              d.stream));
-  db_cluster_pass(pr, k, pblk_dev, r, form ? nullptr : w.dbuf, 0, form ? 0 : 1,
-                  os ? nullptr : w.JTe, 2, t0, t1, nullptr, beta);
+  if (opened) {
+    DB_CHECK(cudaMemcpyAsync(w.JTe, w.JTe_next, sizeof(double) * w.n8, cudaMemcpyDeviceToDevice,
+                             d.stream));
+    DB_CHECK(cudaMemcpyAsync(d.scal + 2, w.cost_next, sizeof(double), cudaMemcpyDeviceToDevice,
+                             d.stream));
+  } else {
+    db_cluster_pass(pr, k, pblk_dev, r, form ? nullptr : w.dbuf, 0, form ? 0 : 1,
+                    os ? nullptr : w.JTe, 2, t0, t1, nullptr, beta);
+  }
   const double c0 = nan("");
   int nu = 2;
   bool ev;
   LmOut o;
   lm_core(pr, k, ck, t0, t1, pblk_dev, nullptr, itmax, opts ? opts : defopts, linsolv, os, 0,
-          randomize, true, c0, &nu, &ev, form ? r : nullptr, &o);
+          randomize, true, c0, &nu, &ev, form ? r : nullptr, &o, k_next, pblk_next);
   if (o.res_in_dbuf) {
     pr->res = w.dbuf;
     w.dbuf = r;
+    w.next_tag = k_next;
   } else if (form) {
     db_cluster_pass(pr, k, pblk_dev, r, r, 3, 1, nullptr, 1, t0, t1, nullptr, 1.0, false,
-                    w.pold, true);
+                    w.pold, true, k_next, pblk_next);
+    w.next_tag = k_next;
   } else {
     db_cluster_pass(pr, k, pblk_dev, w.dbuf, r, 3, 1, nullptr, 1, t0, t1, nullptr, beta,
                     false, beta != 1.0 ? w.pold : nullptr);
@@ -1284,7 +1315,9 @@
                                             const double *pblk, const double *pblk_old,
                                             const double *in, const double *wt,
                                             const double *out_init, int inplace, double *out,
-                                            double *jte, double *cost) {
+                                            double *jte, double *cost, int clus_next,
+                                            const double *pblk_next, double *jte_next,
+                                            double *cost_next) {
   DevProblem &d = pr->d;
   if (clus < 0 || clus >= d.M || chunk < 0 || chunk >= d.h_clus[clus].nchunk) return -1;
   if (mode < 0 || mode > 4 || (mode == 4 && !with_jte) || ((mode == 2 || mode == 3) && with_jte))
@@ -1293,26 +1326,39 @@
       ((mode != 1 && mode != 3) || wt || !db_cluster_pass_forms_hidden(d.N, d.Nbase)))
     return -1;
   if (!pblk_old && (form_hidden || (mode == 3 && beta != 1.0))) return -1;
-  db_lm_init(pr);
-  LMWork &w = pr->lm;
-  const int n = w.n8;
   int t0, t1;
   chunk_range(d, clus, chunk, &t0, &t1);
+  if (clus_next >= 0 &&
+      (clus_next >= d.M || d.h_clus[clus_next].nchunk != 1 || !form_hidden || with_jte ||
+       beta != 1.0 || t0 != 0 || t1 != d.tilesz || !pblk_next || !jte_next || !cost_next ||
+       !db_cluster_pass_opens_next(d.N, d.Nbase)))
+    return -1;
+  db_lm_init(pr);
+  LMWork &w = pr->lm;
+  const int n = w.n8;
   double2 *vin = dalloc<double2>((size_t)4 * d.R);
   double2 *vout = inplace ? vin : dalloc<double2>((size_t)4 * d.R);
   double2 *vwt = wt ? dalloc<double2>((size_t)4 * d.R) : nullptr;
-  double *pb = dalloc<double>((size_t)2 * n);
+  double *pb = dalloc<double>((size_t)3 * n);
   db_upload_vis(pr, in, vin);
   if (!inplace) db_upload_vis(pr, out_init, vout);
   if (wt) db_upload_vis(pr, wt, vwt);
   DB_CHECK(cudaMemcpyAsync(pb, pblk, sizeof(double) * n, cudaMemcpyHostToDevice, d.stream));
   if (pblk_old)
     DB_CHECK(cudaMemcpyAsync(pb + n, pblk_old, sizeof(double) * n, cudaMemcpyHostToDevice, d.stream));
+  if (clus_next >= 0)
+    DB_CHECK(cudaMemcpyAsync(pb + 2 * n, pblk_next, sizeof(double) * n, cudaMemcpyHostToDevice,
+                             d.stream));
   const int slot = mode == 0 ? 2 : 1;
   const int kernel = db_cluster_pass(pr, clus, pb, vin, vout, mode, write_out,
                                      with_jte ? w.JTe : nullptr, slot, t0, t1, vwt, beta, false,
-                                     pblk_old ? pb + n : nullptr, form_hidden != 0);
+                                     pblk_old ? pb + n : nullptr, form_hidden != 0,
+                                     clus_next >= 0 ? clus_next : -1, pb + 2 * n);
   db_download_vis(pr, vout, out);
+  if (clus_next >= 0) {
+    DB_CHECK(cudaMemcpy(jte_next, w.JTe_next, sizeof(double) * n, cudaMemcpyDeviceToHost));
+    DB_CHECK(cudaMemcpy(cost_next, w.cost_next, sizeof(double), cudaMemcpyDeviceToHost));
+  }
   if (with_jte)
     DB_CHECK(cudaMemcpy(jte, w.JTe, sizeof(double) * n, cudaMemcpyDeviceToHost));
   else
diff --git a/sagecal_b200/csrc/problem.cu b/sagecal_b200/csrc/problem.cu
--- a/sagecal_b200/csrc/problem.cu
+++ b/sagecal_b200/csrc/problem.cu
@@ -84,6 +84,7 @@
   if (!strcmp(name, "rtr_nu_unjoined")) { g_opt[DB_OPT_RTR_NU_UNJOINED] = value; return 0; }
   if (!strcmp(name, "admm_lm")) { g_opt[DB_OPT_ADMM_LM] = value; return 0; }
   if (!strcmp(name, "sweep_residual")) { g_opt[DB_OPT_SWEEP_RESIDUAL] = value; return 0; }
+  if (!strcmp(name, "handoff")) { g_opt[DB_OPT_HANDOFF] = value; return 0; }
   return -1;
 }
 int db_sm_count() {
@@ -93,6 +94,18 @@
   if (!n[dev]) {
     int v = 0;
     if (cudaDeviceGetAttribute(&v, cudaDevAttrMultiProcessorCount, dev) != cudaSuccess || v <= 0) v = 132;
+    n[dev] = v;
+  }
+  return n[dev];
+}
+
+long long db_l2_bytes() {
+  static long long n[64];
+  int dev = 0;
+  if (cudaGetDevice(&dev) != cudaSuccess || dev < 0 || dev >= 64) return 50ll << 20;
+  if (!n[dev]) {
+    int v = 0;
+    if (cudaDeviceGetAttribute(&v, cudaDevAttrL2CacheSize, dev) != cudaSuccess || v <= 0) v = 50 << 20;
     n[dev] = v;
   }
   return n[dev];
@@ -291,6 +304,7 @@
     exit(1);
   }
   dirac_b200_problem *pr = new dirac_b200_problem();
+  pr->lm.open_next = pr->lm.next_tag = -1;
   memset(&pr->d, 0, sizeof(DevProblem));
   DevProblem &d = pr->d;
   d.N = N; d.Nbase = Nbase; d.tilesz = tilesz; d.M = M; d.Mt = Mt;
diff --git a/sagecal_b200/csrc/problem.h b/sagecal_b200/csrc/problem.h
--- a/sagecal_b200/csrc/problem.h
+++ b/sagecal_b200/csrc/problem.h
@@ -34,6 +34,11 @@
   double *bt_ws;
   BigChol *bc;
   double *jte_part;
+  double *JTe_next;
+  double *cost_next;
+  double *cost_part;
+  int open_next;
+  int next_tag;
   bool step_armed, step_fused;
   double *jtj_spec;
   cudaEvent_t ev_mail;
diff --git a/sagecal_b200/csrc/rtr.cu b/sagecal_b200/csrc/rtr.cu
--- a/sagecal_b200/csrc/rtr.cu
+++ b/sagecal_b200/csrc/rtr.cu
@@ -11,7 +11,8 @@
 int db_cluster_pass(dirac_b200_problem *pr, int k, const double *pblk_dev, const double2 *in,
                     double2 *out, int mode, int write_out, double *jte_dev, int cost_slot, int t0,
                     int t1, const double2 *wt, double beta, bool jte_zeroed,
-                    const double *pblk_old, bool form_hidden = false);
+                    const double *pblk_old, bool form_hidden = false, int k_next = -1,
+                    const double *pblk_next = nullptr);
 void db_chunk_range(const DevProblem &d, int k, int ck, int *t0, int *t1);
 
 struct RtrWork {
diff --git a/sagecal_b200/csrc/sage.cu b/sagecal_b200/csrc/sage.cu
--- a/sagecal_b200/csrc/sage.cu
+++ b/sagecal_b200/csrc/sage.cu
@@ -75,6 +75,12 @@
   int weighted_iter = 0;
   const int total_iter = MG * max_iter;
   const int iter_bar = (int)ceil((0.80 / (double)MG) * ((double)total_iter));
+  auto plain_visit = [&](int ci, int cl) {
+    const bool plain = solver_mode == SM_LM_LBFGS ||
+                       (solver_mode == SM_OSLM_LBFGS && ci == max_emiter - 1);
+    return plain && !sharded && linsolv == 0 && !pr->aug_rho && hc[cl].nchunk == 1;
+  };
+  if (pr->lm.ready) pr->lm.next_tag = -1;
   for (int ci = 0; ci < max_emiter; ci++) {
     if (sharded) {
       DB_CHECK(cudaMemcpyAsync(pr->pm, pr->res, sizeof(double2) * 4 * d.R, cudaMemcpyDeviceToDevice,
@@ -101,6 +107,16 @@
       }
       if (this_itermax > 0) {
         double init_res = 0.0, final_res = 0.0;
+        int open_next = -1;
+        if (plain_visit(ci, cl)) {
+          if (cl + 1 < M) {
+            const int nb = weighted_iter ? (int)((0.20 * nerr[cg + 1]) * ((double)total_iter)) + iter_bar
+                                         : max_iter;
+            if (nb > 0 && plain_visit(ci, cl + 1)) open_next = cl + 1;
+          } else if (ci + 1 < max_emiter && plain_visit(ci + 1, 0)) {
+            open_next = 0;
+          }
+        }
         const bool hr = db_cluster_needs_rowmap(pr, cj);
         if (hr) db_cluster_hidden(pr, cj, pr->res, +1, pr->world > 1 ? pr->beta : 1.0);
         for (int ck = 0; ck < hc[cj].nchunk; ck++) {
@@ -121,11 +137,15 @@
             db_lm_set_aug(pr->aug_dev + poff, pr->aug_dev + d.npar + poff, pr->aug_y_host + poff,
                           pr->aug_bz_host + poff, pr->aug_rho[cg]);
           if (solver_mode == SM_OSLM_LBFGS) {
+            pr->lm.open_next = open_next;
             db_lm_chunk(pr, cj, ck, pblk, pr->res, this_itermax, opts, linsolv, last ? 0 : 1,
                         randomize, info, hr);
+            pr->lm.open_next = -1;
           } else if (solver_mode == SM_LM_LBFGS) {
+            pr->lm.open_next = open_next;
             db_lm_chunk(pr, cj, ck, pblk, pr->res, this_itermax, opts, linsolv, 0, randomize, info,
                         hr);
+            pr->lm.open_next = -1;
           } else if (solver_mode == SM_RLM_RLBFGS) {
             if (last) {
               double nu = robust_nu0;
diff --git a/sagecal_b200/lib.py b/sagecal_b200/lib.py
--- a/sagecal_b200/lib.py
+++ b/sagecal_b200/lib.py
@@ -403,15 +403,16 @@
                               nulow, nuhigh, C.byref(nu), dptr(info))
         return p, info, nu.value
 
-    CLUSTER_PASS_KERNELS = ("lin", "lin_grad", "split", "tile", "none")
+    CLUSTER_PASS_KERNELS = ("lin", "lin_grad", "split", "tile", "none", "lin_next")
 
     def cluster_pass(self, clus, chunk, mode, pblk, x, write_out=True, with_jte=False,
                      form_hidden=False, beta=1.0, pblk_old=None, wt=None, out_init=None,
-                     inplace=False):
+                     inplace=False, clus_next=None, pblk_next=None):
         L = self.api.lib
         L.dirac_b200_cluster_pass_eval.restype = C.c_int
         L.dirac_b200_cluster_pass_eval.argtypes = ([C.c_void_p] + [C.c_int] * 6 + [C.c_double]
-                                                   + [c_double_p] * 5 + [C.c_int] + [c_double_p] * 3)
+                                                   + [c_double_p] * 5 + [C.c_int] + [c_double_p] * 3
+                                                   + [C.c_int] + [c_double_p] * 3)
         f64 = lambda v: None if v is None else np.ascontiguousarray(v, dtype=np.float64)
         pblk, pblk_old, x, wt = f64(pblk), f64(pblk_old), f64(x), f64(wt)
         out_init = np.zeros(self.n) if out_init is None else f64(out_init)
@@ -419,12 +420,17 @@
         jte = np.full(8 * self.N, np.nan)
         cost = np.full(1, np.nan)
         opt = lambda v: dptr(v) if v is not None else None
+        pblk_next = f64(pblk_next)
+        jte_next = np.full(8 * self.N, np.nan)
+        cost_next = np.full(1, np.nan)
         k = L.dirac_b200_cluster_pass_eval(self.h, clus, chunk, mode, int(write_out), int(with_jte),
                                            int(form_hidden), beta, dptr(pblk), opt(pblk_old),
                                            dptr(x), opt(wt), dptr(out_init), int(inplace),
-                                           dptr(out), dptr(jte), dptr(cost))
+                                           dptr(out), dptr(jte), dptr(cost),
+                                           -1 if clus_next is None else int(clus_next),
+                                           opt(pblk_next), dptr(jte_next), dptr(cost_next))
         return dict(kernel=None if k < 0 else self.CLUSTER_PASS_KERNELS[k], out=out, jte=jte,
-                    cost=float(cost[0]))
+                    cost=float(cost[0]), jte_next=jte_next, cost_next=float(cost_next[0]))
 
     def cluster_hidden(self, clus, sign, beta, pp, r, dh):
         L = self.api.lib
```

New measurement: 7.721 billion (median of 6 runs). 1.04x the previous value.
